# tiborcamargo/KinectPy

Hardware: AMD Instinct MI355X
Metric: Mpoints/sec end-to-end (unproject+filter+ICP), 4-sensor frame (higher is better)
Workload: dtype f64 decisions / f32 storage

## Files before the change

include/kinectpx.h:

```cpp
#ifndef KINECTPX_H
#define KINECTPX_H

#include <stddef.h>
#include <stdint.h>

#ifdef __cplusplus
extern "C" {
#endif

#define KPX_VERSION 100

typedef enum {
    KPX_OK = 0,
    KPX_ERR_INVALID = -1,
    KPX_ERR_WORKSPACE = -2,
    KPX_ERR_RANGE = -3,
    KPX_ERR_HIP = -4,
    KPX_RETRY = 1
} kpx_status;

const char *kpx_last_error(void);
int kpx_version(void);


// ... 124 lines not shown
size_t kpx_kabsch_workspace_bytes(int64_t n_corr);
int kpx_kabsch(const float *src, const float *tgt, const int32_t *corr, int64_t n_corr, double *d_T, void *ws,
               size_t ws_bytes, void *stream);

#define KPX_ICP_POINT_TO_POINT 0
#define KPX_ICP_POINT_TO_PLANE 1
#define KPX_ICP_FIXED 2
size_t kpx_icp_workspace_bytes(int64_t n_src, int64_t n_tgt);
int kpx_icp(const float *src, int64_t n_src, const float *tgt, const float *tgt_normals, int64_t n_tgt,
            double max_dist, const double *h_init, int32_t mode, int32_t max_iteration, double relative_fitness,
            double relative_rmse, int32_t poll_interval, double *d_result, int32_t *idx, double *d2, void *ws,
            size_t ws_bytes, void *stream);


size_t kpx_fpfh_workspace_bytes(int64_t n, int32_t max_nn);
int kpx_fpfh(const float *pts, const float *normals, int64_t n, double radius, int32_t max_nn, double *fpfh, void *ws,
             size_t ws_bytes, void *stream);

size_t kpx_feature_nn_workspace_bytes(int64_t na, int64_t nb);
int kpx_feature_nn(const double *fa, int64_t na, const double *fb, int64_t nb, int32_t *idx, void *ws, size_t ws_bytes,
                   void *stream);

size_t kpx_ransac_workspace_bytes(int64_t n_src, int64_t n_tgt);
int kpx_ransac_corres(const float *src, int64_t n_src, const float *tgt, int64_t n_tgt, const int32_t *corres, int64_t n_corres,
                      double max_dist, int32_t ransac_n, double edge_similarity, int32_t max_iteration, double confidence,
                      uint64_t seed, double *h_result, void *ws, size_t ws_bytes, void *stream);

size_t kpx_icp_batch_workspace_bytes(int32_t count, const int64_t *h_n_src, int64_t n_tgt);
int kpx_icp_batch(int32_t count, const float *const *h_src, const int64_t *h_n_src, const float *tgt,
                  const float *tgt_normals, int64_t n_tgt, double max_dist, const double *h_init, int32_t mode,
                  int32_t max_iteration, double relative_fitness, double relative_rmse, double *d_results, void *ws,
                  size_t ws_bytes, void *stream);

#define KPX_NN_ENGINE_CULLED 0
#define KPX_NN_ENGINE_DENSE 1
#define KPX_NN_ENGINE_DENSE_FP64 2
int kpx_nn_engine(int32_t engine);

size_t kpx_sample_workspace_bytes(int64_t n);
int kpx_sample_points(const float *pts, int64_t n, int64_t k, uint64_t seed, float *out_pts, int32_t *out_idx, void *ws,
                      size_t ws_bytes, void *stream);

size_t kpx_obb_workspace_bytes(int32_t count, int64_t n);
int kpx_obb_batch(const void *pts, int32_t pts_f64, int32_t count, int64_t n, double *d_obb, uint8_t *d_is_vertex, void *ws,
                  size_t ws_bytes, void *stream);

#define KPX_NORM_OBB 0
#define KPX_NORM_OBB_ROT_TRANS 1
#define KPX_NORM_TRANSLATE 2
#define KPX_NORM_OBB_ROT 3
int kpx_normalize_batch(const double *x, int32_t count, int64_t rows, const double *d_obb, int32_t mode, const double *h_M,
                        double *out, void *stream);

size_t kpx_color_gradient_workspace_bytes(int64_t n, int32_t max_nn);
int kpx_color_gradient(const float *pts, const float *normals, const float *colors, int64_t n, double radius, int32_t max_nn,
                       double *grad, void *ws, size_t ws_bytes, void *stream);
size_t kpx_colored_icp_workspace_bytes(int64_t n_src, int64_t n_tgt);
int kpx_colored_icp(const float *src, const float *src_colors, int64_t n_src, const float *tgt, const float *tgt_colors,
                    const float *tgt_normals, const double *tgt_gradient, int64_t n_tgt, double max_dist, const double *h_init,
                    double lambda_geometric, int32_t max_iteration, double relative_fitness, double relative_rmse,
                    int32_t poll_interval, double *d_result, void *ws, size_t ws_bytes, void *stream);

int kpx_gicp_covariances(const float *normals, int64_t n, double epsilon, double *cov, void *stream);
int kpx_rotate_covariances(const double *cov, int64_t n, const double *h_T, double *out, void *stream);
size_t kpx_generalized_icp_workspace_bytes(int64_t n_src, int64_t n_tgt);
int kpx_generalized_icp(const float *src, const double *src_cov, int64_t n_src, const float *tgt, const double *tgt_cov, int64_t n_tgt,
                        double max_dist, const double *h_init, int32_t max_iteration, double relative_fitness, double relative_rmse,
                        int32_t poll_interval, double *d_result, int32_t *idx, double *d2, void *ws, size_t ws_bytes, void *stream);

int kpx_fuse_skeletons(const double *skeletons, int32_t cams, int64_t frames, int32_t joints, double alpha, double beta,
                       int32_t initial_frame, double *out, void *stream);

typedef struct {
    double reg_voxel;
    double icp_max_dist;
    double filt_voxel;
    double filt_ratio;
    double gate;
    int32_t normals_nn;
    int32_t icp_mode;
    int32_t icp_max_iteration;
    int32_t filt_k;
} kpx_frame_params;
size_t kpx_frame_step_workspace_bytes(int32_t sensors, int64_t n_px);
int kpx_frame_step(const uint16_t *depth, const uint8_t *rgb, const float *xy_table, int64_t n_px, int32_t sensors,
                   const double *h_init, const kpx_frame_params *params, float *out_pts, float *out_col, int32_t *h_count,
                   double *h_T, int32_t *h_info, void *ws, size_t ws_bytes, void *stream);
size_t kpx_frame_step_host_workspace_bytes(int32_t sensors, int64_t n_px);
int kpx_frame_step_host(const uint16_t *h_depth, const uint8_t *h_rgb, const float *xy_table, int64_t n_px, int32_t sensors,
                        const double *h_init, const kpx_frame_params *params, float *out_pts, float *out_col, int32_t *h_count,
                        double *h_T, int32_t *h_info, void *ws, size_t ws_bytes, void *stream);

typedef struct kpx_comm kpx_comm;
typedef int (*kpx_bcast_fn)(void *user, void *d_buf, size_t bytes, int32_t root, void *stream);
typedef int (*kpx_allgather_fn)(void *user, const void *d_send, void *d_recv, size_t bytes_per_rank, void *stream);
int kpx_rccl_load(const char *path);
int kpx_rccl_unique_id(void *id128);
int kpx_comm_create_rccl(const void *id128, int32_t rank, int32_t world, kpx_comm **out);
int kpx_comm_create_callbacks(int32_t rank, int32_t world, kpx_bcast_fn bcast, kpx_allgather_fn allgather, void *user, kpx_comm **out);
int kpx_comm_create_replay(int32_t rank, int32_t world, int32_t frames, int32_t first_frame, int32_t stride, int32_t per_frame,
                           const void *const *d_payloads, const size_t *bytes, kpx_comm **out);
int kpx_comm_destroy(kpx_comm *comm);
int kpx_comm_rank(const kpx_comm *comm);
int kpx_comm_world(const kpx_comm *comm);
int kpx_comm_broadcast(kpx_comm *comm, void *d_buf, size_t bytes, int32_t root, void *stream);
int kpx_comm_allgather(kpx_comm *comm, const void *d_send, void *d_recv, size_t bytes_per_rank, void *stream);
int kpx_copy_bytes(void *dst, const void *src, size_t bytes, void *stream, int32_t wait);

typedef struct kpx_order kpx_order;
int kpx_order_create(int32_t depth, kpx_order **out);
int kpx_order_destroy(kpx_order *order);
int kpx_order_submit(kpx_order *order, int64_t *frame);
int kpx_order_block(kpx_order *order, int64_t frame);
int kpx_order_turn_begin(kpx_order *order, int64_t frame, int32_t stage);
int kpx_order_turn_end(kpx_order *order, int64_t frame, int32_t stage);
int kpx_order_skip(kpx_order *order, int64_t frame, int32_t stage);
int kpx_order_finish(kpx_order *order, int64_t frame);
int kpx_order_log(kpx_order *order, int64_t *out, int64_t cap, int64_t *count);

size_t kpx_frame_step_sharded_workspace_bytes(int32_t sensors, int32_t rank, int32_t world, int64_t n_px, int32_t host_input);
int kpx_frame_step_sharded(kpx_comm *comm, kpx_order *order, int64_t frame, const uint16_t *depth, const uint8_t *rgb, int32_t host_input,
                           const float *xy_table, int64_t n_px, int32_t sensors, const double *h_init, const kpx_frame_params *params,
                           int32_t fused_filter, float *out_pts, float *out_col, int32_t *h_count, double *h_T, int32_t *h_info, void *ws,
                           size_t ws_bytes, void *stream);

typedef struct kpx_stream kpx_stream;
size_t kpx_stream_workspace_bytes(int32_t sensors, int32_t rank, int32_t world, int64_t n_px, int32_t depth);
int kpx_stream_create(const float *xy_table, int64_t n_px, int32_t sensors, const double *h_init, const kpx_frame_params *params,
                      int32_t depth, kpx_comm *const *comms, int32_t fused_filter, void *ws, size_t ws_bytes, kpx_stream **out);
int kpx_stream_submit(kpx_stream *stream, const void *depth, const void *rgb, int32_t host_input, float *out_pts, float *out_col);
int kpx_stream_pop(kpx_stream *stream, int32_t *h_count, double *h_T, int32_t *h_info);
int kpx_stream_pending(const kpx_stream *stream);
int kpx_stream_capacity(const kpx_stream *stream);
int kpx_stream_destroy(kpx_stream *stream);
int kpx_stream_stats(const kpx_stream *stream, uint64_t *h_out4);

#define KPX_PROF_NN_MFMA 0
#define KPX_PROF_SOR_KNN 1
#define KPX_PROF_PLANE_SCORE 2
#define KPX_PROF_COMPACT 3
#define KPX_PROF_NN_SCREEN 4
#define KPX_PROF_NN_LOCAL 5
#define KPX_PROF_KERNELS 6
int kpx_prof_begin(int32_t capacity);
int kpx_prof_stride(int32_t stride);
int kpx_prof_end(double *h_ms, int64_t *h_launches, double *h_work);
int kpx_prof_icp_phases(double *h_out8);
int kpx_prof_icp_waves(uint64_t *h_out, int64_t cap_waves, int64_t *h_count);
int kpx_icp_chain(int32_t on);
int kpx_prof_icp_cert(uint64_t *h_out8);
int kpx_prof_icp_chain(uint64_t *h_out3072);

#ifdef __cplusplus
}
#endif
#endif
```

kinectpy_amd/_lib.py:

```python
import ctypes as C
import threading
import weakref
import os

import torch

_HERE = os.path.dirname(os.path.abspath(__file__))
SO_PATH = os.environ.get("KPX_LIBRARY") or os.path.join(_HERE, "libkinectpx.so")

_i64, _i32, _f64, _u64, _vp, _sz = C.c_int64, C.c_int32, C.c_double, C.c_uint64, C.c_void_p, C.c_size_t

SIGNATURES = {
    "kpx_last_error": (C.c_char_p, []),
    "kpx_version": (C.c_int, []),
    "kpx_unproject_u16": (C.c_int, [_vp, _vp, _i64, _i32, _vp, _vp]),
    "kpx_median_workspace_bytes": (_sz, [_i32]),
    "kpx_median_i16": (C.c_int, [_vp, _i64, _i64, _i32, _vp, _vp, _sz, _vp]),
    "kpx_compact_workspace_bytes": (_sz, [_i64, _i32]),
    "kpx_rgbd_compact": (C.c_int, [_vp, _vp, _i64, _i32, _i32, _vp, _f64, _vp, _vp, _vp, _vp, _vp, _sz, _vp]),
    "kpx_depth_to_cloud_workspace_bytes": (_sz, [_i64, _i32]),
    "kpx_depth_to_cloud": (C.c_int, [_vp, _vp, _vp, _i64, _i32, _i32, _f64, _vp, _vp, _vp, _vp, _vp, _sz, _vp]),
    "kpx_transform": (C.c_int, [_vp, _i64, _vp, _vp, _vp]),
    "kpx_rotate": (C.c_int, [_vp, _i64, _vp, _vp, _vp]),
    "kpx_joints_affine_f64": (C.c_int, [_vp, _i64, _vp, _vp, _vp, _vp]),
# ... 8 lines not shown
    "kpx_voxel_workspace_bytes": (_sz, [_i64]),
    "kpx_voxel_downsample": (C.c_int, [_vp, _vp, _vp, _i64, _f64, _vp, _vp, _vp, _vp, _vp, _sz, _vp]),
    "kpx_voxel_batch_workspace_bytes": (_sz, [_i32, _vp]),
    "kpx_voxel_downsample_batch": (C.c_int, [_i32, _vp, _vp, _vp, _f64, _vp, _vp, _vp, _vp, _sz, _vp]),
    "kpx_fuse_voxel_workspace_bytes": (_sz, [_i64]),
    "kpx_fuse_voxel_downsample": (C.c_int, [_i32, _vp, _vp, _vp, _vp, _f64, _vp, _vp, _vp, _vp, _sz, _vp]),
    "kpx_sor_workspace_bytes": (_sz, [_i64, _i32]),
    "kpx_sor": (C.c_int, [_vp, _i64, _i32, _f64, _vp, _vp, _vp, _vp, _vp, _sz, _vp]),
    "kpx_sor_partial": (C.c_int, [_vp, _i64, _i32, _i64, _i64, _vp, _vp, _vp, _sz, _vp]),
    "kpx_sor_finish_workspace_bytes": (_sz, [_i64]),
    "kpx_sor_finish": (C.c_int, [_vp, _vp, _i64, _f64, _vp, _vp, _vp, _vp, _vp, _sz, _vp]),
    "kpx_dbscan_workspace_bytes": (_sz, [_i64]),
    "kpx_cluster_dbscan": (C.c_int, [_vp, _i64, _f64, _i32, _vp, _vp, _vp, _sz, _vp]),
    "kpx_radius_outlier_workspace_bytes": (_sz, [_i64]),
    "kpx_remove_radius_outlier": (C.c_int, [_vp, _i64, _i32, _f64, _vp, _vp, _vp, _sz, _vp]),
    "kpx_fps_workspace_bytes": (_sz, [_i32, _i64]),
    "kpx_farthest_point_sample": (C.c_int, [_vp, _i64, _i32, _i32, _vp, _vp, _vp, _sz, _vp]),
    "kpx_farthest_point_sample_batch": (C.c_int, [_i32, _vp, _vp, _i32, _i32, _vp, _vp, _vp, _sz, _vp]),
    "kpx_normals_workspace_bytes": (_sz, [_i64, _i32]),
    "kpx_estimate_normals": (C.c_int, [_vp, _i64, _f64, _i32, _vp, _vp, _sz, _vp]),
    "kpx_segment_plane_workspace_bytes": (_sz, [_i64, _i32, _i32]),
    "kpx_segment_plane": (C.c_int, [_vp, _i64, _f64, _i32, _i32, _f64, _u64, _vp, _vp, _vp, _vp, _sz, _vp]),
    "kpx_nn_workspace_bytes": (_sz, [_i64, _i64]),
    "kpx_nn_search": (C.c_int, [_vp, _i64, _vp, _i64, _vp, _vp, _vp, _vp, _sz, _vp]),
    "kpx_registration_eval_workspace_bytes": (_sz, [_i64, _i64]),
    "kpx_registration_eval": (C.c_int, [_vp, _i64, _vp, _i64, _vp, _f64, _vp, _vp, _vp, _vp, _sz, _vp]),
    "kpx_kabsch_workspace_bytes": (_sz, [_i64]),
    "kpx_kabsch": (C.c_int, [_vp, _vp, _vp, _i64, _vp, _vp, _sz, _vp]),
    "kpx_icp_workspace_bytes": (_sz, [_i64, _i64]),
    "kpx_icp": (C.c_int, [_vp, _i64, _vp, _vp, _i64, _f64, _vp, _i32, _i32, _f64, _f64, _i32, _vp, _vp, _vp, _vp, _sz, _vp]),
    "kpx_fpfh_workspace_bytes": (_sz, [_i64, _i32]),
    "kpx_fpfh": (C.c_int, [_vp, _vp, _i64, _f64, _i32, _vp, _vp, _sz, _vp]),
    "kpx_feature_nn_workspace_bytes": (_sz, [_i64, _i64]),
    "kpx_feature_nn": (C.c_int, [_vp, _i64, _vp, _i64, _vp, _vp, _sz, _vp]),
    "kpx_ransac_workspace_bytes": (_sz, [_i64, _i64]),
    "kpx_ransac_corres": (C.c_int, [_vp, _i64, _vp, _i64, _vp, _i64, _f64, _i32, _f64, _i32, _f64, _u64, _vp, _vp, _sz, _vp]),
    "kpx_sample_workspace_bytes": (_sz, [_i64]),
    "kpx_sample_points": (C.c_int, [_vp, _i64, _i64, _u64, _vp, _vp, _vp, _sz, _vp]),
    "kpx_obb_workspace_bytes": (_sz, [_i32, _i64]),
    "kpx_obb_batch": (C.c_int, [_vp, _i32, _i32, _i64, _vp, _vp, _vp, _sz, _vp]),
    "kpx_normalize_batch": (C.c_int, [_vp, _i32, _i64, _vp, _i32, _vp, _vp, _vp]),
    "kpx_color_gradient_workspace_bytes": (_sz, [_i64, _i32]),
    "kpx_color_gradient": (C.c_int, [_vp, _vp, _vp, _i64, _f64, _i32, _vp, _vp, _sz, _vp]),
    "kpx_colored_icp_workspace_bytes": (_sz, [_i64, _i64]),
    "kpx_colored_icp": (C.c_int, [_vp, _vp, _i64, _vp, _vp, _vp, _vp, _i64, _f64, _vp, _f64, _i32, _f64, _f64, _i32, _vp, _vp, _sz, _vp]),
    "kpx_covariances_workspace_bytes": (_sz, [_i64, _i32]),
    "kpx_estimate_covariances": (C.c_int, [_vp, _i64, _f64, _i32, _vp, _vp, _sz, _vp]),
    "kpx_gicp_covariances": (C.c_int, [_vp, _i64, _f64, _vp, _vp]),
    "kpx_rotate_covariances": (C.c_int, [_vp, _i64, _vp, _vp, _vp]),
    "kpx_generalized_icp_workspace_bytes": (_sz, [_i64, _i64]),
    "kpx_generalized_icp": (C.c_int, [_vp, _vp, _i64, _vp, _vp, _i64, _f64, _vp, _i32, _f64, _f64, _i32, _vp, _vp, _vp, _vp, _sz, _vp]),
    "kpx_fuse_skeletons": (C.c_int, [_vp, _i32, _i64, _i32, _f64, _f64, _i32, _vp, _vp]),
    "kpx_nn_engine": (C.c_int, [_i32]),
    "kpx_icp_batch_workspace_bytes": (_sz, [_i32, _vp, _i64]),
    "kpx_icp_batch": (C.c_int, [_i32, _vp, _vp, _vp, _vp, _i64, _f64, _vp, _i32, _i32, _f64, _f64, _vp, _vp, _sz, _vp]),
    "kpx_prof_begin": (C.c_int, [_i32]),
    "kpx_prof_stride": (C.c_int, [_i32]),
    "kpx_frame_step_workspace_bytes": (_sz, [_i32, _i64]),
    "kpx_frame_step": (C.c_int, [_vp, _vp, _vp, _i64, _i32, _vp, _vp, _vp, _vp, _vp, _vp, _vp, _vp, _sz, _vp]),
    "kpx_frame_step_host_workspace_bytes": (_sz, [_i32, _i64]),
    "kpx_frame_step_host": (C.c_int, [_vp, _vp, _vp, _i64, _i32, _vp, _vp, _vp, _vp, _vp, _vp, _vp, _vp, _sz, _vp]),
    "kpx_rccl_load": (C.c_int, [_vp]),
    "kpx_rccl_unique_id": (C.c_int, [_vp]),
    "kpx_comm_create_rccl": (C.c_int, [_vp, _i32, _i32, _vp]),
    "kpx_comm_create_callbacks": (C.c_int, [_i32, _i32, _vp, _vp, _vp, _vp]),
    "kpx_comm_create_replay": (C.c_int, [_i32, _i32, _i32, _i32, _i32, _i32, _vp, _vp, _vp]),
    "kpx_comm_destroy": (C.c_int, [_vp]),
    "kpx_comm_rank": (C.c_int, [_vp]),
    "kpx_comm_world": (C.c_int, [_vp]),
    "kpx_comm_broadcast": (C.c_int, [_vp, _vp, _sz, _i32, _vp]),
    "kpx_comm_allgather": (C.c_int, [_vp, _vp, _vp, _sz, _vp]),
    "kpx_copy_bytes": (C.c_int, [_vp, _vp, _sz, _vp, _i32]),
    "kpx_order_create": (C.c_int, [_i32, _vp]),
    "kpx_order_destroy": (C.c_int, [_vp]),
    "kpx_order_submit": (C.c_int, [_vp, _vp]),
    "kpx_order_block": (C.c_int, [_vp, _i64]),
    "kpx_order_turn_begin": (C.c_int, [_vp, _i64, _i32]),
    "kpx_order_turn_end": (C.c_int, [_vp, _i64, _i32]),
    "kpx_order_skip": (C.c_int, [_vp, _i64, _i32]),
    "kpx_order_finish": (C.c_int, [_vp, _i64]),
    "kpx_order_log": (C.c_int, [_vp, _vp, _i64, _vp]),
    "kpx_frame_step_sharded_workspace_bytes": (_sz, [_i32, _i32, _i32, _i64, _i32]),
    "kpx_frame_step_sharded": (C.c_int, [_vp, _vp, _i64, _vp, _vp, _i32, _vp, _i64, _i32, _vp, _vp, _i32, _vp, _vp, _vp, _vp, _vp, _vp, _sz, _vp]),
    "kpx_stream_workspace_bytes": (_sz, [_i32, _i32, _i32, _i64, _i32]),
    "kpx_stream_create": (C.c_int, [_vp, _i64, _i32, _vp, _vp, _i32, _vp, _i32, _vp, _sz, _vp]),
    "kpx_stream_submit": (C.c_int, [_vp, _vp, _vp, _i32, _vp, _vp]),
    "kpx_stream_pop": (C.c_int, [_vp, _vp, _vp, _vp]),
    "kpx_stream_pending": (C.c_int, [_vp]),
    "kpx_stream_capacity": (C.c_int, [_vp]),
    "kpx_stream_destroy": (C.c_int, [_vp]),
    "kpx_stream_stats": (C.c_int, [_vp, _vp]),
    "kpx_sor_select": (C.c_int, [_vp, _vp, C.c_int64, C.c_int32, C.c_double, _vp, _vp, _vp, _vp, _vp, _vp, C.c_size_t, _vp]),
    "kpx_sort_pairs_u32_workspace_bytes": (C.c_size_t, [C.c_int64]),
    "kpx_sort_pairs_u32": (C.c_int, [_vp, _vp, C.c_int64, C.c_int32, _vp, _vp, _vp, C.c_size_t, _vp]),
    "kpx_prof_icp_phases": (C.c_int, [_vp]),
    "kpx_prof_icp_waves": (C.c_int, [_vp, C.c_int64, _vp]),
    "kpx_icp_chain": (C.c_int, [C.c_int32]),
    "kpx_prof_icp_cert": (C.c_int, [_vp]),
    "kpx_prof_icp_chain": (C.c_int, [_vp]),
    "kpx_prof_end": (C.c_int, [_vp, _vp, _vp]),
}

_lib = None


class KinectPxError(RuntimeError):
    pass


def load():
    global _lib
    if _lib is None:
        if not os.path.exists(SO_PATH):
            raise KinectPxError(
                f"{SO_PATH} is missing: build it with `python -c 'import __graft_entry__ as g; g.build()'` "
                "(make -C kinectpy_amd/csrc).  There is no CPU fallback.")
        lib = C.CDLL(SO_PATH)
        for name, (res, args) in SIGNATURES.items():
            fn = getattr(lib, name)
            fn.restype, fn.argtypes = res, args
        _lib = lib
    return _lib


BCAST_FN = C.CFUNCTYPE(C.c_int, C.c_void_p, C.c_void_p, C.c_size_t, C.c_int32, C.c_void_p)
ALLGATHER_FN = C.CFUNCTYPE(C.c_int, C.c_void_p, C.c_void_p, C.c_void_p, C.c_size_t, C.c_void_p)
RETRY = 1


def check(rc):
    if rc != 0:
        msg = load().kpx_last_error().decode() or f"kpx error {rc}"
        raise KinectPxError(msg)


_gpu_checked = False


def device():
    global _gpu_checked
    if not _gpu_checked:
        if not torch.cuda.is_available():
            raise KinectPxError("no ROCm device visible: the kinectpx hot path runs on MI355X only (no CPU fallback)")
        torch.cuda.current_device()
        _gpu_checked = True
    return torch.device("cuda", torch._C._cuda_getDevice())


def _raw_stream():
    device()
    return torch._C._cuda_getCurrentRawStream(torch._C._cuda_getDevice())


def stream_ptr():
    return C.c_void_p(_raw_stream())


def ptr(t):
    if t is None:
        return None
    assert t.is_cuda and t.is_contiguous(), "kinectpx needs contiguous device tensors"
    return C.c_void_p(t.data_ptr())


def hptr(a):
    return a.ctypes.data_as(C.c_void_p)
# ... 49 lines not shown
```

kinectpy_amd/csrc/kpx_common.h:

```cpp
#pragma once
#include <stdlib.h>
#include <hip/hip_runtime.h>
#include <stdint.h>
#include <stdio.h>
#include <string.h>

#include "../../include/kinectpx.h"

#define KPX_EXPORT extern "C" __attribute__((visibility("default")))

namespace kpx {

extern thread_local char g_err[512];
int fail(int code, const char *fmt, ...);

#define KPX_HIP(call)                                                                              \
    do {                                                                                           \
        hipError_t e__ = (call);                                                                   \
        if (e__ != hipSuccess)                                                                     \
            return kpx::fail(KPX_ERR_HIP, "%s failed: %s (%s:%d)", #call, hipGetErrorString(e__),  \
                             __FILE__, __LINE__);                                                  \
    } while (0)
#define KPX_LAUNCH_CHECK() KPX_HIP(hipGetLastError())
#define KPX_REQUIRE(cond, ...)                                                                     \
    do {                                                                                           \
        if (!(cond)) return kpx::fail(KPX_ERR_INVALID, __VA_ARGS__);                               \
    } while (0)

struct Arena {
    char *base;
    size_t off, cap;
    bool dry;
    explicit Arena(void *p, size_t bytes) : base((char *)p), off(0), cap(bytes), dry(p == nullptr) {}
    template <class T> T *get(size_t count)
    {
        size_t bytes = (count * sizeof(T) + 255) & ~(size_t)255;
        T *r = dry ? nullptr : (T *)(base + off);
        off += bytes;
        return r;
    }
    bool ok() const { return dry || off <= cap; }
};
#define KPX_ARENA_CHECK(a)                                                                         \
    do {                                                                                           \
        if (!(a).ok())                                                                             \
            return kpx::fail(KPX_ERR_WORKSPACE, "workspace too small: need %zu bytes, have %zu",   \
                             (a).off, (a).cap);                                                    \
    } while (0)

static inline int64_t cdiv(int64_t a, int64_t b) { return (a + b - 1) / b; }

bool memo_bytes_lookup(unsigned site, int64_t n, size_t *bytes);
void memo_bytes_store(unsigned site, int64_t n, size_t bytes);
template <class F> static inline size_t memo_bytes(unsigned site, int64_t n, F &&query)
{
    size_t b = 0;
    if (memo_bytes_lookup(site, n, &b)) return b;
    b = query();
    memo_bytes_store(site, n, b);
    return b;
}

typedef unsigned int kpx_u4 __attribute__((ext_vector_type(4)));
template <class V> __device__ __forceinline__ V stream_load16(const V *p)
{
    static_assert(sizeof(V) == 16, "16-byte vectors only");
#ifdef KPX_STREAM_PLAIN
    return *p;
#else
    const kpx_u4 r = __builtin_nontemporal_load(reinterpret_cast<const kpx_u4 *>(p));
    V v;
    __builtin_memcpy(&v, &r, 16);
    return v;
#endif
}
template <class V> __device__ __forceinline__ void stream_store16(const V &v, V *p)
{
    static_assert(sizeof(V) == 16, "16-byte vectors only");
#ifdef KPX_STREAM_PLAIN
    *p = v;
#else
    kpx_u4 r;
    __builtin_memcpy(&r, &v, 16);
    __builtin_nontemporal_store(r, reinterpret_cast<kpx_u4 *>(p));
#endif
}
#define KPX_STREAM_LOAD(p) stream_load16(p)
#define KPX_STREAM_STORE(v, p) stream_store16((v), (p))

bool prof_armed();
struct ProfScope {
    int slot;
    hipStream_t st;
    ProfScope(int kernel_id, double work, hipStream_t stream);
    ~ProfScope();
};

constexpr int kWave = 64;

__device__ __forceinline__ int lane_id() { return threadIdx.x & 63; }
__device__ __forceinline__ int wave_id() { return threadIdx.x >> 6; }

template <class T> __device__ __forceinline__ T wave_sum(T v)
{
#pragma unroll
    for (int o = 32; o > 0; o >>= 1) v += __shfl_down(v, o, 64);
    return v;
}
template <class T> __device__ __forceinline__ T wave_min(T v)
{
#pragma unroll
    for (int o = 32; o > 0; o >>= 1) { T t = __shfl_down(v, o, 64); v = t < v ? t : v; }
    return v;
}
template <class T> __device__ __forceinline__ T wave_max(T v)
{
#pragma unroll
    for (int o = 32; o > 0; o >>= 1) { T t = __shfl_down(v, o, 64); v = t > v ? t : v; }
    return v;
}

__device__ __forceinline__ void wave_lds_fence()
{
    __builtin_amdgcn_fence(__ATOMIC_SEQ_CST, "wavefront");
    __builtin_amdgcn_wave_barrier();
}

template <class T> __device__ __forceinline__ T block_sum(T v, T *sh)
{
    v = wave_sum(v);
    __syncthreads();
// ... 365 lines not shown
```

kinectpy_amd/csrc/kpx_extract.hip:

```cpp
#include <stdarg.h>

#include <mutex>

#include "kpx_internal.h"

namespace kpx {

thread_local char g_err[512] = "";
int fail(int code, const char *fmt, ...)
{
    va_list ap;
    va_start(ap, fmt);
    vsnprintf(g_err, sizeof(g_err), fmt, ap);
    va_end(ap);
    return code;
}

static struct {
    bool on = false;
    int stride = 1;
    long long total[KPX_PROF_KERNELS] = {};
    int cap = 0, used = 0;
    hipEvent_t *e0 = nullptr, *e1 = nullptr;
    int *kid = nullptr;
// ... 353 lines not shown
        });
        if (run_cnt) atomicAdd(&mine[run_bin], run_cnt);
    }
    __syncthreads();
    uint32_t c[8];
    int64_t mine_sum = 0;
    {
#pragma unroll
        for (int q = 0; q < 8; ++q) c[q] = 0u;
#pragma unroll
        for (int cp = 0; cp < kMedCopies; ++cp) {
            const uint4 a4 = reinterpret_cast<const uint4 *>(fh + (size_t)cp * kMedWin)[2 * tid], b4 = reinterpret_cast<const uint4 *>(fh + (size_t)cp * kMedWin)[2 * tid + 1];
            c[0] += a4.x; c[1] += a4.y; c[2] += a4.z; c[3] += a4.w; c[4] += b4.x; c[5] += b4.y; c[6] += b4.z; c[7] += b4.w;
        }
#pragma unroll
        for (int q = 0; q < 8; ++q) mine_sum += (int64_t)c[q];
    }
    int64_t incl = mine_sum;
#pragma unroll
    for (int o = 1; o < 64; o <<= 1) { const int64_t t2 = __shfl_up(incl, o, 64); if (lane >= o) incl += t2; }
    if (lane == 63) wsum[wave] = incl;
    __syncthreads();
    if (tid == 0) {
        int64_t runs = 0;
        for (int w = 0; w < kMedFrameThreads / 64; ++w) { const int64_t t2 = wsum[w]; wsum[w] = runs; runs += t2; }
        wsum[kMedFrameThreads / 64] = runs;
        int64_t below = 0;
        for (int b = 0; b < 128; ++b) below += (int64_t)coarse[b];
        const int64_t inwin = runs;
        for (int w = 0; w < 2; ++w) {
            const int64_t r = rank[w];
            if (r < below) {
                int64_t cum = 0;
                for (int b = 0; b < 128; ++b) { if (r < cum + (int64_t)coarse[b]) { s_bin[w] = b; s_rank[w] = r - cum; break; } cum += (int64_t)coarse[b]; }
            } else if (r >= below + inwin) {
                int64_t cum = below + inwin;
                for (int b = 160; b < 256; ++b) { if (r < cum + (int64_t)coarse[b]) { s_bin[w] = b; s_rank[w] = r - cum; break; } cum += (int64_t)coarse[b]; }
            } else {
                s_rank[w] = r - below;
            }
        }
    }
    __syncthreads();
    const int64_t excl = wsum[wave] + incl - mine_sum;
#pragma unroll
    for (int w = 0; w < 2; ++w) {
        const int64_t r = s_rank[w];
        if (s_bin[w] < 0 && r >= excl && r < excl + mine_sum) {
            int64_t cum = excl;
            int found = -1;
#pragma unroll
            for (int q = 0; q < 8; ++q) {
                if (found < 0 && r < cum + (int64_t)c[q]) found = 8 * tid + q;
                cum += (int64_t)c[q];
            }
            s_val[w] = found;
        }
    }
    __syncthreads();
    for (int w = 0; w < 2; ++w) {
        const int b = s_bin[w];
        if (b < 0) continue;
        if (w == 1 && s_bin[0] == b && s_rank[0] == s_rank[1]) { if (tid == 0) s_val[1] = s_val[0]; __syncthreads(); continue; }
        if (tid < 256) fh[tid] = 0u;
        __syncthreads();
        median_frame_scan(p, n, stride, frame_stride, vec, xy, nanmask, [&](uint32_t raw) {
            const unsigned key = (raw & 0xFFFFu) ^ 0x8000u;
            if ((int)(key >> 8) == b) atomicAdd(&fh[key & 255u], 1u);
        });
        __syncthreads();
        if (tid == 0) {
            int64_t cum = 0;
            const int64_t r = s_rank[w];
            for (int q = 0; q < 256; ++q) {
                if (r < cum + (int64_t)fh[q]) { s_val[w] = (int)(int16_t)(uint16_t)((((unsigned)b << 8) | (unsigned)q) ^ 0x8000u); break; }
                cum += (int64_t)fh[q];
            }
        }
        __syncthreads();
    }
    if (tid == 0) d_median[frame] = 0.5 * ((double)s_val[0] + (double)s_val[1]);
}

static int median_impl(const int16_t *v, int64_t n, int64_t stride, int64_t frame_stride, int32_t frames,
                       double *d_median, Arena &a, hipStream_t st, const float *xy = nullptr, void *clear_from = nullptr)
{
    uint32_t *hist = a.get<uint32_t>((size_t)frames * 512);
    MedianSel *sel = a.get<MedianSel>((size_t)frames);
    uint8_t *nanmask = (xy || (a.dry && n > 0)) ? a.get<uint8_t>((size_t)(n / 8 + 1)) : nullptr;
    if (a.dry) return KPX_OK;
    KPX_ARENA_CHECK(a);
    {
        char *c0 = clear_from ? reinterpret_cast<char *>(clear_from) : reinterpret_cast<char *>(hist);
        KPX_HIP(hipMemsetAsync(c0, 0, (size_t)(reinterpret_cast<char *>(hist + (size_t)frames * 512) - c0), st));
    }
    const bool vec = stride == 1 && (n % 8 == 0) && (frame_stride % 8 == 0) && ((uintptr_t)v % 16 == 0) && ((uintptr_t)xy % 16 == 0);
    if (xy && vec)
        hipLaunchKernelGGL(xy_nanmask_kernel, dim3((unsigned)(cdiv(n / 8, 256) > 1024 ? 1024 : cdiv(n / 8, 256))), dim3(256), 0, st, xy, n / 8, nanmask);
    {
        const char *e = getenv("KPX_MEDIAN_FRAME");
        const bool by_frame = e ? e[0] == '1' : (frames >= 64 && n >= 32768);
        if (by_frame) {
            static bool attr_set = false;
            if (!attr_set) {
                KPX_HIP(hipFuncSetAttribute((const void *)median_frame_kernel, hipFuncAttributeMaxDynamicSharedMemorySize, kMedCopies * kMedWin * 4));
                attr_set = true;
            }
            hipLaunchKernelGGL(median_frame_kernel, dim3(frames), dim3(kMedFrameThreads), (size_t)kMedCopies * kMedWin * 4, st, v, n, stride, frame_stride, d_median,
                               xy, (const uint8_t *)(vec ? nanmask : nullptr));
            KPX_LAUNCH_CHECK();
            return KPX_OK;
        }
    }
    const int per_thread = frames >= 64 ? 64 : (frames >= 16 ? 32 : 16);
    int bx = (int)(cdiv(n, 256 * per_thread) < 1 ? 1 : (cdiv(n, 256 * per_thread) > 512 ? 512 : cdiv(n, 256 * per_thread)));
    dim3 grid(bx, frames);
    hipLaunchKernelGGL(median_hist_kernel, grid, dim3(256), 0, st, v, n, stride, frame_stride, sel, hist, 0, xy, nanmask);
    hipLaunchKernelGGL(median_select_kernel, dim3(frames), dim3(64), 0, st, hist, n, sel, d_median, 0);
    hipLaunchKernelGGL(median_hist_kernel, grid, dim3(256), 0, st, v, n, stride, frame_stride, sel, hist, 1, xy, nanmask);
    hipLaunchKernelGGL(median_select_kernel, dim3(frames), dim3(64), 0, st, hist, n, sel, d_median, 1);
    KPX_LAUNCH_CHECK();
    return KPX_OK;
}

struct XyzPred {
    const int16_t *xyz; const uint8_t *rgb; const double *median; int64_t n; int flags; double gate;
    __device__ bool operator()(int64_t i, int f) const
    {
        const int16_t *p = xyz + ((int64_t)f * n + i) * 3;
        int16_t x = p[0], y = p[1], z = p[2];
        bool keep = (x != 0) & (y != 0) & (z != 0);
        if ((flags & KPX_COMPACT_COLOR_MASK) && rgb) {
            const uint8_t *c = rgb + ((int64_t)f * n + i) * 3;
            keep = keep & (c[0] != 0) & (c[1] != 0) & (c[2] != 0);
        }
        if (flags & KPX_COMPACT_DEPTH_GATE) keep = keep & ((double)z <= median[f] + gate);
        return keep;
    }
};
struct XyzEmit {
    const int16_t *xyz; const uint8_t *rgb; int64_t n; float *pts; float *col; int32_t *idx;
    __device__ void operator()(int64_t i, int f, int32_t dst) const
    {
        const int16_t *p = xyz + ((int64_t)f * n + i) * 3;
        int64_t o = ((int64_t)f * n + dst) * 3;
        pts[o] = (float)p[0]; pts[o + 1] = (float)p[1]; pts[o + 2] = (float)p[2];
        if (col && rgb) {
            const uint8_t *c = rgb + ((int64_t)f * n + i) * 3;
            col[o] = (float)((double)c[0] / 255.0); col[o + 1] = (float)((double)c[1] / 255.0); col[o + 2] = (float)((double)c[2] / 255.0);
        }
        if (idx) idx[(int64_t)f * n + dst] = (int32_t)i;
    }
};

struct DepthPred {
    const uint16_t *depth; const float *xy; const uint8_t *rgb; const double *median; int64_t n; int flags; double gate;
    __device__ bool operator()(int64_t i, int f) const
    {
        int16_t x, y, z;
        unproject1(depth[(int64_t)f * n + i], xy[2 * i], xy[2 * i + 1], x, y, z);
        bool keep = (x != 0) & (y != 0) & (z != 0);
        if ((flags & KPX_COMPACT_COLOR_MASK) && rgb) {
            const uint8_t *c = rgb + ((int64_t)f * n + i) * 3;
            keep = keep & (c[0] != 0) & (c[1] != 0) & (c[2] != 0);
        }
        if (flags & KPX_COMPACT_DEPTH_GATE) keep = keep & ((double)z <= median[f] + gate);
        return keep;
    }
};
struct DepthEmit {
    const uint16_t *depth; const float *xy; const uint8_t *rgb; int64_t n; float *pts; float *col; int32_t *idx;
    __device__ void operator()(int64_t i, int f, int32_t dst) const
    {
        int16_t x, y, z;
        unproject1(depth[(int64_t)f * n + i], xy[2 * i], xy[2 * i + 1], x, y, z);
        int64_t o = ((int64_t)f * n + dst) * 3;
        pts[o] = (float)x; pts[o + 1] = (float)y; pts[o + 2] = (float)z;
        if (col && rgb) {
            const uint8_t *c = rgb + ((int64_t)f * n + i) * 3;
            col[o] = (float)((double)c[0] / 255.0); col[o + 1] = (float)((double)c[1] / 255.0); col[o + 2] = (float)((double)c[2] / 255.0);
        }
// ... 192 lines not shown
__global__ __launch_bounds__(kCompactThreads) void depth_onepass_vec_kernel(const uint16_t *__restrict__ depth, const float *__restrict__ xy,
                                                                            const uint8_t *__restrict__ rgb, const double *__restrict__ median,
                                                                            int64_t n, int flags, double gate, unsigned long long *__restrict__ tile_state,
                                                                            float *__restrict__ pts, float *__restrict__ col, int32_t *__restrict__ idx,
                                                                            int32_t *__restrict__ d_count, int frame_major)
{
    __shared__ int sh[kCompactThreads / 64 + 2];
    __shared__ int16_t sp[kCompactTile * 3];
    __shared__ uint8_t sc[COL ? kCompactTile * 3 : 1];
    __shared__ int32_t si[IDX ? kCompactTile : 1];
    const int f = frame_major ? blockIdx.x : blockIdx.y;
    const unsigned tile = frame_major ? blockIdx.y : blockIdx.x, tiles = frame_major ? gridDim.y : gridDim.x;
    const int64_t base = (int64_t)tile * kCompactTile + (int64_t)threadIdx.x * kCompactItems;
    Px8 p;
    p.keep = 0;
    if (base < n) load_px8(depth, xy, rgb, median, n, f, base, flags, gate, p);
    int tot;
    int pos = block_excl_scan(__builtin_popcount(p.keep), sh, &tot);
#pragma unroll
    for (int k = 0; k < 8; ++k)
        if (p.keep & (1u << k)) {
            sp[3 * pos] = p.x[k]; sp[3 * pos + 1] = p.y[k]; sp[3 * pos + 2] = p.z[k];
            if (COL) { sc[3 * pos] = p.c[3 * k]; sc[3 * pos + 1] = p.c[3 * k + 1]; sc[3 * pos + 2] = p.c[3 * k + 2]; }
            if (IDX) si[pos] = (int32_t)(base + k);
            ++pos;
        }
    __syncthreads();
    const int before = lookback_exclusive(tile_state + (int64_t)f * tiles, tile, tot, sh + kCompactThreads / 64 + 1);
    const int64_t o = (int64_t)f * n + before;
    for (int e = threadIdx.x; e < tot * 3; e += kCompactThreads) {
        pts[o * 3 + e] = (float)sp[e];
        if (COL) col[o * 3 + e] = (float)((double)sc[e] / 255.0);
    }
    if (IDX)
        for (int e = threadIdx.x; e < tot; e += kCompactThreads) idx[o + e] = si[e];
    if (tile == tiles - 1 && threadIdx.x == 0) d_count[f] = before + tot;
}

static int32_t max_compact_frames()
{
    static const int32_t lim = [] {
        int dev = 0, y = 0;
        if (hipGetDevice(&dev) != hipSuccess || hipDeviceGetAttribute(&y, hipDeviceAttributeMaxGridDimY, dev) != hipSuccess || y <= 0) y = 65535;
        return (int32_t)y;
    }();
    return lim;
}
static int px8_compact(const uint16_t *depth, const float *xy, const uint8_t *rgb, const double *med, int64_t n, int32_t frames, int32_t flags,
                       double gate, int32_t *counts, float *pts, float *col, int32_t *idx, int32_t *d_count, hipStream_t st, bool state_is_clear = false)
{
    const int32_t tiles = (int32_t)compact_tiles(n);
    const dim3 grid(tiles, frames), thr(kCompactThreads);
    const bool wc = col && rgb;
    static const bool batch_onepass = [] { const char *e = getenv("KPX_ONEPASS_BATCH"); return !(e && e[0] == '0'); }();
    const bool small = use_onepass((int64_t)tiles * frames);
    const bool frame_major = !small && batch_onepass && frames >= 8 && frames <= 65535;
    const bool onepass = small || frame_major;
    const dim3 ogrid = frame_major ? dim3(frames, tiles) : grid;
    unsigned long long *state = reinterpret_cast<unsigned long long *>(counts);
    if (onepass) { if (!state_is_clear) KPX_HIP(hipMemsetAsync(state, 0, (size_t)tiles * frames * sizeof(unsigned long long), st)); }
    else {
        hipLaunchKernelGGL(depth_count_vec_kernel, grid, thr, 0, st, depth, xy, rgb, med, n, flags, gate, counts);
        hipLaunchKernelGGL(compact_scan_kernel, dim3(frames), dim3(compact_scan_threads(tiles)), 0, st, counts, tiles, d_count);
    }
#define KPX_D2C(COL, IDX)                                                                                                       \
    do {                                                                                                                        \
        if (onepass)                                                                                                            \
            hipLaunchKernelGGL((depth_onepass_vec_kernel<COL, IDX>), ogrid, thr, 0, st, depth, xy, rgb, med, n, flags, gate, state, pts, col, idx, d_count, \
                               frame_major ? 1 : 0);                                                                           \
        else                                                                                                                    \
            hipLaunchKernelGGL((depth_scatter_vec_kernel<COL, IDX>), grid, thr, 0, st, depth, xy, rgb, med, n, flags, gate, counts, pts, col, idx);        \
    } while (0)
    if (wc && idx) KPX_D2C(true, true);
    else if (wc) KPX_D2C(true, false);
    else if (idx) KPX_D2C(false, true);
    else KPX_D2C(false, false);
#undef KPX_D2C
    KPX_LAUNCH_CHECK();
    return KPX_OK;
}

static int depth_to_cloud_impl(const uint16_t *depth, const float *xy, const uint8_t *rgb, int64_t n, int32_t frames,
                               int32_t flags, double gate, float *pts, float *col, int32_t *idx, int32_t *d_count,
                               Arena &a, hipStream_t st)
{
    int32_t *counts = a.get<int32_t>((size_t)frames * compact_ws_ints(n));
    double *med = a.get<double>((size_t)frames);
    int rc = KPX_OK;
    const bool gated = (flags & KPX_COMPACT_DEPTH_GATE) != 0;
    if (gated || a.dry)
        rc = median_impl(reinterpret_cast<const int16_t *>(depth), n, 1, n, frames, med, a, st, xy, counts);
    if (a.dry || rc) return rc;
    KPX_ARENA_CHECK(a);
    DepthPred pred{ depth, xy, rgb, med, n, flags, gate };
    DepthEmit emit{ depth, xy, rgb, n, pts, col, idx };
    ProfScope prof(KPX_PROF_COMPACT, (double)frames * (double)n * (2.0 + (rgb ? 3.0 : 0.0)), st);
    const bool vec = (n % 8 == 0) && (((uintptr_t)depth | (uintptr_t)xy) % 16 == 0) && ((uintptr_t)rgb % 8 == 0);
    if (!vec) return compact(pred, emit, n, frames, counts, d_count, st, gated);
    return px8_compact(depth, xy, rgb, med, n, frames, flags, gate, counts, pts, col, idx, d_count, st, gated);
}
KPX_EXPORT int kpx_rgbd_compact(const int16_t *xyz, const uint8_t *rgb, int64_t n, int32_t frames, int32_t flags,
                                const double *d_median, double gate, float *pts, float *col, int32_t *idx,
                                int32_t *d_count, void *ws, size_t ws_bytes, void *stream)
{
    KPX_REQUIRE(n >= 0 && frames > 0, "kpx_rgbd_compact: bad size");
    KPX_REQUIRE(xyz && pts && d_count && ws, "kpx_rgbd_compact: null pointer");
    KPX_REQUIRE(!(flags & KPX_COMPACT_DEPTH_GATE) || d_median, "kpx_rgbd_compact: depth gate needs d_median");
    KPX_REQUIRE(n < ((int64_t)1 << 31), "kpx_rgbd_compact: frame too large");
    KPX_REQUIRE(frames <= max_compact_frames(), "kpx_rgbd_compact: %d frames exceed the device's grid limit of %d per call", frames, max_compact_frames());
    Arena a(ws, ws_bytes);
    int32_t *counts = a.get<int32_t>((size_t)frames * compact_ws_ints(n));
    KPX_ARENA_CHECK(a);
    XyzPred pred{ xyz, rgb, d_median, n, flags, gate };
    XyzEmit emit{ xyz, rgb, n, pts, col, idx };
    if (n == 0) return compact(pred, emit, n, frames, counts, d_count, (hipStream_t)stream);
    const bool vec = (n % 8 == 0) && ((uintptr_t)xyz % 16 == 0) && ((uintptr_t)rgb % 8 == 0);
    if (!vec) return compact(pred, emit, n, frames, counts, d_count, (hipStream_t)stream);
    return px8_compact(reinterpret_cast<const uint16_t *>(xyz), nullptr, rgb, d_median, n, frames, flags, gate, counts, pts, col, idx, d_count,
                       (hipStream_t)stream);
}

KPX_EXPORT size_t kpx_depth_to_cloud_workspace_bytes(int64_t n_px, int32_t frames)
{
    Arena a(nullptr, 0);
    depth_to_cloud_impl(nullptr, nullptr, nullptr, n_px, frames < 1 ? 1 : frames, KPX_COMPACT_DEPTH_GATE, 0, nullptr,
                        nullptr, nullptr, nullptr, a, nullptr);
    return a.off;
}
KPX_EXPORT int kpx_depth_to_cloud(const uint16_t *depth, const float *xy, const uint8_t *rgb, int64_t n_px,
                                  int32_t frames, int32_t flags, double gate, float *pts, float *col, int32_t *idx,
                                  int32_t *d_count, void *ws, size_t ws_bytes, void *stream)
{
    KPX_REQUIRE(n_px > 0 && frames > 0, "kpx_depth_to_cloud: bad size");
    KPX_REQUIRE(depth && xy && pts && d_count && ws, "kpx_depth_to_cloud: null pointer");
    KPX_REQUIRE(n_px < ((int64_t)1 << 31), "kpx_depth_to_cloud: frame too large");
    KPX_REQUIRE(frames <= max_compact_frames(), "kpx_depth_to_cloud: %d frames exceed the device's grid limit of %d per call", frames, max_compact_frames());
    Arena a(ws, ws_bytes);
    return depth_to_cloud_impl(depth, xy, rgb, n_px, frames, flags, gate, pts, col, idx, d_count, a, (hipStream_t)stream);
}
```

kinectpy_amd/csrc/kpx_frame.hip:

```cpp
#include <chrono>
#include <vector>

#include "kpx_internal.h"

namespace kpx {

__global__ void frame_empty_kernel() {}

__global__ void frame_flag_kernel(unsigned long long *flag, unsigned long long seq)
{
    __hip_atomic_store(flag, seq, __ATOMIC_RELEASE, __HIP_MEMORY_SCOPE_SYSTEM);
}
static int frame_wait(hipStream_t st)
{
    static const bool spin = [] { const char *e = getenv("KPX_FRAME_SPIN"); return !(e && e[0] == '0'); }();
    if (!spin) {
        KPX_HIP(hipStreamSynchronize(st));
        return KPX_OK;
    }
    static thread_local unsigned long long *flag = nullptr;
    static thread_local unsigned long long seq = 0;
    if (!flag) {
        KPX_HIP(hipHostMalloc((void **)&flag, 64, hipHostMallocDefault));
        *flag = 0ull;
    }
    ++seq;
    hipLaunchKernelGGL(frame_flag_kernel, dim3(1), dim3(1), 0, st, flag, seq);
    KPX_LAUNCH_CHECK();
    auto t0 = std::chrono::steady_clock::now();
    for (unsigned spins = 0;; ++spins) {
        if (__atomic_load_n(flag, __ATOMIC_ACQUIRE) == seq) return KPX_OK;
        __builtin_ia32_pause();
        if ((spins & 4095u) == 4095u && std::chrono::steady_clock::now() - t0 > std::chrono::milliseconds(1)) {
            const hipError_t q = hipStreamQuery(st);
            if (q == hipSuccess) {
                if (__atomic_load_n(flag, __ATOMIC_ACQUIRE) == seq) return KPX_OK;
                KPX_HIP(hipStreamSynchronize(st));
                if (__atomic_load_n(flag, __ATOMIC_ACQUIRE) == seq) return KPX_OK;
                return fail(KPX_ERR_HIP, "kpx_frame_step: the frame's completion word never arrived");
            }
            if (q != hipErrorNotReady) return fail(KPX_ERR_HIP, "kpx_frame_step: %s while waiting for a read-back", hipGetErrorString(q));
            t0 = std::chrono::steady_clock::now();
        }
    }
}

struct FrameLayout {
    float *full_pts, *mask_pts, *mask_col, *down_pts, *normals, *vox_pts, *vox_col;
    int32_t *vox_cnt, *keep_idx;
    double *icp_res, *sor_stats;
    void *op_ws;
    size_t op_bytes;
};
static size_t max_sz(size_t a, size_t b) { return a > b ? a : b; }
static void frame_carve(Arena &a, int32_t S, int64_t n_px, FrameLayout *L)
{
    const size_t px = (size_t)n_px, all = (size_t)S * px;
    L->full_pts = a.get<float>(all * 3);
    L->mask_pts = a.get<float>(all * 3);
    L->mask_col = a.get<float>(all * 3);
    L->down_pts = a.get<float>(all * 3);
    L->normals = a.get<float>(px * 3);
    L->vox_pts = a.get<float>(all * 3);
    L->vox_col = a.get<float>(all * 3);
    L->keep_idx = a.get<int32_t>(all);
    L->icp_res = a.get<double>((size_t)S * 20 + 1);
    L->vox_cnt = reinterpret_cast<int32_t *>(L->icp_res + (size_t)S * 20);
    L->sor_stats = a.get<double>(4);
    std::vector<int64_t> worst((size_t)S, n_px);
    size_t w = kpx_depth_to_cloud_workspace_bytes(n_px, S);
    w = max_sz(w, kpx_voxel_batch_workspace_bytes(S, worst.data()));
    w = max_sz(w, kpx_normals_workspace_bytes(n_px, KPX_NORMALS_LDS_NN));
    w = max_sz(w, kpx_icp_batch_workspace_bytes(S > 1 ? S - 1 : 1, worst.data(), n_px));
    w = max_sz(w, kpx_fuse_voxel_workspace_bytes((int64_t)all));
    w = max_sz(w, kpx_sor_workspace_bytes((int64_t)all, KPX_SOR_LDS_K));
    w = max_sz(w, kpx_select_workspace_bytes((int64_t)all));
    L->op_bytes = w;
    L->op_ws = a.get<char>(w);
}

}

using namespace kpx;

KPX_EXPORT size_t kpx_frame_step_workspace_bytes(int32_t sensors, int64_t n_px)
{
    if (sensors < 1 || n_px < 1) return 0;
    Arena a(nullptr, 0);
    FrameLayout L;
    frame_carve(a, sensors, n_px, &L);
    return a.off;
}

#define KPX_SUB(call)                    \
    do {                                 \
        const int rc__ = (call);         \
        if (rc__) return rc__;           \
    } while (0)

KPX_EXPORT int kpx_frame_step(const uint16_t *depth, const uint8_t *rgb, const float *xy_table, int64_t n_px, int32_t sensors,
                              const double *h_init, const kpx_frame_params *prm, float *out_pts, float *out_col, int32_t *h_count,
                              double *h_T, int32_t *h_info, void *ws, size_t ws_bytes, void *stream)
{
    KPX_REQUIRE(sensors >= 1 && sensors <= 16 && n_px > 0 && n_px < ((int64_t)1 << 31) / 16, "kpx_frame_step: 1 .. 16 sensors of at most 2^27 pixels");
    KPX_REQUIRE(depth && rgb && xy_table && prm && out_pts && out_col && h_count && h_T && ws, "kpx_frame_step: null pointer");
    KPX_REQUIRE(sensors == 1 || h_init, "kpx_frame_step: initial transforms missing");
    KPX_REQUIRE(prm->icp_mode == KPX_ICP_POINT_TO_POINT || prm->icp_mode == KPX_ICP_POINT_TO_PLANE || prm->icp_mode == KPX_ICP_FIXED, "kpx_frame_step: bad icp_mode");
    const bool fixed = prm->icp_mode == KPX_ICP_FIXED;
    KPX_REQUIRE(prm->filt_k <= KPX_SOR_LDS_K && prm->normals_nn <= KPX_NORMALS_LDS_NN, "kpx_frame_step: filt_k <= %d and normals_nn <= %d (the frame's scratch is "
                "sized for the LDS forms; kpx_sor / kpx_estimate_normals take larger values)", KPX_SOR_LDS_K, KPX_NORMALS_LDS_NN);
    const int S = sensors;
    hipStream_t st = (hipStream_t)stream;
    BusyScope busy;
    static thread_local struct { void *ws; size_t bytes; int S; int64_t n_px; FrameLayout L; size_t off; } cache = { nullptr, 0, 0, 0, {}, 0 };
    FrameLayout L;
    if (cache.ws == ws && cache.bytes == ws_bytes && cache.S == S && cache.n_px == n_px) {
        L = cache.L;
    } else {
        Arena a(ws, ws_bytes);
        frame_carve(a, S, n_px, &L);
        KPX_ARENA_CHECK(a);
        cache.ws = ws; cache.bytes = ws_bytes; cache.S = S; cache.n_px = n_px; cache.L = L; cache.off = a.off;
    }
    static thread_local double *h_d = nullptr;
    static thread_local int32_t *h_i = nullptr;
    if (!h_i) {
        void *blk = nullptr;
        KPX_HIP(hipHostMalloc(&blk, (16 * 20 + 1) * sizeof(double) + 256 * sizeof(int32_t), hipHostMallocDefault));
        h_d = static_cast<double *>(blk);
        h_i = reinterpret_cast<int32_t *>(h_d + (16 * 20 + 1));
    }
    auto negative = [&](const int32_t *c, int n) { for (int i = 0; i < n; ++i) if (c[i] < 0) return c[i]; return 0; };

    if (!fixed) KPX_SUB(kpx_depth_to_cloud(depth, xy_table, nullptr, n_px, S, 0, prm->gate, L.full_pts, nullptr, nullptr, h_i, L.op_ws, L.op_bytes, st));
    else for (int i = 0; i < S; ++i) h_i[i] = 0;
    KPX_SUB(kpx_depth_to_cloud(depth, xy_table, rgb, n_px, S, KPX_COMPACT_COLOR_MASK | KPX_COMPACT_DEPTH_GATE, prm->gate, L.mask_pts, L.mask_col, nullptr,
                               h_i + 16, L.op_ws, L.op_bytes, st));
    static const int extra_dispatches = [] { const char *e = getenv("KPX_FRAME_EXTRA_DISPATCHES"); return e ? atoi(e) : 0; }();
    for (int e = 0; e < extra_dispatches; ++e) hipLaunchKernelGGL(frame_empty_kernel, dim3(1), dim3(64), 0, st);
    std::vector<int64_t> fk((size_t)S), mk((size_t)S), dk((size_t)S);
    std::vector<const float *> p_in((size_t)S), c_in((size_t)S);
    std::vector<float *> p_out((size_t)S);
    for (int i = 0; i < S; ++i) { p_in[(size_t)i] = L.full_pts + (size_t)i * n_px * 3; p_out[(size_t)i] = L.down_pts + (size_t)i * n_px * 3; }
    KPX_SUB(frame_wait(st));
    for (int i = 0; i < S; ++i) { fk[(size_t)i] = h_i[i]; mk[(size_t)i] = h_i[16 + i]; }
    if (negative(h_i, S) || negative(h_i + 16, S)) return fail(KPX_ERR_RANGE, "kpx_frame_step: extraction reported %d", negative(h_i, S) | negative(h_i + 16, S));
    static const bool zorder_on = [] { const char *e = getenv("KPX_FRAME_ZORDER"); return !(e && e[0] == '0'); }();
    const bool zorder = zorder_on && S <= 8;
    static thread_local int spec_bits = 0;
    static const bool speculate = [] { const char *e = getenv("KPX_FRAME_SPECULATE"); return !(e && e[0] == '0'); }();
    if (!speculate) spec_bits = 0;
    for (int i = 0; i < S; ++i) h_i[32 + i] = 0;
    for (int attempt = 0; attempt < 2 && !fixed; ++attempt) {
        KPX_SUB(voxel_downsample_batch_spec(S, p_in.data(), nullptr, fk.data(), prm->reg_voxel, p_out.data(), nullptr, h_i + 32, L.op_ws, L.op_bytes, st,
                                            attempt == 0 ? spec_bits : 0, h_i + 50, zorder));
        KPX_SUB(frame_wait(st));
        const int need = h_i[50];
        const bool narrow = attempt == 0 && spec_bits > 0 && need > spec_bits;
        spec_bits = need > 0 && need <= 32 ? (need + 7) / 8 * 8 : 0;
        if (!narrow) break;
    }
    if (negative(h_i + 32, S)) return fail(KPX_ERR_RANGE, "voxel_size is too small");
    for (int i = 0; i < S; ++i) dk[(size_t)i] = h_i[32 + i];
    for (int q = 0; q < 16; ++q) h_T[q] = (q % 5 == 0) ? 1.0 : 0.0;
    if (h_info) for (int i = 0; i < S; ++i) { h_info[i] = (int32_t)dk[(size_t)i]; h_info[16 + i] = (int32_t)mk[(size_t)i]; h_info[32 + i] = 0; }
    if (fixed)
        for (int i = 1; i < S; ++i)
            for (int q = 0; q < 16; ++q) h_T[16 * i + q] = h_init[16 * (i - 1) + q];
    if (S > 1 && !fixed) {
        const bool plane = prm->icp_mode == KPX_ICP_POINT_TO_PLANE;
        if (plane) KPX_SUB(kpx_estimate_normals(L.down_pts, dk[0], 2.0 * prm->reg_voxel, prm->normals_nn, L.normals, L.op_ws, L.op_bytes, st));
        std::vector<const float *> subs((size_t)S - 1);
        for (int i = 1; i < S; ++i) {
            KPX_REQUIRE(dk[(size_t)i] >= 1 && dk[0] >= 1, "kpx_frame_step: sensor %d has no valid pixel", dk[0] >= 1 ? i : 0);
            subs[(size_t)i - 1] = p_out[(size_t)i];
        }
        KPX_SUB(icp_batch_ordered(S - 1, subs.data(), dk.data() + 1, L.down_pts, plane ? L.normals : nullptr, dk[0], prm->icp_max_dist, h_init, prm->icp_mode,
                                  prm->icp_max_iteration, 1e-6, 1e-6, L.icp_res, L.op_ws, L.op_bytes, st, zorder));
    }
    std::vector<const double *> dT((size_t)S, nullptr);
    for (int i = 0; i < S; ++i) {
        p_in[(size_t)i] = L.mask_pts + (size_t)i * n_px * 3; c_in[(size_t)i] = L.mask_col + (size_t)i * n_px * 3;
        if (i > 0 && !fixed) dT[(size_t)i] = L.icp_res + 20 * (size_t)(i - 1);
    }
    static thread_local int fuse_spec = 0;
    if (!speculate) fuse_spec = 0;
    for (int attempt = 0; attempt < 2; ++attempt) {
        h_i[51] = 0;
        KPX_SUB(fuse_voxel_downsample_dev(S, p_in.data(), c_in.data(), mk.data(), h_T, dT.data(), prm->filt_voxel, L.vox_pts, L.vox_col, L.vox_cnt, L.op_ws,
                                          L.op_bytes, st, attempt == 0 ? fuse_spec : 0, h_i + 51));
        KPX_HIP(hipMemcpyAsync(h_d, L.icp_res, ((size_t)S * 20 + 1) * sizeof(double), hipMemcpyDeviceToHost, st));
        KPX_SUB(frame_wait(st));
        const int need = h_i[51];
        const bool narrow = attempt == 0 && fuse_spec > 0 && need > fuse_spec;
        fuse_spec = (speculate && need > 0 && need <= 32) ? (need + 7) / 8 * 8 : 0;
        if (!narrow) break;
    }
    h_i[48] = *reinterpret_cast<const int32_t *>(h_d + (size_t)S * 20);
    for (int i = 1; i < S && !fixed; ++i)
        if (h_d[20 * (i - 1) + 16] != h_d[20 * (i - 1) + 16]) {
            (void)icp_chain_abort_take();
            return fail(KPX_ERR_HIP, "kpx_frame_step: the one-launch ICP chain of sensor %d gave up waiting for its blocks to become resident; KPX_ICP_CHAIN=0 "
                                     "selects the launch-per-iteration form", i);
        }
    for (int i = 1; i < S && !fixed; ++i) {
        for (int q = 0; q < 16; ++q) h_T[16 * i + q] = h_d[20 * (i - 1) + q];
        if (h_info) h_info[32 + i] = (int32_t)h_d[20 * (i - 1) + 18];
    }
    if (h_i[48] < 0) return fail(KPX_ERR_RANGE, "voxel_size is too small");
    const int64_t M = h_i[48];
    if (h_info) h_info[48] = (int32_t)M;
    *h_count = 0;
    if (M == 0) return KPX_OK;
    KPX_SUB(kpx_sor_select(L.vox_pts, L.vox_col, M, prm->filt_k, prm->filt_ratio, out_pts, out_col, L.keep_idx, h_i + 49, L.sor_stats, L.op_ws, L.op_bytes, st));
    KPX_SUB(frame_wait(st));
    *h_count = h_i[49];
    return KPX_OK;
}

KPX_EXPORT size_t kpx_frame_step_host_workspace_bytes(int32_t sensors, int64_t n_px)
{
    if (sensors < 1 || n_px < 1) return 0;
    Arena a(nullptr, 0);
    a.get<uint16_t>((size_t)sensors * (size_t)n_px);
    a.get<uint8_t>((size_t)sensors * (size_t)n_px * 3);
    return a.off + kpx_frame_step_workspace_bytes(sensors, n_px);
}

KPX_EXPORT int kpx_frame_step_host(const uint16_t *h_depth, const uint8_t *h_rgb, const float *xy_table, int64_t n_px, int32_t sensors,
                                   const double *h_init, const kpx_frame_params *prm, float *out_pts, float *out_col, int32_t *h_count,
                                   double *h_T, int32_t *h_info, void *ws, size_t ws_bytes, void *stream)
{
    KPX_REQUIRE(sensors >= 1 && sensors <= 16 && n_px > 0 && n_px < ((int64_t)1 << 31) / 16, "kpx_frame_step_host: 1 .. 16 sensors of at most 2^27 pixels");
    KPX_REQUIRE(h_depth && h_rgb && ws, "kpx_frame_step_host: null pointer");
    Arena a(ws, ws_bytes);
    const size_t all = (size_t)sensors * (size_t)n_px;
    uint16_t *d_depth = a.get<uint16_t>(all);
    uint8_t *d_rgb = a.get<uint8_t>(all * 3);
    KPX_ARENA_CHECK(a);
    hipStream_t st = (hipStream_t)stream;
    KPX_HIP(hipMemcpyAsync(d_depth, h_depth, all * sizeof(uint16_t), hipMemcpyHostToDevice, st));
    KPX_HIP(hipMemcpyAsync(d_rgb, h_rgb, all * 3, hipMemcpyHostToDevice, st));
    return kpx_frame_step(d_depth, d_rgb, xy_table, n_px, sensors, h_init, prm, out_pts, out_col, h_count, h_T, h_info, (char *)ws + a.off,
                          ws_bytes - a.off, stream);
}

namespace kpx {

int64_t &comm_cap_master(kpx_comm *c);
int64_t &comm_cap_clouds(kpx_comm *c);
int &comm_spec_bits(kpx_comm *c);
int &comm_fuse_bits(kpx_comm *c);

constexpr int kHdrDoubles = 24;

static int shard_first(int n_sensors, int rank, int world)
{
    const int base = n_sensors / world, rem = n_sensors % world;
    return rank * base + (rank < rem ? rank : rem);
}
static int shard_count(int n_sensors, int rank, int world) { return n_sensors / world + (rank < n_sensors % world ? 1 : 0); }
static int64_t round_cap(int64_t need, int64_t worst)
{
    int64_t c = (need + need / 4 + 4095) / 4096 * 4096;
    if (c < 4096) c = 4096;
    return c < worst ? c : worst;
}

struct ShardHeaderArgs {
    int32_t k_max, local, first_is_master;
    int32_t masked[16], down[16];
};
__global__ void shard_header_kernel(double *hdr, ShardHeaderArgs a, const double *icp_res)
{
    const int j = blockIdx.x, t = threadIdx.x;
    if (t >= kHdrDoubles) return;
    double v = 0.0;
    if (j < a.local) {
        const int sub = j - (a.first_is_master ? 1 : 0);
        if (t == 0) v = (double)a.masked[j];
        else if (t == 1) v = (double)a.down[j];
        else if (t < 22) v = sub >= 0 ? icp_res[20 * sub + (t - 2)] : ((t - 2) < 16 && (t - 2) % 5 == 0 ? 1.0 : 0.0);
    } else if (t >= 2 && t < 18 && (t - 2) % 5 == 0) v = 1.0;
    hdr[j * kHdrDoubles + t] = v;
}

struct ShardLayout {
    uint16_t *stage_depth;
    uint8_t *stage_rgb;
    float *full_pts, *mask_pts, *mask_col, *down_pts, *normals, *vox_pts, *vox_col;
    char *msg_master, *xchg_send, *xchg_recv;
    int32_t *keep_idx, *order_idx, *vox_cnt, *keep_cnt;
    double *avg_send, *avg_all, *icp_res, *sor_stats;
    void *op_ws;
    size_t op_bytes, hdr_bytes;
    int k_max;
};
static void shard_carve(Arena &a, int S, int S_l, int world, int64_t n_px, bool host_input, ShardLayout *L)
{
    const size_t px = (size_t)n_px, loc = (size_t)S_l * px, all = (size_t)S * px;
    L->k_max = (S + world - 1) / world;
    L->hdr_bytes = ((size_t)L->k_max * kHdrDoubles * sizeof(double) + 255) & ~(size_t)255;
    L->stage_depth = host_input ? a.get<uint16_t>(loc) : nullptr;
    L->stage_rgb = host_input ? a.get<uint8_t>(loc * 3) : nullptr;
    L->full_pts = a.get<float>(loc * 3);
    L->mask_pts = a.get<float>(loc * 3);
    L->mask_col = a.get<float>(loc * 3);
    L->down_pts = a.get<float>(loc * 3);
    L->normals = a.get<float>(px * 3);
    L->msg_master = a.get<char>(px * 24 + 256);
    const size_t xmsg = (size_t)L->k_max * px * 24 + L->hdr_bytes;
    L->xchg_send = a.get<char>(xmsg);
    L->xchg_recv = a.get<char>(xmsg * (size_t)world);
    L->vox_pts = a.get<float>(all * 3);
    L->vox_col = a.get<float>(all * 3);
    L->keep_idx = a.get<int32_t>(all);
    L->order_idx = a.get<int32_t>(all);
    const size_t rows = (all + (size_t)world - 1) / (size_t)world;
    L->avg_send = a.get<double>(rows);
    L->avg_all = a.get<double>(rows * (size_t)world);
    L->icp_res = a.get<double>((size_t)(S_l > 0 ? S_l : 1) * 20);
    L->vox_cnt = a.get<int32_t>(64);
    L->keep_cnt = L->vox_cnt + 1;
    L->sor_stats = a.get<double>(4);
    std::vector<int64_t> worst((size_t)(S_l > 0 ? S_l : 1), n_px);
    size_t w = kpx_depth_to_cloud_workspace_bytes(n_px, S_l);
    w = max_sz(w, kpx_voxel_batch_workspace_bytes(S_l, worst.data()));
    w = max_sz(w, kpx_normals_workspace_bytes(n_px, KPX_NORMALS_LDS_NN));
    w = max_sz(w, kpx_icp_batch_workspace_bytes(S_l > 0 ? S_l : 1, worst.data(), n_px));
    w = max_sz(w, kpx_fuse_voxel_workspace_bytes((int64_t)all));
    w = max_sz(w, kpx_sor_workspace_bytes((int64_t)all, KPX_SOR_LDS_K));
    w = max_sz(w, kpx_sor_finish_workspace_bytes((int64_t)all));
    w = max_sz(w, kpx_select_workspace_bytes((int64_t)all));
    L->op_bytes = w;
    L->op_ws = a.get<char>(w);
}

static int pinned_block(char **out)
{
    static thread_local char *blk = nullptr;
    if (!blk) {
        void *p = nullptr;
        KPX_HIP(hipHostMalloc(&p, 32768, hipHostMallocDefault));
        blk = static_cast<char *>(p);
    }
    *out = blk;
    return KPX_OK;
}

}

KPX_EXPORT size_t kpx_frame_step_sharded_workspace_bytes(int32_t sensors, int32_t rank, int32_t world, int64_t n_px, int32_t host_input)
{
    if (sensors < 1 || world < 1 || rank < 0 || rank >= world || world > sensors || n_px < 1) return 0;
    Arena a(nullptr, 0);
    ShardLayout L;
    shard_carve(a, sensors, shard_count(sensors, rank, world), world, n_px, host_input != 0, &L);
    return a.off;
}

KPX_EXPORT int kpx_frame_step_sharded(kpx_comm *comm, kpx_order *order, int64_t frame, const uint16_t *depth, const uint8_t *rgb, int32_t host_input,
                                      const float *xy_table, int64_t n_px, int32_t sensors, const double *h_init, const kpx_frame_params *prm,
                                      int32_t fused_filter, float *out_pts, float *out_col, int32_t *h_count, double *h_T, int32_t *h_info, void *ws,
                                      size_t ws_bytes, void *stream)
{
    KPX_REQUIRE(comm, "kpx_frame_step_sharded: communicator missing (kpx_comm_create_*)");
    const int rank = kpx_comm_rank(comm), world = kpx_comm_world(comm), S = sensors;
    KPX_REQUIRE(S >= 1 && S <= 16 && world <= S && n_px > 0 && n_px < ((int64_t)1 << 31) / 16, "kpx_frame_step_sharded: 1 .. 16 sensors on at most as many ranks");
    KPX_REQUIRE(depth && rgb && xy_table && prm && out_pts && out_col && h_count && h_T && ws, "kpx_frame_step_sharded: null pointer");
    KPX_REQUIRE(S == 1 || h_init, "kpx_frame_step_sharded: initial transforms missing");
    KPX_REQUIRE(prm->icp_mode == KPX_ICP_POINT_TO_POINT || prm->icp_mode == KPX_ICP_POINT_TO_PLANE, "kpx_frame_step_sharded: bad icp_mode");
    KPX_REQUIRE(fused_filter >= 0 && fused_filter <= 2, "kpx_frame_step_sharded: fused_filter is 0 (sharded), 1 (rank 0) or 2 (the frames' fuse + filter dealt round robin)");
    const int owner = fused_filter == 2 ? (int)((frame < 0 ? 0 : frame) % world) : 0;
    KPX_REQUIRE(prm->filt_k <= KPX_SOR_LDS_K && prm->normals_nn <= KPX_NORMALS_LDS_NN, "kpx_frame_step_sharded: filt_k <= %d and normals_nn <= %d", KPX_SOR_LDS_K,
                KPX_NORMALS_LDS_NN);
    hipStream_t st = (hipStream_t)stream;
    BusyScope busy;
    const int g0 = shard_first(S, rank, world), S_l = shard_count(S, rank, world);
    const bool owns_master = g0 == 0, plane = prm->icp_mode == KPX_ICP_POINT_TO_PLANE;
    Arena a(ws, ws_bytes);
    ShardLayout L;
    shard_carve(a, S, S_l, world, n_px, host_input != 0, &L);
    KPX_ARENA_CHECK(a);
    const int K = L.k_max;
    char *pin = nullptr;
    KPX_SUB(pinned_block(&pin));
    double *h_d = reinterpret_cast<double *>(pin);
    int32_t *h_i = reinterpret_cast<int32_t *>(pin + 8192);
    double *h_hdr = reinterpret_cast<double *>(pin + 12288);
    auto negative = [&](const int32_t *c, int n) { for (int i = 0; i < n; ++i) if (c[i] < 0) return c[i]; return 0; };
    *h_count = 0;
    if (h_info) memset(h_info, 0, 64 * sizeof(int32_t));

    if (host_input) {
        KPX_HIP(hipMemcpyAsync(L.stage_depth, depth, (size_t)S_l * n_px * sizeof(uint16_t), hipMemcpyHostToDevice, st));
        KPX_HIP(hipMemcpyAsync(L.stage_rgb, rgb, (size_t)S_l * n_px * 3, hipMemcpyHostToDevice, st));
        depth = L.stage_depth;
        rgb = L.stage_rgb;
    }
    KPX_SUB(kpx_depth_to_cloud(depth, xy_table, nullptr, n_px, S_l, 0, prm->gate, L.full_pts, nullptr, nullptr, h_i, L.op_ws, L.op_bytes, st));
    KPX_SUB(kpx_depth_to_cloud(depth, xy_table, rgb, n_px, S_l, KPX_COMPACT_COLOR_MASK | KPX_COMPACT_DEPTH_GATE, prm->gate, L.mask_pts, L.mask_col, nullptr,
                               h_i + 16, L.op_ws, L.op_bytes, st));
    std::vector<int64_t> fk((size_t)S_l), mk((size_t)S_l), dk((size_t)S_l);
    std::vector<const float *> p_in((size_t)S_l);
    std::vector<float *> p_out((size_t)S_l);
    for (int i = 0; i < S_l; ++i) { p_in[(size_t)i] = L.full_pts + (size_t)i * n_px * 3; p_out[(size_t)i] = L.down_pts + (size_t)i * n_px * 3; }
    KPX_SUB(frame_wait(st));
    for (int i = 0; i < S_l; ++i) { fk[(size_t)i] = h_i[i]; mk[(size_t)i] = h_i[16 + i]; }
    int lerr = KPX_OK;
    if (negative(h_i, S_l) || negative(h_i + 16, S_l)) lerr = fail(KPX_ERR_RANGE, "kpx_frame_step_sharded: extraction reported %d", negative(h_i, S_l) | negative(h_i + 16, S_l));
    static const bool zorder_on = [] { const char *e = getenv("KPX_FRAME_ZORDER"); return !(e && e[0] == '0'); }();
    const bool zorder = zorder_on && K <= 8;
    int &spec_bits = comm_spec_bits(comm);
    for (int attempt = 0; attempt < 2 && !lerr; ++attempt) {
        KPX_SUB(voxel_downsample_batch_spec(S_l, p_in.data(), nullptr, fk.data(), prm->reg_voxel, p_out.data(), nullptr, h_i + 32, L.op_ws, L.op_bytes, st,
                                            attempt == 0 ? spec_bits : 0, h_i + 50, zorder));
        KPX_SUB(frame_wait(st));
        const int need = h_i[50];
        const bool narrow = attempt == 0 && spec_bits > 0 && need > spec_bits;
        spec_bits = need > 0 && need <= 32 ? (need + 7) / 8 * 8 : 0;
        if (!narrow) break;
    }
    if (!lerr && negative(h_i + 32, S_l)) lerr = fail(KPX_ERR_RANGE, "voxel_size is too small");
    for (int i = 0; i < S_l; ++i) dk[(size_t)i] = lerr ? 0 : h_i[32 + i];
    for (int i = 0; i < S_l && !lerr; ++i)
        if (dk[(size_t)i] < 1) lerr = fail(KPX_ERR_INVALID, "kpx_frame_step_sharded: sensor %d has no valid pixel", g0 + i);

    static const bool fixed_cap = [] { const char *e = getenv("KPX_SHARD_FIXED_CAP"); return e && e[0] == '1'; }();
    int64_t &cap_m = comm_cap_master(comm);
    if (cap_m <= 0 || fixed_cap) cap_m = n_px;
    const int64_t capm = cap_m;
    static const bool normals_travel = [] { const char *e = getenv("KPX_SHARD_NORMALS"); return !(e && e[0] == '1'); }();
    const bool ship_n = normals_travel && plane && world > 1;
    const size_t row_b = ship_n ? 24 : 12;
    char *msg = L.msg_master;
    float *m_xyz = reinterpret_cast<float *>(msg), *m_nrm = reinterpret_cast<float *>(msg + (size_t)capm * 12);
    double *m_hdr = reinterpret_cast<double *>(msg + (size_t)capm * row_b);
    if (owns_master) {
        if (!lerr && ship_n) lerr = kpx_estimate_normals(L.down_pts, dk[0], 2.0 * prm->reg_voxel, prm->normals_nn, L.normals, L.op_ws, L.op_bytes, st);
        if (!lerr) {
            const size_t rows = (size_t)(dk[0] < capm ? dk[0] : capm);
            KPX_HIP(hipMemcpyAsync(m_xyz, L.down_pts, rows * 12, hipMemcpyDeviceToDevice, st));
            if (ship_n) KPX_HIP(hipMemcpyAsync(m_nrm, L.normals, rows * 12, hipMemcpyDeviceToDevice, st));
        }
        h_d[0] = lerr ? -1.0 : (double)dk[0];
        KPX_HIP(hipMemcpyAsync(m_hdr, h_d, sizeof(double), hipMemcpyHostToDevice, st));
    }
    kpx_order_turn_begin(order, frame, 0);
    int rc = kpx_comm_broadcast(comm, msg, (size_t)capm * row_b + 256, 0, st);
    kpx_order_turn_end(order, frame, 0);
    if (rc) return rc;
    if (owns_master && lerr) {
        kpx_order_finish(order, frame);
        return lerr;
    }
    int64_t m = owns_master ? dk[0] : 0;
    if (!owns_master) {
        KPX_HIP(hipMemcpyAsync(h_d, m_hdr, sizeof(double), hipMemcpyDeviceToHost, st));
        KPX_SUB(frame_wait(st));
        m = (int64_t)h_d[0];
        if (!(m >= 1 && m <= n_px)) {
            kpx_order_finish(order, frame);
            return m < 0 ? fail(KPX_ERR_RANGE, "kpx_frame_step_sharded: rank 0 could not provide the master cloud (see its error)")
                         : fail(KPX_ERR_RANGE, "kpx_frame_step_sharded: bad master header (%lld points)", (long long)m);
        }
    }
    cap_m = fixed_cap ? n_px : round_cap(m, n_px);
    if (m > capm) {
        kpx_order_finish(order, frame);
        return KPX_RETRY;
    }
    const int n_sub = S_l - (owns_master ? 1 : 0);
    if (n_sub > 0 && !lerr) {
        std::vector<const float *> subs((size_t)n_sub);
        std::vector<int64_t> ns((size_t)n_sub);
        for (int j = 0; j < n_sub; ++j) {
            const int i = j + (owns_master ? 1 : 0);
            subs[(size_t)j] = p_out[(size_t)i];
            ns[(size_t)j] = dk[(size_t)i];
        }
        const float *tgt = owns_master ? L.down_pts : m_xyz, *tn = plane ? ((ship_n && !owns_master) ? m_nrm : L.normals) : nullptr;
        if (plane && !ship_n) lerr = kpx_estimate_normals(tgt, m, 2.0 * prm->reg_voxel, prm->normals_nn, L.normals, L.op_ws, L.op_bytes, st);
        const int first_sub = g0 + (owns_master ? 1 : 0);
        if (!lerr)
            lerr = icp_batch_ordered(n_sub, subs.data(), ns.data(), tgt, tn, m, prm->icp_max_dist, h_init + 16 * (size_t)(first_sub - 1), prm->icp_mode,
                                     prm->icp_max_iteration, 1e-6, 1e-6, L.icp_res, L.op_ws, L.op_bytes, st, zorder);
    }
    int64_t &cap_c = comm_cap_clouds(comm);
    const int64_t worst_c = (int64_t)K * n_px;
    if (cap_c <= 0 || fixed_cap) cap_c = worst_c;
    const int64_t capc = cap_c;
    const size_t xbytes = (size_t)capc * 24 + L.hdr_bytes;
    {
        ShardHeaderArgs ha;
        memset(&ha, 0, sizeof(ha));
        ha.k_max = K; ha.local = S_l; ha.first_is_master = owns_master ? 1 : 0;
        int64_t off = 0;
        for (int i = 0; i < S_l; ++i) {
            ha.masked[i] = lerr ? -1 : (int32_t)mk[(size_t)i]; ha.down[i] = (int32_t)dk[(size_t)i];
            int64_t k = capc - off < mk[(size_t)i] ? capc - off : mk[(size_t)i];
            if (k < 0 || lerr) k = 0;
            if (k > 0) {
                KPX_HIP(hipMemcpyAsync(L.xchg_send + (size_t)off * 12, L.mask_pts + (size_t)i * n_px * 3, (size_t)k * 12, hipMemcpyDeviceToDevice, st));
                KPX_HIP(hipMemcpyAsync(L.xchg_send + (size_t)(capc + off) * 12, L.mask_col + (size_t)i * n_px * 3, (size_t)k * 12, hipMemcpyDeviceToDevice, st));
            }
            off += k;
        }
        hipLaunchKernelGGL(shard_header_kernel, dim3((unsigned)K), dim3(32), 0, st, reinterpret_cast<double *>(L.xchg_send + (size_t)capc * 24), ha, L.icp_res);
        KPX_LAUNCH_CHECK();
    }
    kpx_order_turn_begin(order, frame, 1);
    rc = kpx_comm_allgather(comm, L.xchg_send, L.xchg_recv, xbytes, st);
    kpx_order_turn_end(order, frame, 1);
    if (rc) return rc;
    const size_t hrow = (size_t)K * kHdrDoubles * sizeof(double);
    KPX_HIP(hipMemcpy2DAsync(h_hdr, hrow, L.xchg_recv + (size_t)capc * 24, xbytes, hrow, (size_t)world, hipMemcpyDeviceToHost, st));
    KPX_SUB(frame_wait(st));
    std::vector<const float *> f_p((size_t)S), f_c((size_t)S);
    std::vector<int64_t> f_n((size_t)S);
    int64_t need = 0;
    for (int r = 0, g = 0; r < world; ++r) {
        const int own = shard_count(S, r, world);
        int64_t off = 0;
        for (int j = 0; j < own; ++j, ++g) {
            const double *row = h_hdr + ((size_t)r * K + j) * kHdrDoubles;
            const int64_t n = (int64_t)row[0];
            if (!(n >= 0 && n <= n_px)) {
                kpx_order_finish(order, frame);
                if (lerr) return lerr;
                return n < 0 ? fail(KPX_ERR_RANGE, "kpx_frame_step_sharded: rank %d failed on its own sensors (see its error)", r)
                             : fail(KPX_ERR_RANGE, "kpx_frame_step_sharded: bad exchange header (rank %d)", r);
            }
            if (row[2 + 16] != row[2 + 16]) {
                kpx_order_finish(order, frame);
                (void)icp_chain_abort_take();
                return fail(KPX_ERR_HIP, "kpx_frame_step_sharded: the one-launch ICP chain of sensor %d (rank %d) gave up waiting for its blocks to become "
                                         "resident; KPX_ICP_CHAIN=0 selects the launch-per-iteration form", g, r);
            }
            f_p[(size_t)g] = reinterpret_cast<const float *>(L.xchg_recv + (size_t)r * xbytes + (size_t)off * 12);
            f_c[(size_t)g] = reinterpret_cast<const float *>(L.xchg_recv + (size_t)r * xbytes + (size_t)(capc + off) * 12);
            f_n[(size_t)g] = n;
            for (int q = 0; q < 16; ++q) h_T[16 * g + q] = row[2 + q];
            if (h_info) { h_info[g] = (int32_t)row[1]; h_info[16 + g] = (int32_t)n; h_info[32 + g] = g == 0 ? 0 : (int32_t)row[2 + 18]; }
            off += n;
        }
        need = off > need ? off : need;
    }
    cap_c = fixed_cap ? worst_c : round_cap(need, worst_c);
    if (need > capc) {
        kpx_order_finish(order, frame);
        return KPX_RETRY;
    }
    if (fused_filter >= 1 && rank != owner) {
        kpx_order_skip(order, frame, 2);
        return KPX_OK;
    }
    int &fuse_spec = comm_fuse_bits(comm);
    static const bool speculate_fuse = [] { const char *e = getenv("KPX_FRAME_SPECULATE"); return !(e && e[0] == '0'); }();
    if (!speculate_fuse) fuse_spec = 0;
    for (int attempt = 0; attempt < 2; ++attempt) {
        h_i[51] = 0;
        KPX_SUB(fuse_voxel_downsample_dev(S, f_p.data(), f_c.data(), f_n.data(), h_T, nullptr, prm->filt_voxel, L.vox_pts, L.vox_col, L.vox_cnt, L.op_ws,
                                          L.op_bytes, st, attempt == 0 ? fuse_spec : 0, h_i + 51));
        KPX_HIP(hipMemcpyAsync(h_i + 48, L.vox_cnt, sizeof(int32_t), hipMemcpyDeviceToHost, st));
        KPX_SUB(frame_wait(st));
        const int need_bits = h_i[51];
        const bool narrow = attempt == 0 && fuse_spec > 0 && need_bits > fuse_spec;
        fuse_spec = (speculate_fuse && need_bits > 0 && need_bits <= 32) ? (need_bits + 7) / 8 * 8 : 0;
        if (!narrow) break;
    }
    if (h_i[48] < 0) return fail(KPX_ERR_RANGE, "voxel_size is too small");
    const int64_t M = h_i[48];
    if (h_info) h_info[48] = (int32_t)M;
    if (M == 0) {
        kpx_order_skip(order, frame, 2);
        return KPX_OK;
    }
    if (fused_filter >= 1) {
        kpx_order_skip(order, frame, 2);
        KPX_SUB(kpx_sor_select(L.vox_pts, L.vox_col, M, prm->filt_k, prm->filt_ratio, out_pts, out_col, L.keep_idx, h_i + 49, L.sor_stats, L.op_ws, L.op_bytes, st));
        KPX_SUB(frame_wait(st));
        *h_count = h_i[49];
        return KPX_OK;
    }
    const int64_t rows = (M + world - 1) / world;
    const int64_t q0 = rank * rows < M ? rank * rows : M, q1 = (rank + 1) * rows < M ? (rank + 1) * rows : M;
    KPX_SUB(kpx_sor_partial(L.vox_pts, M, prm->filt_k, q0, q1, L.avg_send, L.order_idx, L.op_ws, L.op_bytes, st));
    kpx_order_turn_begin(order, frame, 2);
    rc = kpx_comm_allgather(comm, L.avg_send, L.avg_all, (size_t)rows * sizeof(double), st);
    kpx_order_turn_end(order, frame, 2);
    if (rc) return rc;
    KPX_SUB(kpx_sor_finish(L.avg_all, L.order_idx, M, prm->filt_ratio, L.keep_idx, L.keep_cnt, L.sor_stats, nullptr, L.op_ws, L.op_bytes, st));
    KPX_HIP(hipMemcpyAsync(h_i + 49, L.keep_cnt, sizeof(int32_t), hipMemcpyDeviceToHost, st));
    KPX_SUB(frame_wait(st));
    const int64_t kept = h_i[49];
    if (kept > 0) {
        KPX_SUB(kpx_select_by_index(L.vox_pts, L.vox_col, nullptr, M, L.keep_idx, kept, KPX_SELECT_GATHER, out_pts, out_col, nullptr, nullptr, L.op_ws,
                                    L.op_bytes, st));
        KPX_SUB(frame_wait(st));
    }
    *h_count = (int32_t)kept;
    return KPX_OK;
}
```

kinectpy_amd/csrc/kpx_internal.h:

```cpp
#pragma once
#include "kpx_common.h"

namespace kpx {

constexpr int kBboxBlocks = 1024;
int bbox_f32(const float *pts, int64_t n, double *d_bbox6, double *ws_partials, hipStream_t st);

struct GridParams {
    double org[3];
    double h;
    int32_t dim[3];
    int32_t ncell;
};
constexpr int32_t kGridMaxCells = 1 << 22;

struct Grid {
    GridParams *params;
    uint32_t *cell_start;
    float *sorted_pts;
    int32_t *sorted_idx;
    uint32_t *sorted_keys;
    int32_t *spare;
    int32_t *extra;
};
constexpr int kGridExtraWords = 4104;
int grid_build(const float *pts, int64_t n, double target_per_cell, Arena &a, Grid *g, hipStream_t st);

constexpr int kLaneCount = 4;
struct LaneSet {
    hipStream_t s[kLaneCount];
    hipEvent_t fork, join[kLaneCount];
};
int lanes_get(LaneSet **out);
int lanes_fork(LaneSet *l, hipStream_t caller, int used);
int lanes_join(LaneSet *l, hipStream_t caller, int used);

int voxel_downsample_batch_spec(int32_t count, const float *const *h_pts, const float *const *h_col, const int64_t *h_n, double voxel,
                                float *const *h_opts, float *const *h_ocol, int32_t *d_counts, void *ws, size_t ws_bytes, void *stream,
                                int spec_bits, int32_t *d_bits, bool morton = false);

int fuse_voxel_downsample_dev(int32_t count, const float *const *h_pts, const float *const *h_col, const int64_t *h_n, const double *h_T,
                              const double *const *h_dT, double voxel, float *opts, float *ocol, int32_t *d_count, void *ws, size_t ws_bytes,
                              void *stream, int spec_bits = 0, int32_t *d_bits = nullptr);

struct BusyScope {
    BusyScope();
    ~BusyScope();
    BusyScope(const BusyScope &) = delete;
    BusyScope &operator=(const BusyScope &) = delete;
    bool counted;
};
int busy_threads();
int icp_chain_abort_take();
int icp_batch_ordered(int32_t count, const float *const *h_src, const int64_t *h_n_src, const float *tgt, const float *tgt_normals, int64_t n_tgt,
                      double max_dist, const double *h_init, int32_t mode, int32_t max_iteration, double relative_fitness, double relative_rmse,
                      double *d_results, void *ws, size_t ws_bytes, void *stream, bool presorted);

double nn_local_take_visits();

}
```

kinectpy_amd/csrc/kpx_knn.hip:

```cpp
#include <hipcub/hipcub.hpp>

#include "kpx_gridknn.h"
#include "kpx_morton.h"
#include "kpx_radix.h"
#include "kpx_linalg.h"

namespace kpx {

__device__ __forceinline__ void grid_dims(const double ext[3], double &h, int32_t cell_cap, int dim[3])
{
    for (;;) {
        double tot = 1.0;
        for (int a = 0; a < 3; ++a) {
            double d = floor(ext[a] / h) + 1.0;
            if (d > 1000000.0) d = 1000000.0;
            dim[a] = (int)d; tot *= d;
        }
        if (tot <= (double)cell_cap) break;
        h *= 1.26;
    }
}
__device__ __forceinline__ GridParams grid_params_of(const double *__restrict__ bbox, int64_t n, double target, int32_t cell_cap,
                                                     const unsigned long long *__restrict__ sumsq)
{
// ... 60 lines not shown
    for (int64_t s = (int64_t)blockIdx.x * blockDim.x + threadIdx.x; s < n; s += (int64_t)gridDim.x * blockDim.x) {
        int64_t i = order[s];
        sorted_pts[3 * s] = pts[3 * i]; sorted_pts[3 * s + 1] = pts[3 * i + 1]; sorted_pts[3 * s + 2] = pts[3 * i + 2];
    }
}
__global__ __launch_bounds__(256) void grid_place_kernel(const uint32_t *__restrict__ cell_of, int64_t n, const uint32_t *__restrict__ cell_start,
                                                         uint32_t *__restrict__ cursor, int32_t *__restrict__ slot_idx)
{
    for (int64_t i = (int64_t)blockIdx.x * blockDim.x + threadIdx.x; i < n; i += (int64_t)gridDim.x * blockDim.x) {
        const uint32_t c = cell_of[i];
        slot_idx[cell_start[c] + atomicAdd(&cursor[c], 1u)] = (int32_t)i;
    }
}
__global__ __launch_bounds__(256) void grid_rank_kernel(const float *__restrict__ pts, int64_t n, const uint32_t *__restrict__ cell_of,
                                                        const uint32_t *__restrict__ cell_start, const int32_t *__restrict__ slot_idx,
                                                        int32_t *__restrict__ sorted_idx, float *__restrict__ sorted_pts)
{
    for (int64_t s = (int64_t)blockIdx.x * blockDim.x + threadIdx.x; s < n; s += (int64_t)gridDim.x * blockDim.x) {
        const int32_t i = slot_idx[s];
        const uint32_t c = cell_of[i];
        const int64_t s0 = cell_start[c], s1 = cell_start[c + 1];
        int rank = 0;
        for (int64_t t = s0; t < s1; ++t) rank += slot_idx[t] < i ? 1 : 0;
        const int64_t d = s0 + rank;
        sorted_idx[d] = i;
        sorted_pts[3 * d] = pts[3 * (int64_t)i]; sorted_pts[3 * d + 1] = pts[3 * (int64_t)i + 1]; sorted_pts[3 * d + 2] = pts[3 * (int64_t)i + 2];
    }
}

constexpr int kGridScanItems = 8, kGridScanTile = 256 * kGridScanItems;
constexpr int kGridScanWords = 2 * ((kGridMaxCells + 1 + kGridScanTile - 1) / kGridScanTile) + 2;
__global__ __launch_bounds__(256) void grid_scan_kernel(const uint32_t *__restrict__ counts, int64_t len, uint32_t *__restrict__ out,
                                                        unsigned long long *__restrict__ states)
{
    __shared__ int sh[256 / 64 + 2];
    const int64_t base = (int64_t)blockIdx.x * kGridScanTile + (int64_t)threadIdx.x * kGridScanItems;
    uint32_t v[kGridScanItems];
    int c = 0;
#pragma unroll
    for (int k = 0; k < kGridScanItems; ++k) { v[k] = base + k < len ? counts[base + k] : 0u; c += (int)v[k]; }
    int tot;
    const int ex = block_excl_scan(c, sh, &tot);
    __syncthreads();
    const int before = lookback_exclusive(states, blockIdx.x, tot, sh + 256 / 64 + 1);
    uint32_t run = (uint32_t)(before + ex);
#pragma unroll
    for (int k = 0; k < kGridScanItems; ++k) {
        if (base + k < len) out[base + k] = run;
        run += v[k];
    }
}

int grid_build(const float *pts, int64_t n, double target_per_cell, Arena &a, Grid *g, hipStream_t st)
{
    const size_t nn = (size_t)(n > 0 ? n : 1);
    g->params = a.get<GridParams>(1);
    uint32_t *zero = a.get<uint32_t>(3 * ((size_t)kGridMaxCells + 1) + 32 + kGridExtraWords + kGridScanWords);
    g->cell_start = a.get<uint32_t>((size_t)kGridMaxCells + 1);
    g->sorted_pts = a.get<float>(nn * 3);
    g->sorted_idx = a.get<int32_t>(nn);
    uint32_t *keys_in = a.get<uint32_t>(nn), *keys_out = a.get<uint32_t>(nn);
    g->sorted_keys = keys_out;
    int32_t *vals_in = a.get<int32_t>(nn);
    double *part = a.get<double>((size_t)kBboxBlocks * 6 + 8);
    size_t sort_bytes = 0, scan_bytes = 0;
    sort_bytes = memo_bytes(2, (int64_t)nn, [&] { size_t b = 0; (void)sort_pairs(nullptr, b, keys_in, keys_out, vals_in, g->sorted_idx, (int64_t)nn, 22, st); return b; });
    scan_bytes = memo_bytes(3, 0, [&] { size_t b = 0; (void)hipcub::DeviceScan::ExclusiveSum(nullptr, b, zero, g->cell_start, kGridMaxCells + 1, st); return b; });
    char *tmp = a.get<char>(sort_bytes > scan_bytes ? sort_bytes : scan_bytes);
    RadixScratch rx{};
    const bool own_sort = (int64_t)nn > 65536 && (int64_t)nn <= kRadixMaxPairs;
    radix_carve(a, (int64_t)nn <= kRadixMaxPairs ? (int64_t)nn : kRadixMaxPairs, &rx);
    if (a.dry) return KPX_OK;
    KPX_ARENA_CHECK(a);
    double *bbox = part + (size_t)kBboxBlocks * 6;
    int rc = bbox_f32(pts, n, bbox, part, st);
    if (rc) return rc;
    int32_t cell_cap = 65536;
    while (cell_cap < kGridMaxCells && (int64_t)cell_cap < 16 * n) cell_cap <<= 1;
    g->spare = reinterpret_cast<int32_t *>(zero);
    unsigned long long *sumsq = reinterpret_cast<unsigned long long *>(zero + 16);
    g->extra = reinterpret_cast<int32_t *>(zero + 32);
    unsigned long long *scan_states = reinterpret_cast<unsigned long long *>(zero + 32 + kGridExtraWords);
    uint32_t *count1 = zero + 32 + kGridExtraWords + kGridScanWords, *count2 = count1 + (size_t)cell_cap + 1, *cursor = count2 + (size_t)cell_cap + 1;
    KPX_HIP(hipMemsetAsync(zero, 0, (32 + kGridExtraWords + kGridScanWords + 3 * ((size_t)cell_cap + 1)) * sizeof(uint32_t), st));
    int nb = (int)(cdiv(n, 256) > 4096 ? 4096 : cdiv(n, 256));
    hipLaunchKernelGGL(grid_cell_kernel, dim3(nb), dim3(256), 0, st, pts, n, bbox, target_per_cell, cell_cap, (const unsigned long long *)nullptr, g->params,
                       keys_in, vals_in, count1);
    hipLaunchKernelGGL(grid_occupancy_kernel, dim3(1024), dim3(256), 0, st, count1, g->params, sumsq);
    hipLaunchKernelGGL(grid_cell_kernel, dim3(nb), dim3(256), 0, st, pts, n, bbox, target_per_cell, cell_cap, (const unsigned long long *)sumsq, g->params,
                       keys_in, vals_in, count2);
    static const bool vendor_scan = [] { const char *e = getenv("KPX_GRID_SCAN"); return e && e[0] == '0'; }();
    if (vendor_scan) KPX_HIP(hipcub::DeviceScan::ExclusiveSum(tmp, scan_bytes, count2, g->cell_start, cell_cap + 1, st));
    else
        hipLaunchKernelGGL(grid_scan_kernel, dim3((unsigned)cdiv((int64_t)cell_cap + 1, kGridScanTile)), dim3(256), 0, st, count2, (int64_t)cell_cap + 1, g->cell_start,
                           scan_states);
    static const bool force_sort = [] { const char *e = getenv("KPX_GRID_SORT"); return e && e[0] == '1'; }();
    const bool by_sort = force_sort || n > 65536;
    if (by_sort) {
        if (own_sort) {
            rc = radix_sort_pairs_u32(rx, keys_in, keys_out, vals_in, g->sorted_idx, n, 22, st);
            if (rc) return rc;
        } else {
            KPX_HIP(sort_pairs(tmp, sort_bytes, keys_in, keys_out, vals_in, g->sorted_idx, n, 22, st));
        }
        hipLaunchKernelGGL(grid_gather_kernel, dim3(nb), dim3(256), 0, st, pts, n, g->sorted_idx, g->sorted_pts);
    } else {
        hipLaunchKernelGGL(grid_place_kernel, dim3(nb), dim3(256), 0, st, keys_in, n, g->cell_start, cursor, vals_in);
        hipLaunchKernelGGL(grid_rank_kernel, dim3(nb), dim3(256), 0, st, pts, n, keys_in, g->cell_start, vals_in, g->sorted_idx, g->sorted_pts);
    }
    KPX_LAUNCH_CHECK();
    return KPX_OK;
}

template <int WAVES>
__global__ __launch_bounds__(WAVES * 64) void sor_wave_kernel(const GridParams *__restrict__ gp, const uint32_t *__restrict__ cell_start,
                                                              const float *__restrict__ spts, const int32_t *__restrict__ sidx,
                                                              int64_t q0, int64_t q1, int k, int cap, double *__restrict__ avg,
                                                              const int32_t *__restrict__ in_list, const int32_t *__restrict__ in_count,
                                                              int32_t *__restrict__ fb_list, int32_t *__restrict__ fb_count)
{
    extern __shared__ __align__(16) double lds[];
    __shared__ uint32_t run_s0[WAVES][64];
    __shared__ int32_t run_off[WAVES][64];
    const int wave = threadIdx.x >> 6, lane = threadIdx.x & 63;
    __shared__ __align__(16) uint32_t knn_hist[WAVES][kKnnBuckets];
    const WaveKnnScratch sc{ lds + (size_t)wave * cap, nullptr, run_s0[wave], run_off[wave], cap, knn_hist[wave] };
    const GridParams g = *gp;
    const int64_t nq = in_list ? (int64_t)*in_count : q1 - q0;
    for (int64_t e = (int64_t)blockIdx.x * WAVES + wave; e < nq; e += (int64_t)gridDim.x * WAVES) {
        const int64_t s = in_list ? (int64_t)in_list[e] : q0 + e;
        const double q[3] = { (double)spts[3 * s], (double)spts[3 * s + 1], (double)spts[3 * s + 2] };
        WaveKnnResult res;
        if (!wave_knn_select<false>(g, cell_start, spts, q, k, INFINITY, sc, res)) {
            if (lane == 0) fb_list[atomicAdd(fb_count, 1)] = (int32_t)s;
            continue;
        }
        double sum = 0.0;
        for (int t = lane; t < res.m; t += 64) {
            const double d = sc.vals[t];
            if ((unsigned long long)__double_as_longlong(d) <= res.thr) sum += sqrt(d);
        }
#pragma unroll
        for (int o = 32; o > 0; o >>= 1) sum += __shfl_xor(sum, o, 64);
        const double total = sum - (double)(res.cnt - res.kk) * sqrt(res.top);
        if (lane == 0) avg[sidx ? (int64_t)sidx[s] : s - q0] = res.kk > 0 ? total / (double)res.kk : -1.0;
        wave_lds_fence();
    }
}

__device__ __forceinline__ int dppi(int v, int ctrl_sel)
{
    switch (ctrl_sel) {
    case 1: return __builtin_amdgcn_update_dpp(v, v, 0x121, 0xF, 0xF, false);
    case 2: return __builtin_amdgcn_update_dpp(v, v, 0x122, 0xF, 0xF, false);
    case 4: return __builtin_amdgcn_update_dpp(v, v, 0x124, 0xF, 0xF, false);
    default: return __builtin_amdgcn_update_dpp(v, v, 0x128, 0xF, 0xF, false);
    }
}
template <int L> __device__ __forceinline__ int group_sum_i(int v)
{
    v += dppi(v, 1); v += dppi(v, 2); v += dppi(v, 4); v += dppi(v, 8);
    if (L >= 32) v += __shfl_xor(v, 16, 64);
    if (L >= 64) v += __shfl_xor(v, 32, 64);
    return v;
}
template <int L> __device__ __forceinline__ unsigned group_min_u(unsigned v)
{
// ... 1116 lines not shown
```

kinectpy_amd/csrc/kpx_radix.h:

```cpp
#pragma once
#include "kpx_common.h"

namespace kpx {

constexpr int kRxThreads = 256, kRxWaves = kRxThreads / 64;
constexpr int kRxKeys = 8;
constexpr int kRxTile = kRxThreads * kRxKeys;
constexpr int kRxGroup = 32;
constexpr int kRxAhead = 32;
constexpr int64_t kRadixMaxPairs = (int64_t)kRxTile * kRxGroup * 64;

static inline int64_t radix_tiles(int64_t n) { return cdiv(n > 0 ? n : 1, kRxTile); }
static inline int64_t radix_groups(int64_t n) { return cdiv(radix_tiles(n), kRxGroup); }
static inline int radix_passes(int end_bit) { return end_bit <= 8 ? 1 : (end_bit + 7) / 8; }

struct RadixScratch {
    uint32_t *keys_tmp;
    int32_t *vals_tmp;
    uint32_t *tile_hist;
    uint32_t *group_hist;
};
static inline void radix_carve(Arena &a, int64_t n, RadixScratch *s)
{
    const size_t nn = (size_t)(n > 0 ? n : 1);
// ... 35 lines not shown
    const int tile = blockIdx.x, d = threadIdx.x, wave = threadIdx.x >> 6, lane = threadIdx.x & 63;
    const int64_t base = (int64_t)tile * kRxTile;
    const int tile_n = (int)(n - base < kRxTile ? n - base : kRxTile);

    uint32_t key[kRxKeys];
    int32_t val[kRxKeys];
#pragma unroll
    for (int s = 0; s < kRxKeys; ++s) {
        const int p = wave * (64 * kRxKeys) + s * 64 + lane;
        const bool on = p < tile_n;
        key[s] = on ? keys_in[base + p] : 0xFFFFFFFFu;
        val[s] = on ? vals_in[base + p] : 0;
    }
    const int grp = tile / kRxGroup;
    uint32_t before = 0u, total = 0u;
    for (int g0 = 0; g0 < n_groups; g0 += kRxAhead) {
        uint32_t c[kRxAhead];
#pragma unroll
        for (int u = 0; u < kRxAhead; ++u) c[u] = g0 + u < n_groups ? group_hist[(int64_t)(g0 + u) * 256 + d] : 0u;
#pragma unroll
        for (int u = 0; u < kRxAhead; ++u) { total += c[u]; before += g0 + u < grp ? c[u] : 0u; }
    }
    for (int t0 = grp * kRxGroup; t0 < tile; t0 += kRxAhead) {
        uint32_t c[kRxAhead];
#pragma unroll
        for (int u = 0; u < kRxAhead; ++u) c[u] = t0 + u < tile ? tile_hist[(int64_t)(t0 + u) * 256 + d] : 0u;
#pragma unroll
        for (int u = 0; u < kRxAhead; ++u) before += c[u];
    }
#pragma unroll
    for (int w = 0; w < kRxWaves; ++w) cnt[w][d] = 0u;
    int all;
    const int digit_base = block_excl_scan((int)total, sh, &all);

    uint32_t rank[kRxKeys];
    const unsigned long long lt = (1ull << lane) - 1ull;
#pragma unroll
    for (int s = 0; s < kRxKeys; ++s) {
        const int p = wave * (64 * kRxKeys) + s * 64 + lane;
        const bool on = p < tile_n;
        const uint32_t dg = (key[s] >> shift) & dmask;
        unsigned long long m = __builtin_amdgcn_ballot_w64(on);
#pragma unroll
        for (int b = 0; b < 8; ++b) {
            const unsigned long long bb = __builtin_amdgcn_ballot_w64(((dg >> b) & 1u) != 0u);
            m &= ((dg >> b) & 1u) ? bb : ~bb;
        }
        uint32_t c0 = 0u;
        if (on) c0 = cnt[wave][dg];
        wave_lds_fence();
        rank[s] = c0 + (uint32_t)__builtin_popcountll(m & lt);
        if (on && (m & lt) == 0ull) cnt[wave][dg] = c0 + (uint32_t)__builtin_popcountll(m);
        wave_lds_fence();
    }
    __syncthreads();
    uint32_t tc = 0u;
#pragma unroll
    for (int w = 0; w < kRxWaves; ++w) tc += cnt[w][d];
    int tot;
    const int tstart = block_excl_scan((int)tc, sh, &tot);
    uint32_t run = (uint32_t)tstart;
#pragma unroll
    for (int w = 0; w < kRxWaves; ++w) { woff[w][d] = run; run += cnt[w][d]; }
    sbase[d] = (int64_t)digit_base + (int64_t)before - (int64_t)tstart;
    __syncthreads();
#pragma unroll
    for (int s = 0; s < kRxKeys; ++s) {
        const int p = wave * (64 * kRxKeys) + s * 64 + lane;
        if (p < tile_n) {
            const uint32_t pos = woff[wave][(key[s] >> shift) & dmask] + rank[s];
            skey[pos] = key[s];
            sval[pos] = val[s];
        }
    }
    __syncthreads();
    for (int i = threadIdx.x; i < tile_n; i += kRxThreads) {
        const uint32_t k = skey[i];
        const int64_t o = sbase[(k >> shift) & dmask] + i;
        keys_out[o] = k;
        vals_out[o] = sval[i];
    }
}

static inline int radix_sort_pairs_u32(const RadixScratch &s, const uint32_t *keys_in, uint32_t *keys_out, const int32_t *vals_in, int32_t *vals_out,
                                       int64_t n, int end_bit, hipStream_t st, const void *clear_end = nullptr)
{
    if (n <= 0) return KPX_OK;
    const int passes = radix_passes(end_bit);
    const int tiles = (int)radix_tiles(n), groups = (int)radix_groups(n);
    {
        char *c0 = reinterpret_cast<char *>(s.group_hist);
        const char *c1 = clear_end ? reinterpret_cast<const char *>(clear_end) : c0 + (size_t)passes * groups * 256 * sizeof(uint32_t);
        KPX_HIP(hipMemsetAsync(c0, 0, (size_t)(c1 - c0), st));
    }
    const uint32_t *k_src = keys_in;
    const int32_t *v_src = vals_in;
    for (int p = 0; p < passes; ++p) {
        const bool to_out = ((passes - 1 - p) & 1) == 0;
        uint32_t *k_dst = to_out ? keys_out : s.keys_tmp;
        int32_t *v_dst = to_out ? vals_out : s.vals_tmp;
        uint32_t *gh = s.group_hist + (size_t)p * groups * 256;
        const int bits = end_bit - 8 * p >= 8 ? 8 : (end_bit - 8 * p < 1 ? 1 : end_bit - 8 * p);
        const uint32_t dmask = (1u << bits) - 1u;
        hipLaunchKernelGGL(radix_hist_kernel, dim3(tiles), dim3(kRxThreads), 0, st, k_src, n, 8 * p, dmask, s.tile_hist, gh);
        hipLaunchKernelGGL(radix_scatter_kernel, dim3(tiles), dim3(kRxThreads), 0, st, k_src, v_src, k_dst, v_dst, n, 8 * p, dmask, s.tile_hist, gh, groups);
        k_src = k_dst;
        v_src = v_dst;
    }
    KPX_LAUNCH_CHECK();
    return KPX_OK;
}

}
```

kinectpy_amd/csrc/kpx_stream.hip:

```cpp
#include <atomic>
#include <chrono>
#include <condition_variable>
#include <memory>
#include <mutex>
#include <thread>
#include <vector>

#include "kpx_internal.h"

namespace kpx {

enum : int { kJobEmpty = 0, kJobQueued = 1, kJobRunning = 2, kJobDone = 3 };

struct StreamJob {
    std::atomic<int> state{ kJobEmpty };
    const void *depth = nullptr, *rgb = nullptr;
    int host_input = 0;
    float *out_pts = nullptr, *out_col = nullptr;
    int64_t frame = -1;
    int rc = KPX_OK;
    char err[512] = { 0 };
    int32_t count = 0;
    double T[16 * 16] = { 0.0 };
    int32_t info[64] = { 0 };
// ... 51 lines not shown
            spin_then_wait(S->mu, S->cv_work, [&] {
                if (S->quit.load(std::memory_order_acquire)) return true;
                if (S->sharded) return S->jobs[(size_t)(mine % (uint64_t)S->cap)]->state.load(std::memory_order_acquire) == kJobQueued;
                return S->submitted.load(std::memory_order_acquire) > __atomic_load_n(&S->claimed, __ATOMIC_ACQUIRE);
            });
            if (S->quit.load(std::memory_order_acquire)) return;
            if (S->sharded) {
                j = S->jobs[(size_t)(mine % (uint64_t)S->cap)].get();
                break;
            }
            std::lock_guard<std::mutex> lock(S->mu);
            if (S->submitted.load(std::memory_order_acquire) > S->claimed) {
                j = S->jobs[(size_t)(S->claimed % (uint64_t)S->cap)].get();
                __atomic_store_n(&S->claimed, S->claimed + 1, __ATOMIC_RELEASE);
                break;
            }
        }
        j->state.store(kJobRunning, std::memory_order_relaxed);
        int rc;
        if (S->sharded)
            rc = kpx_frame_step_sharded(s->comm, S->order, j->frame, static_cast<const uint16_t *>(j->depth), static_cast<const uint8_t *>(j->rgb), j->host_input, S->xy,
                                        S->n_px, S->sensors, S->init.data(), &S->prm, S->fused_filter, j->out_pts, j->out_col, &j->count, j->T, j->info, s->ws,
                                        s->ws_bytes, s->st);
        else if (j->host_input)
            rc = kpx_frame_step_host(static_cast<const uint16_t *>(j->depth), static_cast<const uint8_t *>(j->rgb), S->xy, S->n_px, S->sensors, S->init.data(), &S->prm,
                                     j->out_pts, j->out_col, &j->count, j->T, j->info, s->ws, s->ws_bytes, s->st);
        else
            rc = kpx_frame_step(static_cast<const uint16_t *>(j->depth), static_cast<const uint8_t *>(j->rgb), S->xy, S->n_px, S->sensors, S->init.data(), &S->prm,
                                j->out_pts, j->out_col, &j->count, j->T, j->info, s->ws, s->ws_bytes, s->st);
        if (rc < 0) {
            snprintf(j->err, sizeof(j->err), "%s", kpx_last_error());
            (void)hipStreamSynchronize(s->st);
        }
        if (S->sharded) kpx_order_finish(S->order, j->frame);
        j->rc = rc;
        S->frames_done.fetch_add(1, std::memory_order_relaxed);
        if (S->sharded && rc != KPX_RETRY) mine += (uint64_t)S->depth;
        {
            std::lock_guard<std::mutex> lock(S->mu);
            j->state.store(kJobDone, std::memory_order_release);
        }
        S->cv_done.notify_all();
    }
}

static void queue_job(kpx_stream *S, StreamJob *j)
{
    if (S->sharded) (void)kpx_order_submit(S->order, &j->frame);
    {
        std::lock_guard<std::mutex> lock(S->mu);
        j->state.store(kJobQueued, std::memory_order_release);
    }
    S->cv_work.notify_all();
}

}

using namespace kpx;

KPX_EXPORT size_t kpx_stream_workspace_bytes(int32_t sensors, int32_t rank, int32_t world, int64_t n_px, int32_t depth)
{
    if (sensors < 1 || n_px < 1 || depth < 1 || depth > 16 || world < 1 || rank < 0 || rank >= world) return 0;
    const size_t per = world > 1 ? kpx_frame_step_sharded_workspace_bytes(sensors, rank, world, n_px, 1) : kpx_frame_step_host_workspace_bytes(sensors, n_px);
    if (!per) return 0;
    return (size_t)depth * ((per + 255) & ~(size_t)255);
}

KPX_EXPORT int kpx_stream_create(const float *xy_table, int64_t n_px, int32_t sensors, const double *h_init, const kpx_frame_params *prm, int32_t depth,
                                 kpx_comm *const *comms, int32_t fused_filter, void *ws, size_t ws_bytes, kpx_stream **out)
{
    KPX_REQUIRE(out && xy_table && prm && ws, "kpx_stream_create: null pointer");
    KPX_REQUIRE(sensors >= 1 && sensors <= 16 && n_px > 0 && depth >= 1 && depth <= 16, "kpx_stream_create: 1 .. 16 sensors, 1 .. 16 frames in flight");
    KPX_REQUIRE(sensors == 1 || h_init, "kpx_stream_create: initial transforms missing");
    int rank = 0, world = 1;
    if (comms) {
        for (int i = 0; i < depth; ++i) KPX_REQUIRE(comms[i], "kpx_stream_create: one communicator per frame slot");
        rank = kpx_comm_rank(comms[0]);
        world = kpx_comm_world(comms[0]);
    }
    const size_t need = kpx_stream_workspace_bytes(sensors, rank, world, n_px, depth);
    KPX_REQUIRE(need > 0, "kpx_stream_create: bad shape");
    if (ws_bytes < need) return fail(KPX_ERR_WORKSPACE, "workspace too small: need %zu bytes, have %zu", need, ws_bytes);
    std::unique_ptr<kpx_stream> S(new kpx_stream());
    KPX_HIP(hipGetDevice(&S->dev));
    S->depth = depth; S->sensors = sensors; S->n_px = n_px; S->xy = xy_table; S->prm = *prm; S->fused_filter = fused_filter;
    S->sharded = comms != nullptr;
    S->cap = S->sharded ? depth : 2 * depth;
    S->init.assign((size_t)16 * (sensors > 1 ? sensors - 1 : 1), 0.0);
    if (sensors > 1) memcpy(S->init.data(), h_init, sizeof(double) * 16 * (size_t)(sensors - 1));
    if (S->sharded) {
        static const int look_env = [] { const char *e = getenv("KPX_ORDER_LOOKAHEAD"); return e ? atoi(e) : -1; }();
        int look = look_env >= 0 ? look_env : 2;
        if (look > depth - 1) look = depth - 1;
        const int rc = kpx_order_create(look + 1, &S->order);
        if (rc) return rc;
    }
    for (int i = 0; i < S->cap; ++i) S->jobs.emplace_back(new StreamJob());
    const size_t per = need / (size_t)depth;
    for (int i = 0; i < depth; ++i) {
        std::unique_ptr<StreamSlot> s(new StreamSlot());
        s->index = i;
        s->ws = static_cast<char *>(ws) + (size_t)i * per;
        s->ws_bytes = per;
        s->comm = comms ? comms[i] : nullptr;
        if (hipStreamCreateWithFlags(&s->st, hipStreamNonBlocking) != hipSuccess) {
            for (auto &p : S->slots) (void)hipStreamDestroy(p->st);
            if (S->order) kpx_order_destroy(S->order);
            return fail(KPX_ERR_HIP, "kpx_stream_create: hipStreamCreateWithFlags failed");
        }
        S->slots.push_back(std::move(s));
    }
    for (auto &p : S->slots) p->th = std::thread(stream_worker, S.get(), p.get());
    *out = S.release();
    return KPX_OK;
}

KPX_EXPORT int kpx_stream_pending(const kpx_stream *S) { return S ? (int)(S->submitted.load() - S->popped) : 0; }
KPX_EXPORT int kpx_stream_capacity(const kpx_stream *S) { return S ? S->cap : 0; }

KPX_EXPORT int kpx_stream_submit(kpx_stream *S, const void *depth, const void *rgb, int32_t host_input, float *out_pts, float *out_col)
{
    KPX_REQUIRE(S && depth && rgb && out_pts && out_col, "kpx_stream_submit: null pointer");
    const uint64_t n = S->submitted.load(std::memory_order_relaxed);
    KPX_REQUIRE((int)(n - S->popped) < S->cap, "kpx_stream_submit: %d frames queued already (kpx_stream_pop first)", S->cap);
    StreamJob *j = S->jobs[(size_t)(n % (uint64_t)S->cap)].get();
    j->depth = depth; j->rgb = rgb; j->host_input = host_input; j->out_pts = out_pts; j->out_col = out_col;
    if (S->sharded) (void)kpx_order_submit(S->order, &j->frame);
    {
        std::lock_guard<std::mutex> lock(S->mu);
        j->state.store(kJobQueued, std::memory_order_release);
        S->submitted.store(n + 1, std::memory_order_release);
    }
    S->cv_work.notify_all();
    return KPX_OK;
}

KPX_EXPORT int kpx_stream_pop(kpx_stream *S, int32_t *h_count, double *h_T, int32_t *h_info)
{
    KPX_REQUIRE(S && h_count && h_T, "kpx_stream_pop: null pointer");
    KPX_REQUIRE(S->submitted.load() > S->popped, "kpx_stream_pop: no frame in flight");
    StreamJob *j = S->jobs[(size_t)(S->popped % (uint64_t)S->cap)].get();
    for (;;) {
        if (S->sharded) kpx_order_block(S->order, j->frame);
        spin_then_wait(S->mu, S->cv_done, [&] { return j->state.load(std::memory_order_acquire) == kJobDone; });
        if (S->sharded) kpx_order_block(S->order, -1);
        if (j->rc != KPX_RETRY) break;
        queue_job(S, j);
    }
    ++S->popped;
    j->state.store(kJobEmpty, std::memory_order_relaxed);
    if (j->rc < 0) return fail(j->rc, "%s", j->err);
    *h_count = j->count;
    memcpy(h_T, j->T, sizeof(double) * 16 * (size_t)S->sensors);
    if (h_info) memcpy(h_info, j->info, sizeof(j->info));
    return KPX_OK;
}

KPX_EXPORT int kpx_stream_destroy(kpx_stream *S)
{
    if (!S) return KPX_OK;
    int32_t c;
    double T[16 * 16];
    while (S->submitted.load() > S->popped) (void)kpx_stream_pop(S, &c, T, nullptr);
    {
        std::lock_guard<std::mutex> lock(S->mu);
        S->quit.store(true, std::memory_order_release);
// ... 20 lines not shown
```

kinectpy_amd/csrc/kpx_voxel.hip:

```cpp
#include <hipcub/hipcub.hpp>

#include "kpx_internal.h"
#include "kpx_radix.h"

namespace kpx {

__global__ __launch_bounds__(256) void voxel_key_kernel(const float *__restrict__ pts, int64_t n, const double *__restrict__ bbox,
                                                        double voxel, uint64_t *__restrict__ keys, int32_t *__restrict__ vals,
                                                        int32_t *__restrict__ err)
{
    const double ox = bbox[0] - voxel * 0.5, oy = bbox[1] - voxel * 0.5, oz = bbox[2] - voxel * 0.5;
    for (int64_t i = (int64_t)blockIdx.x * blockDim.x + threadIdx.x; i < n; i += (int64_t)gridDim.x * blockDim.x) {
        double fx = floor(((double)pts[3 * i] - ox) / voxel);
        double fy = floor(((double)pts[3 * i + 1] - oy) / voxel);
        double fz = floor(((double)pts[3 * i + 2] - oz) / voxel);
        bool bad = !(fx >= 0.0) || !(fy >= 0.0) || !(fz >= 0.0) || fx >= 2097152.0 || fy >= 2097152.0 || fz >= 2097152.0;
        if (bad) { *err = 1; fx = fy = fz = 0.0; }
        keys[i] = ((uint64_t)fx << 42) | ((uint64_t)fy << 21) | (uint64_t)fz;
        vals[i] = (int32_t)i;
    }
}

template <class Key> struct HeadPredT {
    const Key *keys;
// ... 288 lines not shown
        } else if (b.morton) {
            const int ab[3] = { axis_bits[0], axis_bits[1], axis_bits[2] };
            keys[i] = (Key)(((uint64_t)c << (ab[0] + ab[1] + ab[2])) | voxel_zcode((uint64_t)fx, (uint64_t)fy, (uint64_t)fz, ab));
        }
        else keys[i] = (Key)((((uint64_t)c * DX + (uint64_t)fx) * DY + (uint64_t)fy) * DZ + (uint64_t)fz);
        vals[i] = (int32_t)i;
    }
}
__global__ __launch_bounds__(64) void voxel_batch_locate_kernel(VoxelBatch b, const int32_t *__restrict__ seg_start, const int32_t *__restrict__ d_total,
                                                                const int32_t *__restrict__ err, int32_t *__restrict__ head, int32_t *__restrict__ d_counts)
{
    __shared__ int32_t h[kVoxelBatchMax + 1];
    const int c = threadIdx.x;
    const int32_t m = *d_total;
    if (c <= b.count) {
        int32_t lo = 0, hi = m;
        const int64_t want = b.off[c];
        while (lo < hi) {
            const int32_t mid = lo + (hi - lo) / 2;
            if (seg_start[mid] < want) lo = mid + 1; else hi = mid;
        }
        h[c] = c == b.count ? m : lo;
        head[c] = h[c];
    }
    __syncthreads();
    if (c < b.count) d_counts[c] = err[c] ? KPX_ERR_RANGE : h[c + 1] - h[c];
}
__global__ __launch_bounds__(256) void voxel_batch_mean_kernel(VoxelBatch b, const int32_t *__restrict__ vals, const int32_t *__restrict__ seg_start,
                                                               const int32_t *__restrict__ d_total, const int32_t *__restrict__ head)
{
    const int32_t m_total = *d_total;
    const int64_t total = b.off[b.count];
    for (int64_t m = (int64_t)blockIdx.x * blockDim.x + threadIdx.x; m < m_total; m += (int64_t)gridDim.x * blockDim.x) {
        const int64_t s0 = seg_start[m], s1 = (m + 1 < m_total) ? seg_start[m + 1] : total;
        const int c = voxel_batch_cloud(b, s0);
        const float *pts = b.pts[c], *col = b.col[c];
        const int64_t base = b.off[c];
        double sp[3] = { 0, 0, 0 }, sc[3] = { 0, 0, 0 };
        for (int64_t s = s0; s < s1; s += 8) {
            const int cnt = (int)(s1 - s < 8 ? s1 - s : 8);
            int64_t p[8];
#pragma unroll
            for (int k = 0; k < 8; ++k) p[k] = k < cnt ? (int64_t)vals[s + k] - base : -1;
            float vp[8][3], vc[8][3];
#pragma unroll
            for (int k = 0; k < 8; ++k) {
                if (p[k] < 0) continue;
#pragma unroll
                for (int a = 0; a < 3; ++a) {
                    vp[k][a] = pts[3 * p[k] + a];
                    if (col) vc[k][a] = col[3 * p[k] + a];
                }
            }
#pragma unroll
            for (int k = 0; k < 8; ++k) {
                if (p[k] < 0) continue;
#pragma unroll
                for (int a = 0; a < 3; ++a) {
                    sp[a] += (double)vp[k][a];
                    if (col) sc[a] += (double)vc[k][a];
                }
            }
        }
        const double cn = (double)(s1 - s0);
        const int64_t o = m - head[c];
        float *opts = b.opts[c], *ocol = b.ocol[c];
#pragma unroll
        for (int a = 0; a < 3; ++a) {
            opts[3 * o + a] = (float)(sp[a] / cn);
            if (col && ocol) ocol[3 * o + a] = (float)(sc[a] / cn);
        }
    }
}

struct VoxelBatchScratch {
    uint64_t *keys_in, *keys_out;
    int32_t *vals_in, *vals_out, *seg_start, *counts, *err, *head, *d_total;
    double *part, *bbox;
    char *sort_tmp;
    size_t sort_bytes;
    RadixScratch rx;
    char *counts_end;
};
static void voxel_batch_carve(Arena &a, int64_t total, VoxelBatchScratch *s)
{
    const size_t nn = (size_t)(total > 0 ? total : 1);
    s->keys_in = a.get<uint64_t>(nn); s->keys_out = a.get<uint64_t>(nn);
    s->vals_in = a.get<int32_t>(nn); s->vals_out = a.get<int32_t>(nn);
    s->seg_start = a.get<int32_t>(nn);
    s->err = a.get<int32_t>(kVoxelBatchMax);
    s->head = a.get<int32_t>(kVoxelBatchMax + 1);
    s->d_total = a.get<int32_t>(1);
    s->part = a.get<double>((size_t)kVoxelBatchMax * kVoxelBatchBboxBlocks * 6);
    s->bbox = a.get<double>((size_t)kVoxelBatchMax * 8);
    s->sort_bytes = memo_bytes(5, (int64_t)nn, [&] { size_t b = 0; (void)hipcub::DeviceRadixSort::SortPairs(nullptr, b, s->keys_in, s->keys_out, s->vals_in, s->vals_out, (int)nn, 0, 64, (hipStream_t) nullptr); return b; });
    s->sort_tmp = a.get<char>(s->sort_bytes);
    radix_carve(a, total <= kRadixMaxPairs ? total : kRadixMaxPairs, &s->rx);
    s->counts = a.get<int32_t>((size_t)compact_ws_ints(total));
    s->counts_end = reinterpret_cast<char *>(s->counts + (size_t)compact_ws_ints(total));
}
static int voxel_batch_impl(const VoxelBatch &b, double voxel, int32_t *d_counts, Arena &a, hipStream_t st, int spec_bits = 0,
                            int32_t *d_bits = nullptr)
{
    const int64_t total = b.off[b.count];
    VoxelBatchScratch s;
    voxel_batch_carve(a, total, &s);
    KPX_ARENA_CHECK(a);
    hipLaunchKernelGGL(voxel_batch_bbox_partial_kernel, dim3(kVoxelBatchBboxBlocks, b.count), dim3(256), 0, st, b, s.part);
    hipLaunchKernelGGL(voxel_batch_bbox_final_kernel, dim3(b.count), dim3(64), 0, st, s.part, s.bbox, s.err);
    const int nb = (int)(cdiv(total, 256) > 4096 ? 4096 : cdiv(total, 256));
    int end_bit = 64;
    int32_t *bits_out = nullptr;
    if (spec_bits > 0 && d_bits) {
        bits_out = d_bits;
        end_bit = spec_bits > 64 ? 64 : spec_bits;
    } else if (total > (int64_t)128 * 1024) {
        static thread_local int32_t *h_bits = nullptr;
        if (!h_bits) KPX_HIP(hipHostMalloc((void **)&h_bits, sizeof(int32_t), hipHostMallocDefault));
        hipLaunchKernelGGL(voxel_batch_bits_kernel, dim3(1), dim3(1), 0, st, b, s.bbox, voxel, s.head);
        KPX_HIP(hipMemcpyAsync(h_bits, s.head, sizeof(int32_t), hipMemcpyDeviceToHost, st));
        if (d_bits) KPX_HIP(hipMemcpyAsync(d_bits, s.head, sizeof(int32_t), hipMemcpyDefault, st));
        KPX_HIP(hipStreamSynchronize(st));
        end_bit = *h_bits < 1 ? 1 : (*h_bits > 64 ? 64 : *h_bits);
    } else if (d_bits) {
        hipLaunchKernelGGL(voxel_batch_bits_kernel, dim3(1), dim3(1), 0, st, b, s.bbox, voxel, d_bits);
    }
    size_t bytes = s.sort_bytes;
    int rc;
    if (end_bit <= 32) {
        uint32_t *k_in = reinterpret_cast<uint32_t *>(s.keys_in), *k_out = reinterpret_cast<uint32_t *>(s.keys_out);
        hipLaunchKernelGGL(voxel_batch_key_kernel<uint32_t>, dim3(nb), dim3(256), 0, st, b, s.bbox, voxel, k_in, s.vals_in, s.err, bits_out);
        static const bool vendor_sort = [] { const char *e = getenv("KPX_RADIX"); return e && e[0] == '0'; }();
        bool cleared = false;
        if (total <= kRadixMaxPairs && !vendor_sort) {
            rc = radix_sort_pairs_u32(s.rx, k_in, k_out, s.vals_in, s.vals_out, total, end_bit, st, s.counts_end);
            if (rc) return rc;
            cleared = true;
        } else {
            KPX_HIP(hipcub::DeviceRadixSort::SortPairs(s.sort_tmp, bytes, k_in, k_out, s.vals_in, s.vals_out, (int)total, 0, end_bit, st));
        }
        rc = compact(HeadPredT<uint32_t>{ k_out }, HeadEmit{ s.seg_start }, total, 1, s.counts, s.d_total, st, cleared);
    } else {
        hipLaunchKernelGGL(voxel_batch_key_kernel<uint64_t>, dim3(nb), dim3(256), 0, st, b, s.bbox, voxel, s.keys_in, s.vals_in, s.err, bits_out);
        KPX_HIP(hipcub::DeviceRadixSort::SortPairs(s.sort_tmp, bytes, s.keys_in, s.keys_out, s.vals_in, s.vals_out, (int)total, 0, end_bit, st));
        rc = compact(HeadPred{ s.keys_out }, HeadEmit{ s.seg_start }, total, 1, s.counts, s.d_total, st);
    }
    if (rc) return rc;
    hipLaunchKernelGGL(voxel_batch_locate_kernel, dim3(1), dim3(64), 0, st, b, s.seg_start, s.d_total, s.err, s.head, d_counts);
    hipLaunchKernelGGL(voxel_batch_mean_kernel, dim3(nb), dim3(256), 0, st, b, s.vals_out, s.seg_start, s.d_total, s.head);
    KPX_LAUNCH_CHECK();
    return KPX_OK;
}

constexpr int kFuseMax = 16;
constexpr int kFuseBboxBlocks = 32;
struct FuseBatch {
    const float *pts[kFuseMax];
    const float *col[kFuseMax];
    int64_t off[kFuseMax + 1];
    double T[kFuseMax][12];
    const double *dT[kFuseMax];
    int32_t count;
};
__device__ __forceinline__ int fuse_cloud(const FuseBatch &b, int64_t i)
{
    int c = 0;
#pragma unroll
    for (int k = 1; k < kFuseMax; ++k) c += (k < b.count && i >= b.off[k]) ? 1 : 0;
    return c;
}
__device__ __forceinline__ void fuse_point(const FuseBatch &b, int c, int64_t j, double o[3])
{
    const float *p = b.pts[c] + 3 * j;
    const double x = p[0], y = p[1], z = p[2];
    const double *T = b.dT[c] ? b.dT[c] : b.T[c];
#pragma unroll
    for (int k = 0; k < 3; ++k) o[k] = fma(T[4 * k], x, fma(T[4 * k + 1], y, fma(T[4 * k + 2], z, T[4 * k + 3])));
}
__global__ __launch_bounds__(256) void fuse_bbox_partial_kernel(FuseBatch b, double *__restrict__ part)
{
    __shared__ double sh[6][4];
    const int c = blockIdx.y;
    const int64_t n = b.off[c + 1] - b.off[c];
    double mn[3] = { INFINITY, INFINITY, INFINITY }, mx[3] = { -INFINITY, -INFINITY, -INFINITY };
    for (int64_t i = (int64_t)blockIdx.x * blockDim.x + threadIdx.x; i < n; i += (int64_t)gridDim.x * blockDim.x) {
        double q[3];
        fuse_point(b, c, i, q);
#pragma unroll
        for (int a = 0; a < 3; ++a) { mn[a] = fmin(mn[a], q[a]); mx[a] = fmax(mx[a], q[a]); }
    }
#pragma unroll
    for (int a = 0; a < 3; ++a) { mn[a] = wave_min(mn[a]); mx[a] = wave_max(mx[a]); }
    if (lane_id() == 0)
        for (int a = 0; a < 3; ++a) { sh[a][wave_id()] = mn[a]; sh[3 + a][wave_id()] = mx[a]; }
    __syncthreads();
    if (threadIdx.x < 6) {
        double v = sh[threadIdx.x][0];
        for (int w = 1; w < 4; ++w) v = threadIdx.x < 3 ? fmin(v, sh[threadIdx.x][w]) : fmax(v, sh[threadIdx.x][w]);
        part[((int64_t)c * kFuseBboxBlocks + blockIdx.x) * 6 + threadIdx.x] = v;
    }
}
__global__ __launch_bounds__(64) void fuse_bbox_final_kernel(const double *__restrict__ part, int rows, double *__restrict__ bbox, int32_t *__restrict__ err)
{
    const int lane = lane_id();
    double v[6] = { INFINITY, INFINITY, INFINITY, -INFINITY, -INFINITY, -INFINITY };
    for (int r = lane; r < rows; r += 64) {
#pragma unroll
        for (int a = 0; a < 3; ++a) { v[a] = fmin(v[a], part[(int64_t)r * 6 + a]); v[3 + a] = fmax(v[3 + a], part[(int64_t)r * 6 + 3 + a]); }
    }
#pragma unroll
    for (int a = 0; a < 3; ++a) { v[a] = wave_min(v[a]); v[3 + a] = wave_max(v[3 + a]); }
    if (lane == 0) {
        for (int a = 0; a < 6; ++a) bbox[a] = v[a];
        *err = 0;
    }
}
__global__ __launch_bounds__(256) void fuse_key_kernel(FuseBatch b, const double *__restrict__ bbox, double voxel, uint64_t *__restrict__ keys,
                                                       int32_t *__restrict__ vals, int32_t *__restrict__ err)
{
    const double ox = bbox[0] - voxel * 0.5, oy = bbox[1] - voxel * 0.5, oz = bbox[2] - voxel * 0.5;
    const int64_t total = b.off[b.count];
    for (int64_t i = (int64_t)blockIdx.x * blockDim.x + threadIdx.x; i < total; i += (int64_t)gridDim.x * blockDim.x) {
        const int c = fuse_cloud(b, i);
        double q[3];
        fuse_point(b, c, i - b.off[c], q);
        double fx = floor((q[0] - ox) / voxel), fy = floor((q[1] - oy) / voxel), fz = floor((q[2] - oz) / voxel);
        const bool bad = !(fx >= 0.0) || !(fy >= 0.0) || !(fz >= 0.0) || fx >= 2097152.0 || fy >= 2097152.0 || fz >= 2097152.0;
        if (bad) { *err = 1; fx = fy = fz = 0.0; }
        keys[i] = ((uint64_t)fx << 42) | ((uint64_t)fy << 21) | (uint64_t)fz;
        vals[i] = (int32_t)i;
    }
}
__device__ __forceinline__ int fuse_key_bits(const double *__restrict__ bbox, double voxel, double d[3], bool *sane_out)
{
    const double o[3] = { bbox[0] - voxel * 0.5, bbox[1] - voxel * 0.5, bbox[2] - voxel * 0.5 };
#pragma unroll
    for (int a = 0; a < 3; ++a) d[a] = floor((bbox[3 + a] - o[a]) / voxel) + 1.0;
    const bool sane = d[0] >= 1.0 && d[1] >= 1.0 && d[2] >= 1.0 && d[0] < 2097152.0 && d[1] < 2097152.0 && d[2] < 2097152.0;
    int bits = 64;
    if (sane && d[0] * d[1] * d[2] < 18446744073709551616.0) {
        const unsigned long long range = (unsigned long long)d[0] * (unsigned long long)d[1] * (unsigned long long)d[2];
        bits = 1;
        while (bits < 64 && (range >> bits) != 0ull) ++bits;
    }
    *sane_out = sane;
    return bits;
}
__global__ void fuse_bits_kernel(const double *__restrict__ bbox, double voxel, int32_t *__restrict__ bits_out)
{
    double d[3];
    bool sane;
    *bits_out = fuse_key_bits(bbox, voxel, d, &sane);
}
__global__ __launch_bounds__(256) void fuse_key32_kernel(FuseBatch b, const double *__restrict__ bbox, double voxel, uint32_t *__restrict__ keys,
                                                         int32_t *__restrict__ vals, int32_t *__restrict__ bits_out)
{
    const double ox = bbox[0] - voxel * 0.5, oy = bbox[1] - voxel * 0.5, oz = bbox[2] - voxel * 0.5;
    double dd[3];
    bool sane;
    const int bits = fuse_key_bits(bbox, voxel, dd, &sane);
    const double dx = dd[0], dy = dd[1], dz = dd[2];
    if (blockIdx.x == 0 && threadIdx.x == 0) *bits_out = bits;
    const unsigned long long DY = sane ? (unsigned long long)dy : 1ull, DZ = sane ? (unsigned long long)dz : 1ull;
    const int64_t total = b.off[b.count];
    for (int64_t i = (int64_t)blockIdx.x * blockDim.x + threadIdx.x; i < total; i += (int64_t)gridDim.x * blockDim.x) {
        const int c = fuse_cloud(b, i);
        double q[3];
        fuse_point(b, c, i - b.off[c], q);
        double fx = floor((q[0] - ox) / voxel), fy = floor((q[1] - oy) / voxel), fz = floor((q[2] - oz) / voxel);
        if (!(fx >= 0.0) || !(fy >= 0.0) || !(fz >= 0.0) || !(fx < dx) || !(fy < dy) || !(fz < dz)) fx = fy = fz = 0.0;
        keys[i] = (uint32_t)(((unsigned long long)fx * DY + (unsigned long long)fy) * DZ + (unsigned long long)fz);
        vals[i] = (int32_t)i;
    }
}
__global__ __launch_bounds__(256) void fuse_mean_kernel(FuseBatch b, const int32_t *__restrict__ vals, const int32_t *__restrict__ seg_start,
                                                        int32_t *__restrict__ d_count, const int32_t *__restrict__ err, float *__restrict__ opts,
                                                        float *__restrict__ ocol)
{
    const int32_t m_total = *d_count;
    if (blockIdx.x == 0 && threadIdx.x == 0 && *err) *d_count = KPX_ERR_RANGE;
    const int64_t total = b.off[b.count];
    for (int64_t m = (int64_t)blockIdx.x * blockDim.x + threadIdx.x; m < m_total; m += (int64_t)gridDim.x * blockDim.x) {
        const int64_t s0 = seg_start[m], s1 = (m + 1 < m_total) ? seg_start[m + 1] : total;
        double sp[3] = { 0, 0, 0 }, sc[3] = { 0, 0, 0 };
        for (int64_t s = s0; s < s1; s += 8) {
            const int cnt = (int)(s1 - s < 8 ? s1 - s : 8);
            int64_t p[8];
            int cl[8];
#pragma unroll
            for (int k = 0; k < 8; ++k) {
                p[k] = k < cnt ? (int64_t)vals[s + k] : -1;
                cl[k] = p[k] >= 0 ? fuse_cloud(b, p[k]) : 0;
            }
            double vq[8][3];
            float vc[8][3];
#pragma unroll
            for (int k = 0; k < 8; ++k) {
                if (p[k] < 0) continue;
                const int64_t j = p[k] - b.off[cl[k]];
                fuse_point(b, cl[k], j, vq[k]);
                const float *col = b.col[cl[k]];
#pragma unroll
                for (int a = 0; a < 3; ++a) vc[k][a] = col ? col[3 * j + a] : 0.0f;
            }
#pragma unroll
            for (int k = 0; k < 8; ++k) {
                if (p[k] < 0) continue;
#pragma unroll
                for (int a = 0; a < 3; ++a) { sp[a] += vq[k][a]; sc[a] += (double)vc[k][a]; }
            }
        }
        const double cn = (double)(s1 - s0);
#pragma unroll
        for (int a = 0; a < 3; ++a) {
            opts[3 * m + a] = (float)(sp[a] / cn);
            if (ocol) ocol[3 * m + a] = (float)(sc[a] / cn);
        }
    }
}
struct FuseScratch {
    uint64_t *keys_in, *keys_out;
    int32_t *vals_in, *vals_out, *seg_start, *counts, *err;
    double *part, *bbox;
    char *sort_tmp;
    size_t sort_bytes;
    RadixScratch rx;
    char *counts_end;
};
static void fuse_carve(Arena &a, int64_t total, FuseScratch *s)
{
    const size_t nn = (size_t)(total > 0 ? total : 1);
    s->keys_in = a.get<uint64_t>(nn); s->keys_out = a.get<uint64_t>(nn);
    s->vals_in = a.get<int32_t>(nn); s->vals_out = a.get<int32_t>(nn);
    s->seg_start = a.get<int32_t>(nn);
    radix_carve(a, total <= kRadixMaxPairs ? total : kRadixMaxPairs, &s->rx);
    s->counts = a.get<int32_t>((size_t)compact_ws_ints(total));
    s->counts_end = reinterpret_cast<char *>(s->counts + (size_t)compact_ws_ints(total));
    s->err = a.get<int32_t>(1);
    s->part = a.get<double>((size_t)kFuseMax * kFuseBboxBlocks * 6);
    s->bbox = a.get<double>(8);
    s->sort_bytes = memo_bytes(6, (int64_t)nn, [&] { size_t b = 0; (void)hipcub::DeviceRadixSort::SortPairs(nullptr, b, s->keys_in, s->keys_out, s->vals_in, s->vals_out, (int)nn, 0, 63, (hipStream_t) nullptr); return b; });
    s->sort_tmp = a.get<char>(s->sort_bytes);
}
static int fuse_voxel_impl(const FuseBatch &b, double voxel, float *opts, float *ocol, int32_t *d_count, Arena &a, hipStream_t st, int spec_bits = 0,
                           int32_t *d_bits = nullptr)
{
    const int64_t total = b.off[b.count];
    FuseScratch s;
    fuse_carve(a, total, &s);
    KPX_ARENA_CHECK(a);
    hipLaunchKernelGGL(fuse_bbox_partial_kernel, dim3(kFuseBboxBlocks, b.count), dim3(256), 0, st, b, s.part);
    hipLaunchKernelGGL(fuse_bbox_final_kernel, dim3(1), dim3(64), 0, st, s.part, b.count * kFuseBboxBlocks, s.bbox, s.err);
    const int nb = (int)(cdiv(total, 256) > 4096 ? 4096 : cdiv(total, 256));
    if (spec_bits > 0 && spec_bits <= 32 && d_bits && total <= kRadixMaxPairs) {
        uint32_t *k_in = reinterpret_cast<uint32_t *>(s.keys_in), *k_out = reinterpret_cast<uint32_t *>(s.keys_out);
        hipLaunchKernelGGL(fuse_key32_kernel, dim3(nb), dim3(256), 0, st, b, s.bbox, voxel, k_in, s.vals_in, d_bits);
        int rc = radix_sort_pairs_u32(s.rx, k_in, k_out, s.vals_in, s.vals_out, total, spec_bits, st, s.counts_end);
        if (rc) return rc;
        rc = compact(HeadPredT<uint32_t>{ k_out }, HeadEmit{ s.seg_start }, total, 1, s.counts, d_count, st, true);
        if (rc) return rc;
        hipLaunchKernelGGL(fuse_mean_kernel, dim3(nb), dim3(256), 0, st, b, s.vals_out, s.seg_start, d_count, s.err, opts, ocol);
        KPX_LAUNCH_CHECK();
        return KPX_OK;
    }
    if (d_bits) hipLaunchKernelGGL(fuse_bits_kernel, dim3(1), dim3(1), 0, st, s.bbox, voxel, d_bits);
    hipLaunchKernelGGL(fuse_key_kernel, dim3(nb), dim3(256), 0, st, b, s.bbox, voxel, s.keys_in, s.vals_in, s.err);
    size_t bytes = s.sort_bytes;
    KPX_HIP(hipcub::DeviceRadixSort::SortPairs(s.sort_tmp, bytes, s.keys_in, s.keys_out, s.vals_in, s.vals_out, (int)total, 0, 63, st));
    int rc = compact(HeadPred{ s.keys_out }, HeadEmit{ s.seg_start }, total, 1, s.counts, d_count, st);
    if (rc) return rc;
    hipLaunchKernelGGL(fuse_mean_kernel, dim3(nb), dim3(256), 0, st, b, s.vals_out, s.seg_start, d_count, s.err, opts, ocol);
    KPX_LAUNCH_CHECK();
    return KPX_OK;
}

}

using namespace kpx;

KPX_EXPORT size_t kpx_fuse_voxel_workspace_bytes(int64_t total)
{
    Arena a(nullptr, 0);
    FuseScratch s;
    fuse_carve(a, total, &s);
    return a.off;
}
KPX_EXPORT int kpx_fuse_voxel_downsample(int32_t count, const float *const *h_pts, const float *const *h_col, const int64_t *h_n,
                                         const double *h_T, double voxel, float *opts, float *ocol, int32_t *d_count, void *ws,
                                         size_t ws_bytes, void *stream)
{
    return kpx::fuse_voxel_downsample_dev(count, h_pts, h_col, h_n, h_T, nullptr, voxel, opts, ocol, d_count, ws, ws_bytes, stream, 0, nullptr);
}
int kpx::fuse_voxel_downsample_dev(int32_t count, const float *const *h_pts, const float *const *h_col, const int64_t *h_n, const double *h_T,
                                   const double *const *h_dT, double voxel, float *opts, float *ocol, int32_t *d_count, void *ws, size_t ws_bytes,
                                   void *stream, int spec_bits, int32_t *d_bits)
{
    KPX_REQUIRE(voxel > 0.0, "voxel_size <= 0");
    KPX_REQUIRE(count >= 1 && count <= kFuseMax, "kpx_fuse_voxel_downsample: 1 .. %d clouds", kFuseMax);
    KPX_REQUIRE(h_pts && h_n && h_T && d_count && ws, "kpx_fuse_voxel_downsample: null pointer");
    hipStream_t st = (hipStream_t)stream;
    FuseBatch b;
    b.count = count;
    b.off[0] = 0;
    bool any_col = false, all_col = true;
    for (int i = 0; i < kFuseMax; ++i) {
        const bool on = i < count;
        if (on) {
            KPX_REQUIRE(h_n[i] >= 0 && (h_n[i] == 0 || h_pts[i]), "kpx_fuse_voxel_downsample: bad cloud %d", i);
            if (h_n[i] > 0) { const bool hc = h_col && h_col[i]; any_col |= hc; all_col &= hc; }
        }
        b.pts[i] = on ? h_pts[i] : nullptr;
        b.col[i] = (on && h_col) ? h_col[i] : nullptr;
        b.off[i + 1] = b.off[i] + (on ? h_n[i] : 0);
        for (int k = 0; k < 12; ++k) b.T[i][k] = on ? h_T[16 * i + k] : 0.0;
        b.dT[i] = (on && h_dT) ? h_dT[i] : nullptr;
    }
    const int64_t total = b.off[count];
    KPX_REQUIRE(total < ((int64_t)1 << 31), "kpx_fuse_voxel_downsample: bad size");
    KPX_REQUIRE(!ocol || !any_col || all_col, "kpx_fuse_voxel_downsample: colours on some clouds only");
    if (total == 0) { KPX_HIP(hipMemsetAsync(d_count, 0, sizeof(int32_t), st)); return KPX_OK; }
    KPX_REQUIRE(opts, "kpx_fuse_voxel_downsample: null pointer");
    Arena a(ws, ws_bytes);
    return fuse_voxel_impl(b, voxel, opts, (any_col && all_col) ? ocol : nullptr, d_count, a, st, spec_bits, d_bits);
}

KPX_EXPORT size_t kpx_voxel_workspace_bytes(int64_t n)
{
    Arena a(nullptr, 0);
    voxel_impl(nullptr, nullptr, nullptr, n, 1.0, nullptr, nullptr, nullptr, nullptr, a, nullptr);
    Arena one(nullptr, 0);
    VoxelBatchScratch s;
    voxel_batch_carve(one, n, &s);
    return a.off > one.off ? a.off : one.off;
}
KPX_EXPORT int kpx_voxel_downsample(const float *pts, const float *col, const float *nrm, int64_t n, double voxel,
                                    float *opts, float *ocol, float *onrm, int32_t *d_count, void *ws, size_t ws_bytes,
                                    void *stream)
{
    KPX_REQUIRE(voxel > 0.0, "voxel_size <= 0");
    KPX_REQUIRE(n >= 0 && n < ((int64_t)1 << 31), "kpx_voxel_downsample: bad size");
    KPX_REQUIRE(d_count && ws, "kpx_voxel_downsample: null pointer");
    hipStream_t st = (hipStream_t)stream;
    if (n == 0) { KPX_HIP(hipMemsetAsync(d_count, 0, sizeof(int32_t), st)); return KPX_OK; }
    KPX_REQUIRE(pts && opts, "kpx_voxel_downsample: null pointer");
    Arena a(ws, ws_bytes);
    static const bool single_batch = [] { const char *e = getenv("KPX_VOXEL_SINGLE"); return !(e && e[0] == '0'); }();
    if (!nrm && single_batch) {
        VoxelBatch b;
        b.count = 1;
        b.morton = 0;
        b.off[0] = 0;
        for (int i = 0; i < kVoxelBatchMax; ++i) {
            b.pts[i] = i == 0 ? pts : nullptr;
            b.col[i] = i == 0 ? col : nullptr;
            b.opts[i] = i == 0 ? opts : nullptr;
            b.ocol[i] = (i == 0 && col) ? ocol : nullptr;
            b.off[i + 1] = n;
        }
        return voxel_batch_impl(b, voxel, d_count, a, st);
    }
    return voxel_impl(pts, col, nrm, n, voxel, opts, ocol, onrm, d_count, a, st);
}

KPX_EXPORT size_t kpx_voxel_batch_workspace_bytes(int32_t count, const int64_t *h_n)
{
    if (count < 1 || !h_n) return 0;
    Arena a(nullptr, 0);
    int64_t total = 0;
    for (int i = 0; i < count; ++i) {
        voxel_impl(nullptr, nullptr, nullptr, h_n[i], 1.0, nullptr, nullptr, nullptr, nullptr, a, nullptr);
        total += h_n[i] > 0 ? h_n[i] : 0;
    }
    Arena one(nullptr, 0);
    VoxelBatchScratch s;
    voxel_batch_carve(one, total, &s);
    return a.off > one.off ? a.off : one.off;
}
KPX_EXPORT int kpx_voxel_downsample_batch(int32_t count, const float *const *h_pts, const float *const *h_col, const int64_t *h_n,
                                          double voxel, float *const *h_opts, float *const *h_ocol, int32_t *d_counts, void *ws,
                                          size_t ws_bytes, void *stream)
{
    return kpx::voxel_downsample_batch_spec(count, h_pts, h_col, h_n, voxel, h_opts, h_ocol, d_counts, ws, ws_bytes, stream, 0, nullptr, false);
}
int kpx::voxel_downsample_batch_spec(int32_t count, const float *const *h_pts, const float *const *h_col, const int64_t *h_n, double voxel,
                                     float *const *h_opts, float *const *h_ocol, int32_t *d_counts, void *ws, size_t ws_bytes, void *stream,
                                     int spec_bits, int32_t *d_bits, bool morton)
{
    KPX_REQUIRE(voxel > 0.0, "voxel_size <= 0");
    KPX_REQUIRE(count >= 1 && count <= 64 && h_pts && h_n && h_opts && d_counts && ws, "kpx_voxel_downsample_batch: bad arguments");
    for (int i = 0; i < count; ++i)
        KPX_REQUIRE(h_n[i] >= 0 && h_n[i] < ((int64_t)1 << 31) && (h_n[i] == 0 || (h_pts[i] && h_opts[i])),
                    "kpx_voxel_downsample_batch: bad cloud %d", i);
    hipStream_t st = (hipStream_t)stream;
    int64_t total = 0;
    for (int i = 0; i < count; ++i) total += h_n[i];
    if (count <= kVoxelBatchMax && total > 0 && total < ((int64_t)1 << 31)) {
        VoxelBatch b;
        b.count = count;
        static const int curve = [] { const char *e = getenv("KPX_VOXEL_CURVE"); return (e && e[0] == 'z') ? 1 : 2; }();
        b.morton = morton ? curve : 0;
        b.off[0] = 0;
        for (int i = 0; i < kVoxelBatchMax; ++i) {
            const bool on = i < count;
            b.pts[i] = on ? h_pts[i] : nullptr;
            b.col[i] = (on && h_col) ? h_col[i] : nullptr;
            b.opts[i] = on ? h_opts[i] : nullptr;
            b.ocol[i] = (on && h_col && h_ocol) ? h_ocol[i] : nullptr;
            b.off[i + 1] = b.off[i] + (on ? h_n[i] : 0);
        }
        Arena one(ws, ws_bytes);
        return voxel_batch_impl(b, voxel, d_counts, one, st, spec_bits, d_bits);
    }
    if (d_bits) KPX_HIP(hipMemsetAsync(d_bits, 0, sizeof(int32_t), st));
    if (count > kVoxelBatchMax && total > 0) {
        int gstart[65], ng = 0;
        bool ok = true;
        for (int i = 0; i < count;) {
            gstart[ng++] = i;
            int64_t gt = 0;
            int gc = 0;
            while (i < count && gc < kVoxelBatchMax) { gt += h_n[i]; ++gc; ++i; }
            ok = ok && gt < ((int64_t)1 << 31);
        }
        gstart[ng] = count;
        if (ok) {
            for (int g = 0; g < ng; ++g) {
                const int g0 = gstart[g], gc = gstart[g + 1] - g0;
                int64_t gt = 0;
                for (int i = 0; i < gc; ++i) gt += h_n[g0 + i];
                if (gt == 0) { KPX_HIP(hipMemsetAsync(d_counts + g0, 0, (size_t)gc * sizeof(int32_t), st)); continue; }
                VoxelBatch b;
                b.count = gc;
                b.morton = 0;
                b.off[0] = 0;
                for (int i = 0; i < kVoxelBatchMax; ++i) {
                    const bool on = i < gc;
                    b.pts[i] = on ? h_pts[g0 + i] : nullptr;
                    b.col[i] = (on && h_col) ? h_col[g0 + i] : nullptr;
                    b.opts[i] = on ? h_opts[g0 + i] : nullptr;
                    b.ocol[i] = (on && h_col && h_ocol) ? h_ocol[g0 + i] : nullptr;
                    b.off[i + 1] = b.off[i] + (on ? h_n[g0 + i] : 0);
                }
                Arena one(ws, ws_bytes);
                const int grc = voxel_batch_impl(b, voxel, d_counts + g0, one, st);
                if (grc) return grc;
            }
            return KPX_OK;
        }
    }
    LaneSet *ln = nullptr;
    int rc = lanes_get(&ln);
    if (rc) return rc;
    const int used = count < kLaneCount ? count : kLaneCount;
    rc = lanes_fork(ln, st, used);
    if (rc) return rc;
    Arena a(ws, ws_bytes);
    for (int i = 0; i < count && !rc; ++i) {
        hipStream_t ls = ln->s[i % kLaneCount];
        if (h_n[i] == 0) { rc = hipMemsetAsync(d_counts + i, 0, sizeof(int32_t), ls) == hipSuccess ? KPX_OK : fail(KPX_ERR_HIP, "memset failed"); continue; }
        rc = voxel_impl(h_pts[i], h_col ? h_col[i] : nullptr, nullptr, h_n[i], voxel, h_opts[i], (h_col && h_ocol) ? h_ocol[i] : nullptr, nullptr,
                        d_counts + i, a, ls);
    }
    const int jrc = lanes_join(ln, st, used);
    return rc ? rc : jrc;
}
```

kinectpy_amd/pipeline.py:

```python
from collections import deque
from concurrent.futures import ThreadPoolExecutor
from dataclasses import dataclass
import contextlib
import os
from typing import List, Optional

import numpy as np
import torch

from . import ops, parallel


ICP_MODES = {"p2p": 0, "p2plane": 1, "fixed": 2}


@dataclass
class PipelineParams:
    reg_voxel: float = 35.0
    normals_nn: int = 40
    icp_max_dist: float = 100.0
    icp_mode: str = "p2plane"
    icp_max_iteration: int = 30
    filt_voxel: float = 10.0
    filt_k: int = 20
# ... 78 lines not shown
        self.transforms = None
        self.last = {}
        self.order = None

    def _turn(self, stage):
        if self.order is None:
            return contextlib.nullcontext()
        return self.order[0].turn(self.order[1], stage)

    def calibrate(self, depth: torch.Tensor):
        return self._calibrate(depth, None)[0]

    def _calibrate(self, depth, queue_next):
        o, p = self.ops, self.p
        S = depth.shape[0]
        assert S == len(self.sensors)
        fp, _, _, fcnt = o.depth_to_cloud(depth, self.xy, None, S, False, False, sync=False)
        nxt = queue_next() if queue_next is not None else None
        fk = o._count(fcnt)
        downs = [d[0] for d in o.voxel_downsample_batch([fp[i, :fk[i]] for i in range(S)], p.reg_voxel)]
        owns_master = self.sensors[0] == 0
        master = downs[0] if owns_master else None
        tn = o.estimate_normals(master, 2.0 * p.reg_voxel, p.normals_nn) if (owns_master and p.icp_mode == "p2plane") else None
        with self._turn(0):
            master, tn = self._bcast(master, tn, device=fp.device)
        subs = downs[1:] if owns_master else downs
        ids = [g for g in self.sensors if g != 0]
        Ts = [np.eye(4)] if owns_master else []
        stats = []
        if subs:
            rs = o.icp_batch(subs, master, p.icp_max_dist, [self.init[g - 1] for g in ids], p.icp_mode, tn, p.icp_max_iteration)
            for r in rs:
                Ts.append(r["transformation"])
                stats.append((r["iterations"], r["fitness"], r["inlier_rmse"]))
        self.transforms = np.stack(Ts)
        self.last = {"icp": stats, "n_down": [int(d.shape[0]) for d in downs], "n_master": int(master.shape[0])}
        return self.transforms, nxt

    def fuse(self, depth: torch.Tensor, rgb: torch.Tensor, extracted=None):
        o, p = self.ops, self.p
        if self.transforms is None:
            raise RuntimeError("calibrate() first (or load transforms)")
        S = depth.shape[0]
        mp, mc, _, mcnt = extracted if extracted is not None else o.depth_to_cloud(depth, self.xy, rgb, S, True, True, gate=p.gate, sync=False)
        mk = o._count(mcnt)
        local = [(mp[i, :mk[i]], mc[i, :mk[i]]) for i in range(S)]
        with self._turn(1):
            segs, all_T, counts = self._xchg(local, self.transforms)
        owned = [len(parallel.shard_sensors(self.n_sensors, r, self.world)) for r in range(self.world)]
        Ts = np.concatenate([all_T[r, :owned[r]] for r in range(self.world)])
        clouds = [seg for r in range(self.world) for seg in segs[r][:owned[r]]]
        self.last.update(n_masked=[int(k) for k in mk], n_fused=int(counts.sum()), counts=[int(c) for c in counts.sum(1)])
        dist_on = parallel.collectives_on(self.group)
        if dist_on and self.fused_filter == "rank0" and self.rank != 0:
            return None, None, Ts
        vp, vc = o.fuse_voxel_downsample([c[0] for c in clouds], [c[1] for c in clouds], Ts, p.filt_voxel)
        M = int(vp.shape[0])
        if dist_on and self.fused_filter == "sharded" and M > 0:
            rows = -(-M // self.world)
            q0, q1 = min(M, self.rank * rows), min(M, (self.rank + 1) * rows)
            part, order = o.sor_partial(vp, p.filt_k, q0, q1)
            with self._turn(2):
                slabs = parallel.allgather_slabs(part, rows, self.group)
            keep, _, _ = o.sor_finish(slabs.reshape(-1)[:M], order, p.filt_ratio)
        else:
            if self.order is not None:
                self.order[0].skip(self.order[1], 2)
            if hasattr(o, "sor_select"):
                out_p, out_c, keep, _ = o.sor_select(vp, vc, p.filt_k, p.filt_ratio)
                self.last.update(n_voxel=M, n_out=int(out_p.shape[0]))
                return out_p, out_c, Ts
            keep, _, _ = o.sor(vp, p.filt_k, p.filt_ratio)
        out_p, out_c, _ = o.select_by_index([vp, vc], keep, trusted=True)
        self.last.update(n_voxel=M, n_out=int(out_p.shape[0]))
        return out_p, out_c, Ts

    def step(self, depth: torch.Tensor, rgb: torch.Tensor):
        o, p = self.ops, self.p
        S = depth.shape[0]
        _, masked = self._calibrate(depth, lambda: o.depth_to_cloud(depth, self.xy, rgb, S, True, True, gate=p.gate, sync=False))
        return self.fuse(depth, rgb, masked)


class NativeFramePipeline:

    def __init__(self, xy_table, n_sensors: int, init_transforms: List[np.ndarray], params: Optional[PipelineParams] = None,
                 out_ring: int = 0):
        self.p = params or PipelineParams()
        self.n_sensors = int(n_sensors)
        self._ring, self._ring_n, self._ring_k = [], int(out_ring), 0
        if len(init_transforms) != self.n_sensors - 1:
            raise ValueError("init_transforms: one 4x4 per sub sensor (sensors 1 .. n-1)")
        self.init = [np.asarray(T, dtype=np.float64) for T in init_transforms]
        self.xy = ops._dev(xy_table, torch.float32).reshape(-1)
        p = self.p
        self._c = ops.FrameParams(p.reg_voxel, p.icp_max_dist, p.filt_voxel, p.filt_ratio, p.gate, p.normals_nn,
                                  ICP_MODES[p.icp_mode], p.icp_max_iteration, p.filt_k)
        self.last = {}

    def step(self, depth: torch.Tensor, rgb: torch.Tensor):
        S = self.n_sensors
        out = None
        if self._ring_n:
            if len(self._ring) < self._ring_n:
                rows = S * int(depth.numel() // S)
                self._ring.append(tuple(torch.empty((rows, 3), dtype=torch.float32, device=self.xy.device) for _ in range(2)))
            out = self._ring[self._ring_k % len(self._ring)]
            self._ring_k += 1
        out_p, out_c, Ts, info = ops.frame_step(depth, rgb, self.xy, self.init, self._c, out=out)
        self.last = {"icp": [(int(info[32 + i]), None, None) for i in range(1, S)], "n_down": [int(v) for v in info[:S]],
                     "n_masked": [int(v) for v in info[16:16 + S]], "n_fused": int(info[16:16 + S].sum()), "n_voxel": int(info[48]),
                     "n_out": int(out_p.shape[0])}
        return out_p, out_c, Ts


class NativeShardPipeline:

    def __init__(self, xy_table, n_sensors: int, init_transforms: List[np.ndarray], params: Optional[PipelineParams] = None,
                 comm=None, fused_filter: str = "sharded", out_ring: int = 0):
        if comm is None:
            raise ValueError("NativeShardPipeline needs a communicator (parallel.NativeComm.rccl / staged / local)")
        self.p = params or PipelineParams()
        if self.p.icp_mode == "fixed":
            raise ValueError('icp_mode "fixed" (no registration in the frame) is a one-GPU form: SensorGroupPipeline / NativeFramePipeline')
        self.comm = comm
        self.n_sensors = int(n_sensors)
        if comm.world > self.n_sensors:
            raise ValueError(f"{comm.world} ranks for {self.n_sensors} sensors: a rank needs at least one sensor")
        self.sensors = parallel.shard_sensors(self.n_sensors, comm.rank, comm.world)
        if len(init_transforms) != self.n_sensors - 1:
            raise ValueError("init_transforms: one 4x4 per sub sensor (sensors 1 .. n-1)")
        self.init = [np.asarray(T, dtype=np.float64) for T in init_transforms]
        if fused_filter not in ("rank0", "sharded", "round_robin"):
            raise ValueError("fused_filter must be 'rank0', 'sharded' or 'round_robin'")
        self.fused_filter = fused_filter
        self.xy = ops._dev(xy_table, torch.float32).reshape(-1)
        p = self.p
        self._c = ops.FrameParams(p.reg_voxel, p.icp_max_dist, p.filt_voxel, p.filt_ratio, p.gate, p.normals_nn,
                                  ICP_MODES[p.icp_mode], p.icp_max_iteration, p.filt_k)
        self._ring, self._ring_n, self._ring_k = [], int(out_ring), 0
        self.order = None
        self.native_order = True
        self.retries = 0
        self.last = {}

    def step(self, depth: torch.Tensor, rgb: torch.Tensor):
        from . import _lib
        S = self.n_sensors
        out = None
        if self._ring_n:
            if len(self._ring) < self._ring_n:
                rows = S * int(depth.numel() // max(1, len(self.sensors)))
                self._ring.append(tuple(torch.empty((rows, 3), dtype=torch.float32, device=self.xy.device) for _ in range(2)))
            out = self._ring[self._ring_k % len(self._ring)]
            self._ring_k += 1
        order, frame = self.order if self.order is not None else (None, None)
        while True:
            res = ops.frame_step_sharded(self.comm, order, frame, depth, rgb, self.xy, S, self.init, self._c,
                                         {"sharded": 0, "rank0": 1, "round_robin": 2}[self.fused_filter], out=out)
            if res is not _lib.RETRY:
                break
            self.retries += 1
            if order is not None:
                if self._ring_n:
                    self._ring_k -= 1
                return _lib.RETRY
        out_p, out_c, Ts, info = res
        self.last = {"icp": [(int(info[32 + i]), None, None) for i in range(1, S)], "n_down": [int(v) for v in info[:S]],
                     "n_masked": [int(v) for v in info[16:16 + S]], "n_fused": int(info[16:16 + S].sum()), "n_voxel": int(info[48]),
                     "n_out": int(out_p.shape[0])}
        return out_p, out_c, Ts


class FrameStream:

    def __init__(self, pipe, depth: int = 2):
        self.pipes = list(pipe) if isinstance(pipe, (list, tuple)) else None
        self.depth = len(self.pipes) if self.pipes else max(1, int(depth))
        self.pipe = self.pipes[0] if self.pipes else pipe
        self.device = torch.cuda.current_device()
        self.streams = [torch.cuda.Stream(device=self.device) for _ in range(self.depth)]
        self.pool = ThreadPoolExecutor(max_workers=self.depth)
        self.pending = deque()
        self.submitted = 0
        native = self.pipes is not None and all(getattr(p_, "native_order", False) for p_ in self.pipes)
        ordered = self.pipes is not None and self.depth > 1 and all(hasattr(p_, "order") for p_ in self.pipes) and \
            (native or parallel.collectives_on(getattr(self.pipes[0], "group", None)))
        look = int(os.environ.get("KPX_ORDER_LOOKAHEAD", "2"))
        self.order = parallel.CollectiveOrder(max(1, min(self.depth, look + 1)), native=native) if ordered else None

    def _run(self, slot, depth, rgb, frame=None):
        torch.cuda.set_device(self.device)
        stream = self.streams[slot]
        pipe = self.pipes[slot] if self.pipes else self.pipe
        try:
            with torch.cuda.stream(stream):
                if not depth.is_cuda and not isinstance(pipe, (NativeFramePipeline, NativeShardPipeline)):
                    depth = depth.to(self.device, non_blocking=True)
                    rgb = rgb.to(self.device, non_blocking=True)
                if frame is not None:
                    pipe.order = (self.order, frame)
                out = pipe.step(depth, rgb)
                stream.synchronize()
        finally:
            if frame is not None:
                pipe.order = None
                self.order.finish(frame)
        return out

    def full(self) -> bool:
        return len(self.pending) >= self.depth

    def submit(self, depth: torch.Tensor, rgb: torch.Tensor):
        assert not self.full()
        slot = self.submitted % self.depth
        self.submitted += 1
        frame = self.order.submit() if self.order is not None else None
        fut = self.pool.submit(self._run, slot, depth, rgb, frame)
        fut.frame, fut.args = frame, (slot, depth, rgb)
# ... 139 lines not shown
```

Baseline: 2460.

## Batch per-frame counter clears, cache xy NaN mask, fold result copy into kernel

Allocates one per-frame clear region, zeroed by a single memset, from which compaction counters, median histograms and radix-sort counters are carved. This replaces several separate memset dispatches. The xy-table NaN mask is now cached across frames per thread and invalidated by a generation counter bumped from Python when a new table is set. The ICP result mirror copy is folded into fuse_mean_kernel, which drops a device-to-host memcpy when masked points exist. The aim is fewer small dispatches per frame, at the cost of a cache that can go stale if the xy table changes in place without notification.

```diff
diff --git a/include/kinectpx.h b/include/kinectpx.h
--- a/include/kinectpx.h
+++ b/include/kinectpx.h
@@ -230,6 +230,7 @@
     int32_t icp_max_iteration;
     int32_t filt_k;
 } kpx_frame_params;
+int kpx_xy_table_changed(void);
 size_t kpx_frame_step_workspace_bytes(int32_t sensors, int64_t n_px);
 int kpx_frame_step(const uint16_t *depth, const uint8_t *rgb, const float *xy_table, int64_t n_px, int32_t sensors,
                    const double *h_init, const kpx_frame_params *params, float *out_pts, float *out_col, int32_t *h_count,
diff --git a/kinectpy_amd/_lib.py b/kinectpy_amd/_lib.py
--- a/kinectpy_amd/_lib.py
+++ b/kinectpy_amd/_lib.py
@@ -114,6 +114,7 @@
     "kpx_order_log": (C.c_int, [_vp, _vp, _i64, _vp]),
     "kpx_frame_step_sharded_workspace_bytes": (_sz, [_i32, _i32, _i32, _i64, _i32]),
     "kpx_frame_step_sharded": (C.c_int, [_vp, _vp, _i64, _vp, _vp, _i32, _vp, _i64, _i32, _vp, _vp, _i32, _vp, _vp, _vp, _vp, _vp, _vp, _sz, _vp]),
+    "kpx_xy_table_changed": (C.c_int, []),
     "kpx_stream_workspace_bytes": (_sz, [_i32, _i32, _i32, _i64, _i32]),
     "kpx_stream_create": (C.c_int, [_vp, _i64, _i32, _vp, _vp, _i32, _vp, _i32, _vp, _sz, _vp]),
     "kpx_stream_submit": (C.c_int, [_vp, _vp, _vp, _i32, _vp, _vp]),
diff --git a/kinectpy_amd/csrc/kpx_common.h b/kinectpy_amd/csrc/kpx_common.h
--- a/kinectpy_amd/csrc/kpx_common.h
+++ b/kinectpy_amd/csrc/kpx_common.h
@@ -47,6 +47,19 @@
             return kpx::fail(KPX_ERR_WORKSPACE, "workspace too small: need %zu bytes, have %zu",   \
                              (a).off, (a).cap);                                                    \
     } while (0)
+
+struct ClearArena {
+    char *base;
+    size_t off, cap;
+    void *take(size_t bytes)
+    {
+        bytes = (bytes + 255) & ~(size_t)255;
+        if (!base || off + bytes > cap) return nullptr;
+        void *p = base + off;
+        off += bytes;
+        return p;
+    }
+};
 
 static inline int64_t cdiv(int64_t a, int64_t b) { return (a + b - 1) / b; }
 
diff --git a/kinectpy_amd/csrc/kpx_extract.hip b/kinectpy_amd/csrc/kpx_extract.hip
--- a/kinectpy_amd/csrc/kpx_extract.hip
+++ b/kinectpy_amd/csrc/kpx_extract.hip
@@ -459,21 +459,28 @@
     if (tid == 0) d_median[frame] = 0.5 * ((double)s_val[0] + (double)s_val[1]);
 }
 
+static void xy_nanmask_launch(const float *xy, int64_t n, uint8_t *mask, hipStream_t st)
+{
+    hipLaunchKernelGGL(xy_nanmask_kernel, dim3((unsigned)(cdiv(n / 8, 256) > 1024 ? 1024 : cdiv(n / 8, 256))), dim3(256), 0, st, xy, n / 8, mask);
+}
+
 static int median_impl(const int16_t *v, int64_t n, int64_t stride, int64_t frame_stride, int32_t frames,
-                       double *d_median, Arena &a, hipStream_t st, const float *xy = nullptr, void *clear_from = nullptr)
+                       double *d_median, Arena &a, hipStream_t st, const float *xy = nullptr, void *clear_from = nullptr,
+                       uint32_t *hist_clear = nullptr, const uint8_t *mask_ready = nullptr)
 {
     uint32_t *hist = a.get<uint32_t>((size_t)frames * 512);
     MedianSel *sel = a.get<MedianSel>((size_t)frames);
-    uint8_t *nanmask = (xy || (a.dry && n > 0)) ? a.get<uint8_t>((size_t)(n / 8 + 1)) : nullptr;
+    uint8_t *own_mask = (xy || (a.dry && n > 0)) ? a.get<uint8_t>((size_t)(n / 8 + 1)) : nullptr;
     if (a.dry) return KPX_OK;
     KPX_ARENA_CHECK(a);
-    {
+    const uint8_t *nanmask = (xy && mask_ready) ? mask_ready : own_mask;
+    if (hist_clear) hist = hist_clear;
+    else {
         char *c0 = clear_from ? reinterpret_cast<char *>(clear_from) : reinterpret_cast<char *>(hist);
         KPX_HIP(hipMemsetAsync(c0, 0, (size_t)(reinterpret_cast<char *>(hist + (size_t)frames * 512) - c0), st));
     }
     const bool vec = stride == 1 && (n % 8 == 0) && (frame_stride % 8 == 0) && ((uintptr_t)v % 16 == 0) && ((uintptr_t)xy % 16 == 0);
-    if (xy && vec)
-        hipLaunchKernelGGL(xy_nanmask_kernel, dim3((unsigned)(cdiv(n / 8, 256) > 1024 ? 1024 : cdiv(n / 8, 256))), dim3(256), 0, st, xy, n / 8, nanmask);
+    if (xy && vec && !mask_ready) xy_nanmask_launch(xy, n, own_mask, st);
     {
         const char *e = getenv("KPX_MEDIAN_FRAME");
         const bool by_frame = e ? e[0] == '1' : (frames >= 64 && n >= 32768);
@@ -832,22 +839,32 @@
 
 static int depth_to_cloud_impl(const uint16_t *depth, const float *xy, const uint8_t *rgb, int64_t n, int32_t frames,
                                int32_t flags, double gate, float *pts, float *col, int32_t *idx, int32_t *d_count,
-                               Arena &a, hipStream_t st)
+                               Arena &a, hipStream_t st, ClearArena *clr = nullptr, const uint8_t *mask_ready = nullptr)
 {
     int32_t *counts = a.get<int32_t>((size_t)frames * compact_ws_ints(n));
     double *med = a.get<double>((size_t)frames);
     int rc = KPX_OK;
     const bool gated = (flags & KPX_COMPACT_DEPTH_GATE) != 0;
+    uint32_t *hist_clear = nullptr;
+    bool pre = false;
+    if (clr && !a.dry) {
+        const size_t cb = ((size_t)frames * compact_ws_ints(n) * sizeof(int32_t) + 255) & ~(size_t)255;
+        if (char *blk = static_cast<char *>(clr->take(cb + (gated ? (size_t)frames * 512 * sizeof(uint32_t) : 0)))) {
+            counts = reinterpret_cast<int32_t *>(blk);
+            if (gated) hist_clear = reinterpret_cast<uint32_t *>(blk + cb);
+            pre = true;
+        }
+    }
     if (gated || a.dry)
-        rc = median_impl(reinterpret_cast<const int16_t *>(depth), n, 1, n, frames, med, a, st, xy, counts);
+        rc = median_impl(reinterpret_cast<const int16_t *>(depth), n, 1, n, frames, med, a, st, xy, counts, hist_clear, mask_ready);
     if (a.dry || rc) return rc;
     KPX_ARENA_CHECK(a);
     DepthPred pred{ depth, xy, rgb, med, n, flags, gate };
     DepthEmit emit{ depth, xy, rgb, n, pts, col, idx };
     ProfScope prof(KPX_PROF_COMPACT, (double)frames * (double)n * (2.0 + (rgb ? 3.0 : 0.0)), st);
     const bool vec = (n % 8 == 0) && (((uintptr_t)depth | (uintptr_t)xy) % 16 == 0) && ((uintptr_t)rgb % 8 == 0);
-    if (!vec) return compact(pred, emit, n, frames, counts, d_count, st, gated);
-    return px8_compact(depth, xy, rgb, med, n, frames, flags, gate, counts, pts, col, idx, d_count, st, gated);
+    if (!vec) return compact(pred, emit, n, frames, counts, d_count, st, gated || pre);
+    return px8_compact(depth, xy, rgb, med, n, frames, flags, gate, counts, pts, col, idx, d_count, st, gated || pre);
 }
 KPX_EXPORT int kpx_rgbd_compact(const int16_t *xyz, const uint8_t *rgb, int64_t n, int32_t frames, int32_t flags,
                                 const double *d_median, double gate, float *pts, float *col, int32_t *idx,
@@ -888,3 +905,18 @@
     Arena a(ws, ws_bytes);
     return depth_to_cloud_impl(depth, xy, rgb, n_px, frames, flags, gate, pts, col, idx, d_count, a, (hipStream_t)stream);
 }
+
+int kpx::depth_to_cloud_frame(const uint16_t *depth, const float *xy, const uint8_t *rgb, int64_t n_px, int32_t frames, int32_t flags, double gate,
+                              float *pts, float *col, int32_t *d_count, void *ws, size_t ws_bytes, void *stream, ClearArena *clr, const uint8_t *xy_mask)
+{
+    KPX_REQUIRE(n_px > 0 && n_px < ((int64_t)1 << 31) && frames > 0 && frames <= max_compact_frames(), "kpx_depth_to_cloud: bad size");
+    Arena a(ws, ws_bytes);
+    return depth_to_cloud_impl(depth, xy, rgb, n_px, frames, flags, gate, pts, col, nullptr, d_count, a, (hipStream_t)stream, clr, xy_mask);
+}
+bool kpx::xy_nanmask_used(const float *xy, int64_t n_px) { return n_px % 8 == 0 && (uintptr_t)xy % 16 == 0; }
+int kpx::xy_nanmask_build(const float *xy, int64_t n_px, uint8_t *mask, void *stream)
+{
+    xy_nanmask_launch(xy, n_px, mask, (hipStream_t)stream);
+    KPX_LAUNCH_CHECK();
+    return KPX_OK;
+}
diff --git a/kinectpy_amd/csrc/kpx_frame.hip b/kinectpy_amd/csrc/kpx_frame.hip
--- a/kinectpy_amd/csrc/kpx_frame.hip
+++ b/kinectpy_amd/csrc/kpx_frame.hip
@@ -1,7 +1,15 @@
+#include <atomic>
 #include <chrono>
 #include <vector>
 
 #include "kpx_internal.h"
+#include "kpx_radix.h"
+
+#define KPX_SUB(call)                    \
+    do {                                 \
+        const int rc__ = (call);         \
+        if (rc__) return rc__;           \
+    } while (0)
 
 namespace kpx {
 
@@ -45,7 +53,44 @@
     }
 }
 
+constexpr size_t kFrameClearMax = (size_t)1 << 20;
+static size_t frame_clear_bytes(int32_t S, int64_t n_px, int64_t fused_pts)
+{
+    auto r256 = [](size_t b) { return (b + 255) & ~(size_t)255; };
+    const int64_t reg = (int64_t)S * n_px < kRadixMaxPairs ? (int64_t)S * n_px : kRadixMaxPairs, fus = fused_pts < kRadixMaxPairs ? fused_pts : kRadixMaxPairs;
+    const size_t states = r256((size_t)S * compact_ws_ints(n_px) * sizeof(int32_t));
+    size_t b = 2 * states + r256((size_t)S * 512 * sizeof(uint32_t));
+    b += r256(radix_clear_bytes(reg) + (size_t)compact_ws_ints(reg) * sizeof(int32_t));
+    b += r256(radix_clear_bytes(fus) + (size_t)compact_ws_ints(fus) * sizeof(int32_t));
+    return b < kFrameClearMax ? b : kFrameClearMax;
+}
+
+static std::atomic<uint64_t> g_xy_generation{ 1 };
+static int frame_xy_mask(const float *xy, int64_t n_px, hipStream_t st, const uint8_t **out)
+{
+    static thread_local struct { const float *xy; int64_t n_px; uint64_t gen; uint8_t *mask; size_t cap; } c = { nullptr, 0, 0, nullptr, 0 };
+    *out = nullptr;
+    if (!xy_nanmask_used(xy, n_px)) return KPX_OK;
+    const uint64_t gen = g_xy_generation.load(std::memory_order_acquire);
+    if (!(c.mask && c.xy == xy && c.n_px == n_px && c.gen == gen)) {
+        const size_t need = (size_t)(n_px / 8 + 1);
+        if (c.cap < need) {
+            if (c.mask) (void)hipFree(c.mask);
+            c.mask = nullptr; c.cap = 0;
+            KPX_HIP(hipMalloc((void **)&c.mask, need));
+            c.cap = need;
+        }
+        c.xy = nullptr;
+        KPX_SUB(xy_nanmask_build(xy, n_px, c.mask, st));
+        c.xy = xy; c.n_px = n_px; c.gen = gen;
+    }
+    *out = c.mask;
+    return KPX_OK;
+}
+
 struct FrameLayout {
+    char *clear;
+    size_t clear_bytes;
     float *full_pts, *mask_pts, *mask_col, *down_pts, *normals, *vox_pts, *vox_col;
     int32_t *vox_cnt, *keep_idx;
     double *icp_res, *sor_stats;
@@ -56,6 +101,8 @@
 static void frame_carve(Arena &a, int32_t S, int64_t n_px, FrameLayout *L)
 {
     const size_t px = (size_t)n_px, all = (size_t)S * px;
+    L->clear_bytes = frame_clear_bytes(S, n_px, (int64_t)all);
+    L->clear = a.get<char>(L->clear_bytes);
     L->full_pts = a.get<float>(all * 3);
     L->mask_pts = a.get<float>(all * 3);
     L->mask_col = a.get<float>(all * 3);
@@ -83,6 +130,12 @@
 
 using namespace kpx;
 
+KPX_EXPORT int kpx_xy_table_changed(void)
+{
+    g_xy_generation.fetch_add(1, std::memory_order_acq_rel);
+    return KPX_OK;
+}
+
 KPX_EXPORT size_t kpx_frame_step_workspace_bytes(int32_t sensors, int64_t n_px)
 {
     if (sensors < 1 || n_px < 1) return 0;
@@ -91,12 +144,6 @@
     frame_carve(a, sensors, n_px, &L);
     return a.off;
 }
-
-#define KPX_SUB(call)                    \
-    do {                                 \
-        const int rc__ = (call);         \
-        if (rc__) return rc__;           \
-    } while (0)
 
 KPX_EXPORT int kpx_frame_step(const uint16_t *depth, const uint8_t *rgb, const float *xy_table, int64_t n_px, int32_t sensors,
                               const double *h_init, const kpx_frame_params *prm, float *out_pts, float *out_col, int32_t *h_count,
@@ -132,10 +179,14 @@
     }
     auto negative = [&](const int32_t *c, int n) { for (int i = 0; i < n; ++i) if (c[i] < 0) return c[i]; return 0; };
 
-    if (!fixed) KPX_SUB(kpx_depth_to_cloud(depth, xy_table, nullptr, n_px, S, 0, prm->gate, L.full_pts, nullptr, nullptr, h_i, L.op_ws, L.op_bytes, st));
+    ClearArena clr{ L.clear, 0, L.clear_bytes };
+    KPX_HIP(hipMemsetAsync(L.clear, 0, L.clear_bytes, st));
+    const uint8_t *xy_mask = nullptr;
+    KPX_SUB(frame_xy_mask(xy_table, n_px, st, &xy_mask));
+    if (!fixed) KPX_SUB(depth_to_cloud_frame(depth, xy_table, nullptr, n_px, S, 0, prm->gate, L.full_pts, nullptr, h_i, L.op_ws, L.op_bytes, st, &clr, xy_mask));
     else for (int i = 0; i < S; ++i) h_i[i] = 0;
-    KPX_SUB(kpx_depth_to_cloud(depth, xy_table, rgb, n_px, S, KPX_COMPACT_COLOR_MASK | KPX_COMPACT_DEPTH_GATE, prm->gate, L.mask_pts, L.mask_col, nullptr,
-                               h_i + 16, L.op_ws, L.op_bytes, st));
+    KPX_SUB(depth_to_cloud_frame(depth, xy_table, rgb, n_px, S, KPX_COMPACT_COLOR_MASK | KPX_COMPACT_DEPTH_GATE, prm->gate, L.mask_pts, L.mask_col,
+                                 h_i + 16, L.op_ws, L.op_bytes, st, &clr, xy_mask));
     static const int extra_dispatches = [] { const char *e = getenv("KPX_FRAME_EXTRA_DISPATCHES"); return e ? atoi(e) : 0; }();
     for (int e = 0; e < extra_dispatches; ++e) hipLaunchKernelGGL(frame_empty_kernel, dim3(1), dim3(64), 0, st);
     std::vector<int64_t> fk((size_t)S), mk((size_t)S), dk((size_t)S);
@@ -153,7 +204,7 @@
     for (int i = 0; i < S; ++i) h_i[32 + i] = 0;
     for (int attempt = 0; attempt < 2 && !fixed; ++attempt) {
         KPX_SUB(voxel_downsample_batch_spec(S, p_in.data(), nullptr, fk.data(), prm->reg_voxel, p_out.data(), nullptr, h_i + 32, L.op_ws, L.op_bytes, st,
-                                            attempt == 0 ? spec_bits : 0, h_i + 50, zorder));
+                                            attempt == 0 ? spec_bits : 0, h_i + 50, zorder, &clr));
         KPX_SUB(frame_wait(st));
         const int need = h_i[50];
         const bool narrow = attempt == 0 && spec_bits > 0 && need > spec_bits;
@@ -185,11 +236,14 @@
     }
     static thread_local int fuse_spec = 0;
     if (!speculate) fuse_spec = 0;
+    int64_t masked_total = 0;
+    for (int i = 0; i < S; ++i) masked_total += mk[(size_t)i];
+    const FuseMirror mirror{ L.icp_res, h_d, S * 20, reinterpret_cast<int32_t *>(h_d + (size_t)S * 20) };
     for (int attempt = 0; attempt < 2; ++attempt) {
         h_i[51] = 0;
         KPX_SUB(fuse_voxel_downsample_dev(S, p_in.data(), c_in.data(), mk.data(), h_T, dT.data(), prm->filt_voxel, L.vox_pts, L.vox_col, L.vox_cnt, L.op_ws,
-                                          L.op_bytes, st, attempt == 0 ? fuse_spec : 0, h_i + 51));
-        KPX_HIP(hipMemcpyAsync(h_d, L.icp_res, ((size_t)S * 20 + 1) * sizeof(double), hipMemcpyDeviceToHost, st));
+                                          L.op_bytes, st, attempt == 0 ? fuse_spec : 0, h_i + 51, &clr, &mirror));
+        if (masked_total == 0) KPX_HIP(hipMemcpyAsync(h_d, L.icp_res, ((size_t)S * 20 + 1) * sizeof(double), hipMemcpyDeviceToHost, st));
         KPX_SUB(frame_wait(st));
         const int need = h_i[51];
         const bool narrow = attempt == 0 && fuse_spec > 0 && need > fuse_spec;
@@ -286,6 +340,8 @@
 }
 
 struct ShardLayout {
+    char *clear;
+    size_t clear_bytes;
     uint16_t *stage_depth;
     uint8_t *stage_rgb;
     float *full_pts, *mask_pts, *mask_col, *down_pts, *normals, *vox_pts, *vox_col;
@@ -301,6 +357,8 @@
     const size_t px = (size_t)n_px, loc = (size_t)S_l * px, all = (size_t)S * px;
     L->k_max = (S + world - 1) / world;
     L->hdr_bytes = ((size_t)L->k_max * kHdrDoubles * sizeof(double) + 255) & ~(size_t)255;
+    L->clear_bytes = frame_clear_bytes(S_l > 0 ? S_l : 1, n_px, (int64_t)all);
+    L->clear = a.get<char>(L->clear_bytes);
     L->stage_depth = host_input ? a.get<uint16_t>(loc) : nullptr;
     L->stage_rgb = host_input ? a.get<uint8_t>(loc * 3) : nullptr;
     L->full_pts = a.get<float>(loc * 3);
@@ -398,9 +456,13 @@
         depth = L.stage_depth;
         rgb = L.stage_rgb;
     }
-    KPX_SUB(kpx_depth_to_cloud(depth, xy_table, nullptr, n_px, S_l, 0, prm->gate, L.full_pts, nullptr, nullptr, h_i, L.op_ws, L.op_bytes, st));
-    KPX_SUB(kpx_depth_to_cloud(depth, xy_table, rgb, n_px, S_l, KPX_COMPACT_COLOR_MASK | KPX_COMPACT_DEPTH_GATE, prm->gate, L.mask_pts, L.mask_col, nullptr,
-                               h_i + 16, L.op_ws, L.op_bytes, st));
+    ClearArena clr{ L.clear, 0, L.clear_bytes };
+    KPX_HIP(hipMemsetAsync(L.clear, 0, L.clear_bytes, st));
+    const uint8_t *xy_mask = nullptr;
+    KPX_SUB(frame_xy_mask(xy_table, n_px, st, &xy_mask));
+    KPX_SUB(depth_to_cloud_frame(depth, xy_table, nullptr, n_px, S_l, 0, prm->gate, L.full_pts, nullptr, h_i, L.op_ws, L.op_bytes, st, &clr, xy_mask));
+    KPX_SUB(depth_to_cloud_frame(depth, xy_table, rgb, n_px, S_l, KPX_COMPACT_COLOR_MASK | KPX_COMPACT_DEPTH_GATE, prm->gate, L.mask_pts, L.mask_col,
+                                 h_i + 16, L.op_ws, L.op_bytes, st, &clr, xy_mask));
     std::vector<int64_t> fk((size_t)S_l), mk((size_t)S_l), dk((size_t)S_l);
     std::vector<const float *> p_in((size_t)S_l);
     std::vector<float *> p_out((size_t)S_l);
@@ -414,7 +476,7 @@
     int &spec_bits = comm_spec_bits(comm);
     for (int attempt = 0; attempt < 2 && !lerr; ++attempt) {
         KPX_SUB(voxel_downsample_batch_spec(S_l, p_in.data(), nullptr, fk.data(), prm->reg_voxel, p_out.data(), nullptr, h_i + 32, L.op_ws, L.op_bytes, st,
-                                            attempt == 0 ? spec_bits : 0, h_i + 50, zorder));
+                                            attempt == 0 ? spec_bits : 0, h_i + 50, zorder, &clr));
         KPX_SUB(frame_wait(st));
         const int need = h_i[50];
         const bool narrow = attempt == 0 && spec_bits > 0 && need > spec_bits;
@@ -561,7 +623,7 @@
     for (int attempt = 0; attempt < 2; ++attempt) {
         h_i[51] = 0;
         KPX_SUB(fuse_voxel_downsample_dev(S, f_p.data(), f_c.data(), f_n.data(), h_T, nullptr, prm->filt_voxel, L.vox_pts, L.vox_col, L.vox_cnt, L.op_ws,
-                                          L.op_bytes, st, attempt == 0 ? fuse_spec : 0, h_i + 51));
+                                          L.op_bytes, st, attempt == 0 ? fuse_spec : 0, h_i + 51, &clr));
         KPX_HIP(hipMemcpyAsync(h_i + 48, L.vox_cnt, sizeof(int32_t), hipMemcpyDeviceToHost, st));
         KPX_SUB(frame_wait(st));
         const int need_bits = h_i[51];
diff --git a/kinectpy_amd/csrc/kpx_internal.h b/kinectpy_amd/csrc/kpx_internal.h
--- a/kinectpy_amd/csrc/kpx_internal.h
+++ b/kinectpy_amd/csrc/kpx_internal.h
@@ -35,13 +35,25 @@
 int lanes_fork(LaneSet *l, hipStream_t caller, int used);
 int lanes_join(LaneSet *l, hipStream_t caller, int used);
 
+int depth_to_cloud_frame(const uint16_t *depth, const float *xy, const uint8_t *rgb, int64_t n_px, int32_t frames, int32_t flags, double gate,
+                         float *pts, float *col, int32_t *d_count, void *ws, size_t ws_bytes, void *stream, ClearArena *clr, const uint8_t *xy_mask);
+bool xy_nanmask_used(const float *xy, int64_t n_px);
+int xy_nanmask_build(const float *xy, int64_t n_px, uint8_t *mask, void *stream);
+
 int voxel_downsample_batch_spec(int32_t count, const float *const *h_pts, const float *const *h_col, const int64_t *h_n, double voxel,
                                 float *const *h_opts, float *const *h_ocol, int32_t *d_counts, void *ws, size_t ws_bytes, void *stream,
-                                int spec_bits, int32_t *d_bits, bool morton = false);
+                                int spec_bits, int32_t *d_bits, bool morton = false, ClearArena *clr = nullptr);
+
+struct FuseMirror {
+    const double *src;
+    double *dst;
+    int32_t n;
+    int32_t *count;
+};
 
 int fuse_voxel_downsample_dev(int32_t count, const float *const *h_pts, const float *const *h_col, const int64_t *h_n, const double *h_T,
                               const double *const *h_dT, double voxel, float *opts, float *ocol, int32_t *d_count, void *ws, size_t ws_bytes,
-                              void *stream, int spec_bits = 0, int32_t *d_bits = nullptr);
+                              void *stream, int spec_bits = 0, int32_t *d_bits = nullptr, ClearArena *clr = nullptr, const FuseMirror *mirror = nullptr);
 
 struct BusyScope {
     BusyScope();
diff --git a/kinectpy_amd/csrc/kpx_knn.hip b/kinectpy_amd/csrc/kpx_knn.hip
--- a/kinectpy_amd/csrc/kpx_knn.hip
+++ b/kinectpy_amd/csrc/kpx_knn.hip
@@ -166,7 +166,7 @@
     g->extra = reinterpret_cast<int32_t *>(zero + 32);
     unsigned long long *scan_states = reinterpret_cast<unsigned long long *>(zero + 32 + kGridExtraWords);
     uint32_t *count1 = zero + 32 + kGridExtraWords + kGridScanWords, *count2 = count1 + (size_t)cell_cap + 1, *cursor = count2 + (size_t)cell_cap + 1;
-    KPX_HIP(hipMemsetAsync(zero, 0, (32 + kGridExtraWords + kGridScanWords + 3 * ((size_t)cell_cap + 1)) * sizeof(uint32_t), st));
+    KPX_HIP(hipMemsetAsync(zero, 0, ((32 + kGridExtraWords + kGridScanWords + 3 * ((size_t)cell_cap + 1)) * sizeof(uint32_t) + 15) & ~(size_t)15, st));
     int nb = (int)(cdiv(n, 256) > 4096 ? 4096 : cdiv(n, 256));
     hipLaunchKernelGGL(grid_cell_kernel, dim3(nb), dim3(256), 0, st, pts, n, bbox, target_per_cell, cell_cap, (const unsigned long long *)nullptr, g->params,
                        keys_in, vals_in, count1);
diff --git a/kinectpy_amd/csrc/kpx_radix.h b/kinectpy_amd/csrc/kpx_radix.h
--- a/kinectpy_amd/csrc/kpx_radix.h
+++ b/kinectpy_amd/csrc/kpx_radix.h
@@ -141,13 +141,14 @@
     }
 }
 
+static inline size_t radix_clear_bytes(int64_t n) { return (size_t)4 * radix_groups(n) * 256 * sizeof(uint32_t); }
 static inline int radix_sort_pairs_u32(const RadixScratch &s, const uint32_t *keys_in, uint32_t *keys_out, const int32_t *vals_in, int32_t *vals_out,
-                                       int64_t n, int end_bit, hipStream_t st, const void *clear_end = nullptr)
+                                       int64_t n, int end_bit, hipStream_t st, const void *clear_end = nullptr, bool is_clear = false)
 {
     if (n <= 0) return KPX_OK;
     const int passes = radix_passes(end_bit);
     const int tiles = (int)radix_tiles(n), groups = (int)radix_groups(n);
-    {
+    if (!is_clear) {
         char *c0 = reinterpret_cast<char *>(s.group_hist);
         const char *c1 = clear_end ? reinterpret_cast<const char *>(clear_end) : c0 + (size_t)passes * groups * 256 * sizeof(uint32_t);
         KPX_HIP(hipMemsetAsync(c0, 0, (size_t)(c1 - c0), st));
diff --git a/kinectpy_amd/csrc/kpx_stream.hip b/kinectpy_amd/csrc/kpx_stream.hip
--- a/kinectpy_amd/csrc/kpx_stream.hip
+++ b/kinectpy_amd/csrc/kpx_stream.hip
@@ -157,6 +157,7 @@
     KPX_REQUIRE(need > 0, "kpx_stream_create: bad shape");
     if (ws_bytes < need) return fail(KPX_ERR_WORKSPACE, "workspace too small: need %zu bytes, have %zu", need, ws_bytes);
     std::unique_ptr<kpx_stream> S(new kpx_stream());
+    (void)kpx_xy_table_changed();
     KPX_HIP(hipGetDevice(&S->dev));
     S->depth = depth; S->sensors = sensors; S->n_px = n_px; S->xy = xy_table; S->prm = *prm; S->fused_filter = fused_filter;
     S->sharded = comms != nullptr;
diff --git a/kinectpy_amd/csrc/kpx_voxel.hip b/kinectpy_amd/csrc/kpx_voxel.hip
--- a/kinectpy_amd/csrc/kpx_voxel.hip
+++ b/kinectpy_amd/csrc/kpx_voxel.hip
@@ -394,6 +394,15 @@
     RadixScratch rx;
     char *counts_end;
 };
+static bool sort_counters_take(ClearArena *clr, int64_t total, RadixScratch *rx, int32_t **counts)
+{
+    const size_t gh = radix_clear_bytes(total);
+    char *blk = clr ? static_cast<char *>(clr->take(gh + (size_t)compact_ws_ints(total) * sizeof(int32_t))) : nullptr;
+    if (!blk) return false;
+    rx->group_hist = reinterpret_cast<uint32_t *>(blk);
+    *counts = reinterpret_cast<int32_t *>(blk + gh);
+    return true;
+}
 static void voxel_batch_carve(Arena &a, int64_t total, VoxelBatchScratch *s)
 {
     const size_t nn = (size_t)(total > 0 ? total : 1);
@@ -412,7 +421,7 @@
     s->counts_end = reinterpret_cast<char *>(s->counts + (size_t)compact_ws_ints(total));
 }
 static int voxel_batch_impl(const VoxelBatch &b, double voxel, int32_t *d_counts, Arena &a, hipStream_t st, int spec_bits = 0,
-                            int32_t *d_bits = nullptr)
+                            int32_t *d_bits = nullptr, ClearArena *clr = nullptr)
 {
     const int64_t total = b.off[b.count];
     VoxelBatchScratch s;
@@ -445,7 +454,8 @@
         static const bool vendor_sort = [] { const char *e = getenv("KPX_RADIX"); return e && e[0] == '0'; }();
         bool cleared = false;
         if (total <= kRadixMaxPairs && !vendor_sort) {
-            rc = radix_sort_pairs_u32(s.rx, k_in, k_out, s.vals_in, s.vals_out, total, end_bit, st, s.counts_end);
+            const bool pre = sort_counters_take(clr, total, &s.rx, &s.counts);
+            rc = radix_sort_pairs_u32(s.rx, k_in, k_out, s.vals_in, s.vals_out, total, end_bit, st, s.counts_end, pre);
             if (rc) return rc;
             cleared = true;
         } else {
@@ -587,10 +597,17 @@
 }
 __global__ __launch_bounds__(256) void fuse_mean_kernel(FuseBatch b, const int32_t *__restrict__ vals, const int32_t *__restrict__ seg_start,
                                                         int32_t *__restrict__ d_count, const int32_t *__restrict__ err, float *__restrict__ opts,
-                                                        float *__restrict__ ocol)
+                                                        float *__restrict__ ocol, FuseMirror mir)
 {
     const int32_t m_total = *d_count;
-    if (blockIdx.x == 0 && threadIdx.x == 0 && *err) *d_count = KPX_ERR_RANGE;
+    if (blockIdx.x == 0) {
+        if (threadIdx.x == 0) {
+            const int32_t c = *err ? KPX_ERR_RANGE : m_total;
+            if (*err) *d_count = c;
+            if (mir.count) *mir.count = c;
+        }
+        for (int t = threadIdx.x; t < mir.n; t += blockDim.x) mir.dst[t] = mir.src[t];
+    }
     const int64_t total = b.off[b.count];
     for (int64_t m = (int64_t)blockIdx.x * blockDim.x + threadIdx.x; m < m_total; m += (int64_t)gridDim.x * blockDim.x) {
         const int64_t s0 = seg_start[m], s1 = (m + 1 < m_total) ? seg_start[m + 1] : total;
@@ -655,8 +672,9 @@
     s->sort_tmp = a.get<char>(s->sort_bytes);
 }
 static int fuse_voxel_impl(const FuseBatch &b, double voxel, float *opts, float *ocol, int32_t *d_count, Arena &a, hipStream_t st, int spec_bits = 0,
-                           int32_t *d_bits = nullptr)
-{
+                           int32_t *d_bits = nullptr, ClearArena *clr = nullptr, const FuseMirror *mirror = nullptr)
+{
+    const FuseMirror mir = mirror ? *mirror : FuseMirror{ nullptr, nullptr, 0, nullptr };
     const int64_t total = b.off[b.count];
     FuseScratch s;
     fuse_carve(a, total, &s);
@@ -667,11 +685,12 @@
     if (spec_bits > 0 && spec_bits <= 32 && d_bits && total <= kRadixMaxPairs) {
         uint32_t *k_in = reinterpret_cast<uint32_t *>(s.keys_in), *k_out = reinterpret_cast<uint32_t *>(s.keys_out);
         hipLaunchKernelGGL(fuse_key32_kernel, dim3(nb), dim3(256), 0, st, b, s.bbox, voxel, k_in, s.vals_in, d_bits);
-        int rc = radix_sort_pairs_u32(s.rx, k_in, k_out, s.vals_in, s.vals_out, total, spec_bits, st, s.counts_end);
+        const bool pre = sort_counters_take(clr, total, &s.rx, &s.counts);
+        int rc = radix_sort_pairs_u32(s.rx, k_in, k_out, s.vals_in, s.vals_out, total, spec_bits, st, s.counts_end, pre);
         if (rc) return rc;
         rc = compact(HeadPredT<uint32_t>{ k_out }, HeadEmit{ s.seg_start }, total, 1, s.counts, d_count, st, true);
         if (rc) return rc;
-        hipLaunchKernelGGL(fuse_mean_kernel, dim3(nb), dim3(256), 0, st, b, s.vals_out, s.seg_start, d_count, s.err, opts, ocol);
+        hipLaunchKernelGGL(fuse_mean_kernel, dim3(nb), dim3(256), 0, st, b, s.vals_out, s.seg_start, d_count, s.err, opts, ocol, mir);
         KPX_LAUNCH_CHECK();
         return KPX_OK;
     }
@@ -681,7 +700,7 @@
     KPX_HIP(hipcub::DeviceRadixSort::SortPairs(s.sort_tmp, bytes, s.keys_in, s.keys_out, s.vals_in, s.vals_out, (int)total, 0, 63, st));
     int rc = compact(HeadPred{ s.keys_out }, HeadEmit{ s.seg_start }, total, 1, s.counts, d_count, st);
     if (rc) return rc;
-    hipLaunchKernelGGL(fuse_mean_kernel, dim3(nb), dim3(256), 0, st, b, s.vals_out, s.seg_start, d_count, s.err, opts, ocol);
+    hipLaunchKernelGGL(fuse_mean_kernel, dim3(nb), dim3(256), 0, st, b, s.vals_out, s.seg_start, d_count, s.err, opts, ocol, mir);
     KPX_LAUNCH_CHECK();
     return KPX_OK;
 }
@@ -705,7 +724,7 @@
 }
 int kpx::fuse_voxel_downsample_dev(int32_t count, const float *const *h_pts, const float *const *h_col, const int64_t *h_n, const double *h_T,
                                    const double *const *h_dT, double voxel, float *opts, float *ocol, int32_t *d_count, void *ws, size_t ws_bytes,
-                                   void *stream, int spec_bits, int32_t *d_bits)
+                                   void *stream, int spec_bits, int32_t *d_bits, ClearArena *clr, const FuseMirror *mirror)
 {
     KPX_REQUIRE(voxel > 0.0, "voxel_size <= 0");
     KPX_REQUIRE(count >= 1 && count <= kFuseMax, "kpx_fuse_voxel_downsample: 1 .. %d clouds", kFuseMax);
@@ -733,7 +752,7 @@
     if (total == 0) { KPX_HIP(hipMemsetAsync(d_count, 0, sizeof(int32_t), st)); return KPX_OK; }
     KPX_REQUIRE(opts, "kpx_fuse_voxel_downsample: null pointer");
     Arena a(ws, ws_bytes);
-    return fuse_voxel_impl(b, voxel, opts, (any_col && all_col) ? ocol : nullptr, d_count, a, st, spec_bits, d_bits);
+    return fuse_voxel_impl(b, voxel, opts, (any_col && all_col) ? ocol : nullptr, d_count, a, st, spec_bits, d_bits, clr, mirror);
 }
 
 KPX_EXPORT size_t kpx_voxel_workspace_bytes(int64_t n)
@@ -796,7 +815,7 @@
 }
 int kpx::voxel_downsample_batch_spec(int32_t count, const float *const *h_pts, const float *const *h_col, const int64_t *h_n, double voxel,
                                      float *const *h_opts, float *const *h_ocol, int32_t *d_counts, void *ws, size_t ws_bytes, void *stream,
-                                     int spec_bits, int32_t *d_bits, bool morton)
+                                     int spec_bits, int32_t *d_bits, bool morton, ClearArena *clr)
 {
     KPX_REQUIRE(voxel > 0.0, "voxel_size <= 0");
     KPX_REQUIRE(count >= 1 && count <= 64 && h_pts && h_n && h_opts && d_counts && ws, "kpx_voxel_downsample_batch: bad arguments");
@@ -821,7 +840,7 @@
             b.off[i + 1] = b.off[i] + (on ? h_n[i] : 0);
         }
         Arena one(ws, ws_bytes);
-        return voxel_batch_impl(b, voxel, d_counts, one, st, spec_bits, d_bits);
+        return voxel_batch_impl(b, voxel, d_counts, one, st, spec_bits, d_bits, clr);
     }
     if (d_bits) KPX_HIP(hipMemsetAsync(d_bits, 0, sizeof(int32_t), st));
     if (count > kVoxelBatchMax && total > 0) {
diff --git a/kinectpy_amd/pipeline.py b/kinectpy_amd/pipeline.py
--- a/kinectpy_amd/pipeline.py
+++ b/kinectpy_amd/pipeline.py
@@ -184,6 +184,11 @@
         return self.fuse(depth, rgb, masked)
 
 
+def _new_xy_table():
+    from . import _lib
+    _lib.load().kpx_xy_table_changed()
+
+
 class NativeFramePipeline:
 
     def __init__(self, xy_table, n_sensors: int, init_transforms: List[np.ndarray], params: Optional[PipelineParams] = None,
@@ -195,6 +200,7 @@
             raise ValueError("init_transforms: one 4x4 per sub sensor (sensors 1 .. n-1)")
         self.init = [np.asarray(T, dtype=np.float64) for T in init_transforms]
         self.xy = ops._dev(xy_table, torch.float32).reshape(-1)
+        _new_xy_table()
         p = self.p
         self._c = ops.FrameParams(p.reg_voxel, p.icp_max_dist, p.filt_voxel, p.filt_ratio, p.gate, p.normals_nn,
                                   ICP_MODES[p.icp_mode], p.icp_max_iteration, p.filt_k)
@@ -237,6 +243,7 @@
             raise ValueError("fused_filter must be 'rank0', 'sharded' or 'round_robin'")
         self.fused_filter = fused_filter
         self.xy = ops._dev(xy_table, torch.float32).reshape(-1)
+        _new_xy_table()
         p = self.p
         self._c = ops.FrameParams(p.reg_voxel, p.icp_max_dist, p.filt_voxel, p.filt_ratio, p.gate, p.normals_nn,
                                   ICP_MODES[p.icp_mode], p.icp_max_iteration, p.filt_k)
```

Result: no change. 2456 (median of 2 runs) (-0.2%).
